# WHU-USI3DV/LaneMapping

Measured on AMD Instinct MI355X. Metric: BEV tiles/sec end-to-end (LAS points -> polylines), higher is better.
Workload: dtype f32; 1 GPU; on-GPU LAS->BEV raster (4,194,304 points/tile resident in HBM) + configs/Proj_polyline_fpn_vit_vertex_2.py, batch=16 per GPU, seeded random weights; lines_per_tile=45, streams=2, hip_graphs=True, points=resident, stream_check=not run (--full runs it), gather_check=n/a (1 rank), raster_check=not run (--full runs it), dist_ranks=1, rccl_ranks=1

## Files before the change

include/lanemap_hip.h:

```cpp
#ifndef LANEMAP_HIP_H
#define LANEMAP_HIP_H
#include <stdint.h>
#ifdef __cplusplus
extern "C" {
#endif

enum { LM_OK = 0, LM_ERR_ARG = 1, LM_ERR_HIP = 2, LM_ERR_NO_DEVICE = 3, LM_ERR_CAPACITY = 4 };
enum { LM_ACT_NONE = 0, LM_ACT_RELU = 1, LM_ACT_GELU = 2 };

int lm_abi_version(void);
const char* lm_last_error(void);
int lm_device_count(void);

int lm_conv2d_nhwc_mfma_f32(void* stream, const float* x, int ldx, const float* wp, int CoutP,
                            const float* scale, const float* shift, const float* res, int ldr, int res_rows,
                            float* y, int ldy, int B, int H, int W, int Cin, int Cout, int KH, int KW,
                            int stride, int pad_h, int pad_w, int dil, int act);
int lm_conv2d_nhwc_mfma_resup_f32(void* stream, const float* x, int ldx, const float* wp, int CoutP, const float* scale,
                                  const float* shift, const float* res_coarse, int ldr, int Hr, int Wr, float* y, int ldy,
                                  int B, int H, int W, int Cin, int Cout, int KH, int KW, int stride, int pad_h, int pad_w,
                                  int dil, int act);

int lm_winograd44_supported(int H, int W, int Cin, int dil);
int lm_winograd44_gn_chunks(int H, int W, int dil);
long lm_winograd44_tiles(int B, int H, int W, int dil);
long lm_winograd44_twin_workspace_bytes(int B, int H, int W, int Cin, int CoutP, int dil);
int lm_conv3x3_winograd44_f32(void* stream, const float* x, int ldx, const float* wu_frag, int CoutP, const float* scale,
                              const float* shift, const float* res, int ldr, float* y, int ldy, int B, int H, int W,
                              int Cin, int Cout, int dil, int act, double* gn_partial);
int lm_conv3x3_winograd44_twin_f32(void* stream, const float* x, int ldx, const float* wu, int CoutP, const float* scale,
                                   const float* shift, const float* res, int ldr, float* y, int ldy, int B, int H, int W,
                                   int Cin, int Cout, int dil, int act, void* workspace, long workspace_bytes);
int lm_wino44_split_fragments(void* stream, const float* frag, float* out, long n_quads);
int lm_conv3x3_winograd44_split_f32(void* stream, const float* x, int ldx, const float* wu_split, int CoutP, const float* scale,
                                    const float* shift, const float* res, int ldr, float* y, int ldy, int B, int H, int W,
                                    int Cin, int Cout, int dil, int act, double* gn_partial, float post);
int lm_conv3x3_winograd44_split_twin_f32(void* stream, const float* x, int ldx, const float* wu, int CoutP, const float* scale,
                                         const float* shift, const float* res, int ldr, float* y, int ldy, int B, int H, int W,
                                         int Cin, int Cout, int dil, int act, void* workspace, long workspace_bytes, float post);

int lm_conv2d_nhwc_mfma_f32_gnstats(void* stream, const float* x, int ldx, const float* wp, int CoutP, const float* shift,
                                    float* y, int ldy, double* gn_partial, int B, int H, int W, int Cin, int Cout,
                                    int KH, int KW, int stride, int pad_h, int pad_w, int dil);
int lm_gn_finalize(void* stream, const double* partial, float* stats, int B, int HW, int C, int nchunk, float eps);
int lm_gn_finalize_split(void* stream, const double* partial, float* stats, int B, int HW, int C, int nchunk, float eps, int split);

int lm_stem_conv7x7_bn_relu(void* stream, const float* x_chw, const float* w_k64, const float* scale,
                            const float* shift, float* y_nhwc, int B, int H, int W);
int lm_stem_conv7x7_bn_relu_u8(void* stream, const unsigned char* x_hwc3, const float* w_k64, const float* scale,
                               const float* shift, float* y_nhwc, int B, int H, int W);
int lm_maxpool3x3s2_nhwc(void* stream, const float* x, float* y, int B, int H, int W, int C);
int lm_conv2d_nhwc_small(void* stream, const float* x, int ldx, const float* w_tc16, const float* scale,
                         const float* shift, float* y, int ldy, int B, int H, int W, int Cin, int Cout,
                         int KH, int KW, int stride, int pad_h, int pad_w, int pre_relu, int act);

int lm_gn_stats(void* stream, const float* x, double* workspace, float* stats, int B, int HW, int C, float eps);
long lm_gn_stats_workspace_bytes(int B, int HW, int C);
int lm_gn_relu_upsample(void* stream, const float* x, const float* stats, const float* gamma, const float* beta,
                        float* y, int B, int Hi, int Wi, int Ho, int Wo, int C, int accumulate);
int lm_gn_relu_upsample_sum(void* stream, int n, const float* const* x, const float* const* stats, const int* Hi, const int* Wi,
                            const int* ldx , const float* gamma, const float* beta,
                            float* y, int B, int Ho, int Wo, int C);
int lm_gn_relu_upsample_sum_conv1x1(void* stream, int n, const float* const* x, const float* const* stats, const int* Hi, const int* Wi,
                                    const int* ldx, const float* gamma, const float* beta, float* y, int B, int Ho, int Wo, int C,
                                    const float* w_c16, const float* bias, int cout, float* y1, int ldy1);
int lm_upsample_bilinear_nhwc(void* stream, const float* x, int ldx, const float* add, int lda, float* y, int ldy,
                              int B, int Hi, int Wi, int Ho, int Wo, int C);
int lm_upsample_bilinear_to_chw(void* stream, const float* x, int ldx, float* y_chw, int B, int Hi, int Wi,
                                int Ho, int Wo, int C);
int lm_layernorm_rows(void* stream, const float* x, const float* gamma, const float* beta, float* y,
                      long rows, int D, float eps);
int lm_unpatchify(void* stream, const float* tokens, float* y_nhwc, int B, int G, int P, int C);
int lm_token_mix_mfma_f32(void* stream, const float* x, const float* wt, int ldw, const float* bias, const float* res, float* y,
                          int B, int M, int K, int N, int act);

int lm_attention_f32(void* stream, const float* qkv, float* out, int B, int N, int heads, int dim_head, float scale);
int lm_attention_masked_f32(void* stream, const float* qkv, float* out, const int* valid, int B, int N, int heads, int dim_head, float scale);

int lm_head_tokens(void* stream, const float* seg, const float* row_nhwc16, float* tok, float seg_bias,
                   int B, int P, int Hr, int Wr, int prop_width, int half_buff);
int lm_head_tokens_window(void* stream, const float* row_nhwc16, float* tok, int B, int P, int Hr, int Wr, int prop_width, int half_buff);
int lm_head_stage2(void* stream, const float* hid, int ldh, int D, const float* w2, const float* b2,
                   float* ext2, float* cls2, float* off2, long M);
int lm_head_proposal_conf(void* stream, const float* tok, const float* wt, const float* bias, float* conf,
                          int BP, int L);

int lm_head_endpoint_tile(void);
int lm_head_endpoint(void* hip_stream, const float* col, int ldc, const float* x_endp, const float* w1p, const float* b1,
                     const float* bn_scale, const float* bn_shift, const float* w2, const float* b2, float* out, int B, int h, int w,
                     int H, int W);

int lm_decode_proposals(void* stream, const float* pconf, const float* ext2, const float* cls2, const float* off2,
                        float* prop_conf, float* v_ext, float* cls_conf, int* cls_idx, double* cls_offset,
                        int B, int P, int R, float exist_thre, int prop_width, int half_buff);
int lm_decode_orient(void* stream, const float* x_nhwc, int ldx, int C, unsigned char* y, long pixels);
int lm_decode_semantic(void* stream, const float* logit_chw3, unsigned char* sem, float* biseg, float* rows,
                       int B, int H, int W, float thre, int raw_mode);
long lm_endp_topk_workspace_bytes(int B);
int lm_endp_topk(void* stream, const float* endp_logit, void* workspace, int* out_idx, float* out_score,
                 int* out_status, int B, int H, int W, int clip, int K);

int lm_pack_segments(void* stream, int n, const void* const* src, const long* bytes, const long* dst_offsets, void* dst);


typedef struct {
    float quat[4];
    float trans[3];
    float bev_img_offset[2];
    float img_reso[2];
    float local_min_ele;
    float ele_reso;
    float inten_lo, inten_hi;
} LmRasterParams;
long lm_bev_raster_workspace_bytes(int B, long max_points_per_tile, int H, int W);
int lm_bev_raster_batch(void* stream, const float* points_xyzi, const long* tile_offsets, const LmRasterParams* params,
                        int B, void* workspace, long workspace_bytes, float* out_chw, unsigned char* out_hwc_u8,
                        int H, int W);
int lm_bev_raster_batch_scaled(void* hip_stream, const float* points_xyzi, const long* tile_offsets, const LmRasterParams* params,
                               int B, void* workspace, long workspace_bytes, float* out_chw, unsigned char* out_hwc_u8,
                               int H, int W, const float* inten_scale);
int lm_tile_ingest_u8(void* stream, const unsigned char* src_hwc, float* dst_chw, int B, int H, int W, int C);

typedef struct {
    double x0, y0, cell;
    int nx, ny;
} LmStripGrid;
int lm_strip_build_grid(const LmRasterParams* params, int T, int H, int W, double z_lo, double z_hi, LmStripGrid* grid,
                        unsigned short* cells, long cells_cap);
long lm_strip_bin_workspace_bytes(long N, int T);
int lm_strip_bin_points(void* hip_stream, const float* points_xyzi, long N, const LmRasterParams* params, int T, int H, int W,
                        double z_lo, double z_hi, void* workspace, long workspace_bytes, long* counts, long* offsets,
                        long* offsets_host, float* binned, long capacity);

long lm_tile_ground_workspace_bytes(int B, int H, int W, int cell_px);
int lm_tile_ground(void* hip_stream, const float* points_xyzi, const long* tile_offsets, const LmRasterParams* params, int B, int H,
                   int W, int cell_px, void* workspace, long workspace_bytes, float* ground, float* ground_min, float* cell_min);
long lm_ground_select_workspace_bytes(long N, int B);
int lm_ground_select(void* hip_stream, const float* points_xyzi, const long* tile_offsets, const LmRasterParams* params, int B, int H,
                     int W, int cell_px, const float* ground, float h_lo, float h_hi, void* workspace, long workspace_bytes,
                     float* points_out, long* out_offsets, long* out_offsets_host);

long lm_tile_intensity_workspace_bytes(int B, int G);
int lm_tile_intensity_window(void* hip_stream, const float* points_xyzi, const long* tile_offsets, const LmRasterParams* params, int B,
                             int H, int W, const int* group, int G, int q_lo_ppm, int q_hi_ppm, void* workspace, long workspace_bytes,
                             int* window, long* count, unsigned* coarse_hist);

long lm_drape_workspace_bytes(long n_vertices, int B, int radius_px);
int lm_drape_vertices(void* hip_stream, const float* points_xyzi, const long* tile_offsets, const LmRasterParams* params, int B, int H,
                      int W, const int* vertices_rc, const long* vertex_offsets, int radius_px, void* workspace, long workspace_bytes,
                      float* z, int* npix, float* pixel_min);

int lm_tile_gap_hist(void* hip_stream, const unsigned char* tiles_hwc_u8, int B, int H, int W, int max_radius_px, unsigned* hist);
int lm_tile_gap_fill(void* hip_stream, const unsigned char* tiles_hwc_u8, int B, int H, int W, const int* radius_px,
                     unsigned char* out_hwc_u8);

int lm_endp_cluster(const int* topk_idx, int n_avail, int Wc, int clip, int k0, int k_step, int k_max, int radius,
                    int min_clusters, int* out_hw, int max_out, int* n_out, int* k_used);
int lm_polyline_assemble(const float* prop_conf, const float* prop_v_ext, const double* cls_offset,
                         const float* bi_seg_rows, const int* endp_hw, int n_endp, int P, int R, float obj_thre,
                         int min_vertices, double* out_lanes, int* endp_keep);
int lm_raster_polylines(const double* lanes, int P, int R, unsigned char* out);
int lm_line8(unsigned char* out, int x1, int y1, int x2, int y2, int colour);
int lm_trace_lines(const double* cols, int n, int R, const float* seg_rows, double* out);
int lm_polyline_backproject(unsigned char* bev_hwc, int H, int W, int C, const double* img_seqs, const int* seq_lens, int L,
                            int Vmax, const double* params13, const double* las_read_offset, double* out);
int lm_polyline_backproject_z(unsigned char* bev_hwc, int H, int W, int C, const double* img_seqs, const int* seq_lens, int L,
                              int Vmax, const double* params13, const double* las_read_offset, double* out,
                              const float* vertex_z, int fit);

long lm_skeletonize_lee_2d(unsigned char* img, int H, int W);

void* lm_merge_create(void);
void lm_merge_destroy(void* merger);
int lm_merge_add_tile(void* merger, const double* points, const int* lens, int n);
long lm_merge_finish(void* merger, long* total_points);
int lm_merge_result(void* merger, double* points, int* lens);
int lm_downsample_seq(const double* seq, int n, double dist_min, double* out);

int lm_softmax_rows(void* stream, float* x, long rows, int cols);
int lm_rowref_select(void* stream, const float* ext, const float* cls, float* mean_out, int* valid, float thr_ext, int* corr,
                     int B, int H, int W, int L);
int lm_rowref_gather(void* stream, const float* x_nhwc8, const int* corr, float* tok, int B, int H, int W, int L);
int lm_rowref_scatter(void* stream, const float* x_nhwc8, const float* tok, const int* corr, const int* valid,
                      float* y_nhwc8, int B, int H, int W, int L);
int lm_rowref_gather_win(void* hip_stream, const float* x_nhwc8, const int* corr, float* tok, int B, int H, int W, int L, int off_grid);
int lm_rowref_scatter_win(void* hip_stream, const float* x_nhwc8, const float* tok, const int* corr, const int* valid,
                          float* y_nhwc8, int B, int H, int W, int L, int off_grid);
int lm_rowref_decode(void* stream, const float* ext2, const float* cls2, unsigned char* conf, unsigned char* cls_map,
                     int* col_idx, int B, int H, int W, int L);

long lm_voxelize_workspace_bytes(long n_points);
long lm_scan_workspace_bytes(long n);
int lm_exclusive_scan_u32(void* stream, const unsigned* in, unsigned* out, long n, void* workspace, long workspace_bytes);
long lm_sort_pairs_workspace_bytes(long n);
int lm_sort_pairs_u32(void* stream, unsigned* keys_io, unsigned* vals_io, long n, int end_bit, void* workspace, long workspace_bytes);
int lm_voxelize_hard(void* stream, const float* points, long n, const float* range_lo_xyz, const float* voxel_size_xyz,
                     const int* grid_xyz, int max_points, int max_voxels, int batch_idx, const int* row_base, int cap_rows,
                     float* feats, int ldf, int* coords, int* row_end, int raster_order, void* workspace,
                     long workspace_bytes);
int lm_sparse_grid_build(void* stream, const int* coords, long n, int* grid, int B, int D, int H, int W);
long lm_sparse_conv_outputs_workspace_bytes(long out_cells);
int lm_sparse_conv_outputs(void* stream, const int* in_coords, long n_in, int B, const int* ksp_zyx9, int Do, int Ho, int Wo,
                           int* out_grid, int* out_coords, int cap_rows, int* out_count, void* workspace, long workspace_bytes);
int lm_sparse_rulebook(void* stream, const int* out_coords, long n_out, const int* in_grid, int B, int D, int H, int W,
                       const int* ksp_zyx9, int* nbr);
int lm_conv_gather_mfma_f32(void* stream, const float* x, int ldx, const int* nbr, int taps, const float* wp, int CoutP,
                            const float* scale, const float* shift, const float* res, int ldr, float* y, int ldy,
                            long M, int Cin, int Cout, int act);
int lm_sparse_to_dense_nhwc(void* stream, const float* feats, int ldf, const int* coords, long n, float* out, int B, int D,
                            int H, int W, int C, int flip_h);
int lm_upsample_bicubic_nhwc(void* stream, const float* x, float* y, int B, int H, int W, int C, int Ho, int Wo);

typedef struct {
    int version_major, version_minor, point_format, record_len;
    long n_points, offset_to_points;
    double scale[3], offset[3], min_xyz[3], max_xyz[3];
} LmLasHeader;
int lm_las_parse_header(const unsigned char* bytes, long len, LmLasHeader* out);
int lm_las_decode_points(void* stream, const unsigned char* records, int record_len, long n, const double* scale,
                         const double* offset, const double* shift, float inten_lo, float inten_hi, int normalise,
                         float* out_xyzi);
enum { LM_LAS_DROP_SYNTHETIC = 1, LM_LAS_DROP_KEYPOINT = 2, LM_LAS_DROP_WITHHELD = 4, LM_LAS_DROP_OVERLAP = 8 };
enum { LM_LAS_RETURNS_ALL = 0, LM_LAS_RETURNS_FIRST = 1, LM_LAS_RETURNS_LAST = 2, LM_LAS_RETURNS_SINGLE = 3 };
typedef struct { unsigned class_mask[8]; unsigned drop_flags; int returns; float z_lo, z_hi; } LmLasSelect;
long lm_las_select_workspace_bytes(long n);
int lm_las_decode_select(void* hip_stream, const unsigned char* records, int record_len, int point_format, long n,
                         const double* scale, const double* offset, const double* shift, float inten_lo, float inten_hi,
                         int normalise, const LmLasSelect* select, void* workspace, long workspace_bytes, float* out_xyzi,
                         long* kept, unsigned long* class_hist);

typedef struct {
    double x0, y0, cell;
    int nx, ny, min_line, max_line;
    long n_segments, n_entries;
    float half_width;
} LmLineGrid;
int lm_line_index_build(const float* segments, long S, float half_width, double cell, LmLineGrid* grid, int* cell_start,
                        long cell_start_cap, int* cell_segs, long cell_segs_cap);
int lm_label_points(void* hip_stream, const float* points_xyzi, long N, const float* segments, long S, const LmLineGrid* grid,
                    const int* cell_start, const int* cell_segs, float half_width, float z_tol, float min_intensity, int* line,
                    float* dist2);
int lm_las_label_records(void* hip_stream, const unsigned char* records, int record_len, int point_format, long n, const double* scale,
                         const double* offset, const double* shift, const LmLasSelect* select, const float* segments, long S,
                         const LmLineGrid* grid, const int* cell_start, const int* cell_segs, float half_width, float z_tol,
                         float min_intensity, int marking_class, int write_line_id, unsigned char* records_out, int* line,
                         unsigned long* counts, int L);

int lm_line_profile_points(void* hip_stream, const float* points_xyzi, long N, const float* segments, long S, const LmLineGrid* grid,
                           const int* cell_start, const int* cell_segs, float half_width, const float* stations, const int* bin_start,
                           const int* bin_start_host, int L, double bin, float z_tol, float min_intensity, int accumulate, long* bins,
                           long n_bins);
int lm_las_line_profile_records(void* hip_stream, const unsigned char* records, int record_len, int point_format, long n,
                                const double* scale, const double* offset, const double* shift, const LmLasSelect* select,
                                const float* segments, long S, const LmLineGrid* grid, const int* cell_start, const int* cell_segs,
                                float half_width, const float* stations, const int* bin_start, const int* bin_start_host, int L, double bin,
                                float z_tol, float min_intensity, int accumulate, long* bins, long n_bins);

int lm_png_info(const unsigned char* data, long size, int* H, int* W, int* C);
int lm_png_decode_u8(const unsigned char* data, long size, unsigned char* out_hwc, long out_bytes);
int lm_png_decode_files_u8(const char* const* paths, int n, unsigned char* out_nhwc, int H, int W, int C, int threads);
int lm_zlib_inflate(const unsigned char* data, long size, unsigned char* out, long capacity, long* produced);

long lm_lane_json_text(const double* lane_vertexes, int n_lines, int row_size, int with_pervertex_semantics, char* out, long cap);
int lm_lane_json_write(const double* lane_vertexes, int n_lines, int row_size, int with_pervertex_semantics, const char* path);
int lm_seqs_json_write(const double* seqs, const int* lens, int L, int Vmax, int D, const char* path);

#ifdef __cplusplus
}
#endif
#endif
```

lanemapping_amd/_lib.py:

```python
import ctypes as C
import os

_HERE = os.path.dirname(os.path.abspath(__file__))
LIB_PATH = os.environ.get('LANEMAP_HIP_LIB') or os.path.join(_HERE, 'liblanemap_hip.so')

c_f32p = C.POINTER(C.c_float)
vp, i32, i64, f32 = C.c_void_p, C.c_int, C.c_long, C.c_float


class LmRasterParams(C.Structure):
    _fields_ = [('quat', C.c_float * 4), ('trans', C.c_float * 3), ('bev_img_offset', C.c_float * 2),
                ('img_reso', C.c_float * 2), ('local_min_ele', C.c_float), ('ele_reso', C.c_float),
                ('inten_lo', C.c_float), ('inten_hi', C.c_float)]


class LmLasHeader(C.Structure):
    _fields_ = [('version_major', C.c_int), ('version_minor', C.c_int), ('point_format', C.c_int), ('record_len', C.c_int),
                ('n_points', C.c_long), ('offset_to_points', C.c_long), ('scale', C.c_double * 3), ('offset', C.c_double * 3),
                ('min_xyz', C.c_double * 3), ('max_xyz', C.c_double * 3)]


class LmStripGrid(C.Structure):
    _fields_ = [('x0', C.c_double), ('y0', C.c_double), ('cell', C.c_double), ('nx', C.c_int), ('ny', C.c_int)]


class LmLasSelect(C.Structure):
    _fields_ = [('class_mask', C.c_uint * 8), ('drop_flags', C.c_uint), ('returns', C.c_int), ('z_lo', C.c_float), ('z_hi', C.c_float)]


class LmLineGrid(C.Structure):
    _fields_ = [('x0', C.c_double), ('y0', C.c_double), ('cell', C.c_double), ('nx', C.c_int), ('ny', C.c_int), ('min_line', C.c_int),
                ('max_line', C.c_int), ('n_segments', C.c_long), ('n_entries', C.c_long), ('half_width', C.c_float)]


SIGNATURES = {
    'lm_abi_version': (i32, []),
    'lm_last_error': (C.c_char_p, []),
    'lm_device_count': (i32, []),
    'lm_conv2d_nhwc_mfma_f32': (i32, [vp, vp, i32, vp, i32, vp, vp, vp, i32, i32, vp, i32,
                                      i32, i32, i32, i32, i32, i32, i32, i32, i32, i32, i32, i32]),
    'lm_conv2d_nhwc_mfma_resup_f32': (i32, [vp, vp, i32, vp, i32, vp, vp, vp, i32, i32, i32, vp, i32,
                                            i32, i32, i32, i32, i32, i32, i32, i32, i32, i32, i32, i32]),
    'lm_winograd44_supported': (i32, [i32, i32, i32, i32]),
    'lm_winograd44_gn_chunks': (i32, [i32, i32, i32]),
    'lm_winograd44_tiles': (i64, [i32, i32, i32, i32]),
    'lm_winograd44_twin_workspace_bytes': (i64, [i32, i32, i32, i32, i32, i32]),
    'lm_conv3x3_winograd44_f32': (i32, [vp, vp, i32, vp, i32, vp, vp, vp, i32, vp, i32, i32, i32, i32, i32, i32, i32, i32, vp]),
    'lm_conv3x3_winograd44_twin_f32': (i32, [vp, vp, i32, vp, i32, vp, vp, vp, i32, vp, i32, i32, i32, i32, i32, i32, i32, i32, vp, i64]),
    'lm_wino44_split_fragments': (i32, [vp, vp, vp, i64]),
    'lm_conv3x3_winograd44_split_f32': (i32, [vp, vp, i32, vp, i32, vp, vp, vp, i32, vp, i32, i32, i32, i32, i32, i32, i32, i32, vp, f32]),
    'lm_conv3x3_winograd44_split_twin_f32': (i32, [vp, vp, i32, vp, i32, vp, vp, vp, i32, vp, i32, i32, i32, i32, i32, i32, i32, i32, vp, i64, f32]),
    'lm_conv2d_nhwc_mfma_f32_gnstats': (i32, [vp, vp, i32, vp, i32, vp, vp, i32, vp] + [i32] * 11),
    'lm_gn_finalize': (i32, [vp, vp, vp, i32, i32, i32, i32, f32]),
    'lm_gn_finalize_split': (i32, [vp, vp, vp, i32, i32, i32, i32, f32, i32]),
    'lm_stem_conv7x7_bn_relu': (i32, [vp, vp, vp, vp, vp, vp, i32, i32, i32]),
    'lm_stem_conv7x7_bn_relu_u8': (i32, [vp, vp, vp, vp, vp, vp, i32, i32, i32]),
    'lm_maxpool3x3s2_nhwc': (i32, [vp, vp, vp, i32, i32, i32, i32]),
    'lm_conv2d_nhwc_small': (i32, [vp, vp, i32, vp, vp, vp, vp, i32, i32, i32, i32, i32, i32, i32, i32, i32, i32, i32, i32, i32]),
    'lm_gn_stats': (i32, [vp, vp, vp, vp, i32, i32, i32, f32]),
    'lm_gn_stats_workspace_bytes': (i64, [i32, i32, i32]),
    'lm_gn_relu_upsample': (i32, [vp, vp, vp, vp, vp, vp, i32, i32, i32, i32, i32, i32, i32]),
    'lm_gn_relu_upsample_sum': (i32, [vp, i32, vp, vp, vp, vp, vp, vp, vp, vp, i32, i32, i32, i32]),
    'lm_gn_relu_upsample_sum_conv1x1': (i32, [vp, i32, vp, vp, vp, vp, vp, vp, vp, vp, i32, i32, i32, i32, vp, vp, i32, vp, i32]),
    'lm_upsample_bilinear_nhwc': (i32, [vp, vp, i32, vp, i32, vp, i32, i32, i32, i32, i32, i32, i32]),
    'lm_upsample_bilinear_to_chw': (i32, [vp, vp, i32, vp, i32, i32, i32, i32, i32, i32]),
    'lm_layernorm_rows': (i32, [vp, vp, vp, vp, vp, i64, i32, f32]),
    'lm_token_mix_mfma_f32': (i32, [vp, vp, vp, i32, vp, vp, vp, i32, i32, i32, i32, i32]),
    'lm_unpatchify': (i32, [vp, vp, vp, i32, i32, i32, i32]),
    'lm_attention_f32': (i32, [vp, vp, vp, i32, i32, i32, i32, f32]),
    'lm_attention_masked_f32': (i32, [vp, vp, vp, vp, i32, i32, i32, i32, f32]),
    'lm_head_tokens': (i32, [vp, vp, vp, vp, f32, i32, i32, i32, i32, i32, i32]),
    'lm_head_tokens_window': (i32, [vp, vp, vp, i32, i32, i32, i32, i32, i32]),
    'lm_head_stage2': (i32, [vp, vp, i32, i32, vp, vp, vp, vp, vp, i64]),
    'lm_head_proposal_conf': (i32, [vp, vp, vp, vp, vp, i32, i32]),
    'lm_head_endpoint_tile': (i32, []),
    'lm_head_endpoint': (i32, [vp, vp, i32, vp, vp, vp, vp, vp, vp, vp, vp, i32, i32, i32, i32, i32]),
    'lm_decode_proposals': (i32, [vp, vp, vp, vp, vp, vp, vp, vp, vp, vp, i32, i32, i32, f32, i32, i32]),
    'lm_decode_orient': (i32, [vp, vp, i32, i32, vp, i64]),
    'lm_decode_semantic': (i32, [vp, vp, vp, vp, vp, i32, i32, i32, f32, i32]),
    'lm_endp_topk_workspace_bytes': (i64, [i32]),
    'lm_endp_topk': (i32, [vp, vp, vp, vp, vp, vp, i32, i32, i32, i32, i32]),
    'lm_pack_segments': (i32, [vp, i32, vp, vp, vp, vp]),
    'lm_bev_raster_workspace_bytes': (i64, [i32, i64, i32, i32]),
    'lm_bev_raster_batch': (i32, [vp, vp, C.POINTER(i64), C.POINTER(LmRasterParams), i32, vp, i64, vp, vp, i32, i32]),
    'lm_bev_raster_batch_scaled': (i32, [vp, vp, C.POINTER(i64), C.POINTER(LmRasterParams), i32, vp, i64, vp, vp, i32, i32, c_f32p]),
    'lm_tile_ingest_u8': (i32, [vp, vp, vp, i32, i32, i32, i32]),
    'lm_strip_build_grid': (i32, [C.POINTER(LmRasterParams), i32, i32, i32, C.c_double, C.c_double, C.POINTER(LmStripGrid), vp, i64]),
    'lm_strip_bin_workspace_bytes': (i64, [i64, i32]),
    'lm_strip_bin_points': (i32, [vp, vp, i64, C.POINTER(LmRasterParams), i32, i32, i32, C.c_double, C.c_double, vp, i64, vp, vp,
                                  C.POINTER(i64), vp, i64]),
    'lm_tile_ground_workspace_bytes': (i64, [i32, i32, i32, i32]),
    'lm_tile_ground': (i32, [vp, vp, C.POINTER(i64), C.POINTER(LmRasterParams), i32, i32, i32, i32, vp, i64, vp, vp, vp]),
    'lm_ground_select_workspace_bytes': (i64, [i64, i32]),
    'lm_ground_select': (i32, [vp, vp, C.POINTER(i64), C.POINTER(LmRasterParams), i32, i32, i32, i32, vp, f32, f32, vp, i64, vp, vp,
                               C.POINTER(i64)]),
    'lm_tile_intensity_workspace_bytes': (i64, [i32, i32]),
    'lm_tile_intensity_window': (i32, [vp, vp, C.POINTER(i64), C.POINTER(LmRasterParams), i32, i32, i32, C.POINTER(i32), i32, i32, i32, vp, i64,
                                       vp, vp, vp]),
    'lm_drape_workspace_bytes': (i64, [i64, i32, i32]),
    'lm_drape_vertices': (i32, [vp, vp, C.POINTER(i64), C.POINTER(LmRasterParams), i32, i32, i32, vp, C.POINTER(i64), i32, vp, i64, vp, vp, vp]),
    'lm_tile_gap_hist': (i32, [vp, vp, i32, i32, i32, i32, vp]),
    'lm_tile_gap_fill': (i32, [vp, vp, i32, i32, i32, C.POINTER(i32), vp]),
    'lm_endp_cluster': (i32, [vp, i32, i32, i32, i32, i32, i32, i32, i32, vp, i32, vp, vp]),
    'lm_polyline_assemble': (i32, [vp, vp, vp, vp, vp, i32, i32, i32, f32, i32, vp, vp]),
    'lm_raster_polylines': (i32, [vp, i32, i32, vp]),
    'lm_line8': (i32, [vp, i32, i32, i32, i32, i32]),
    'lm_trace_lines': (i32, [vp, i32, i32, vp, vp]),
    'lm_polyline_backproject': (i32, [vp, i32, i32, i32, vp, vp, i32, i32, vp, vp, vp]),
    'lm_polyline_backproject_z': (i32, [vp, i32, i32, i32, vp, vp, i32, i32, vp, vp, vp, vp, i32]),
    'lm_skeletonize_lee_2d': (i64, [vp, i32, i32]),
    'lm_merge_create': (vp, []),
    'lm_merge_destroy': (None, [vp]),
    'lm_merge_add_tile': (i32, [vp, vp, vp, i32]),
    'lm_merge_finish': (i64, [vp, C.POINTER(i64)]),
    'lm_merge_result': (i32, [vp, vp, vp]),
    'lm_downsample_seq': (i32, [vp, i32, C.c_double, vp]),
    'lm_softmax_rows': (i32, [vp, vp, i64, i32]),
    'lm_rowref_select': (i32, [vp, vp, vp, vp, vp, f32, vp, i32, i32, i32, i32]),
    'lm_rowref_gather': (i32, [vp, vp, vp, vp, i32, i32, i32, i32]),
    'lm_rowref_scatter': (i32, [vp, vp, vp, vp, vp, vp, i32, i32, i32, i32]),
    'lm_rowref_gather_win': (i32, [vp, vp, vp, vp, i32, i32, i32, i32, i32]),
    'lm_rowref_scatter_win': (i32, [vp, vp, vp, vp, vp, vp, i32, i32, i32, i32, i32]),
    'lm_rowref_decode': (i32, [vp, vp, vp, vp, vp, vp, i32, i32, i32, i32]),
    'lm_voxelize_workspace_bytes': (i64, [i64]),
    'lm_scan_workspace_bytes': (i64, [i64]),
    'lm_exclusive_scan_u32': (i32, [vp, vp, vp, i64, vp, i64]),
    'lm_sort_pairs_workspace_bytes': (i64, [i64]),
    'lm_sort_pairs_u32': (i32, [vp, vp, vp, i64, i32, vp, i64]),
    'lm_voxelize_hard': (i32, [vp, vp, i64, c_f32p, c_f32p, C.POINTER(i32), i32, i32, i32, vp, i32, vp, i32, vp, vp, i32, vp, i64]),
    'lm_sparse_grid_build': (i32, [vp, vp, i64, vp, i32, i32, i32, i32]),
    'lm_sparse_conv_outputs_workspace_bytes': (i64, [i64]),
    'lm_sparse_conv_outputs': (i32, [vp, vp, i64, i32, C.POINTER(i32), i32, i32, i32, vp, vp, i32, vp, vp, i64]),
    'lm_sparse_rulebook': (i32, [vp, vp, i64, vp, i32, i32, i32, i32, C.POINTER(i32), vp]),
    'lm_conv_gather_mfma_f32': (i32, [vp, vp, i32, vp, i32, vp, i32, vp, vp, vp, i32, vp, i32, i64, i32, i32, i32]),
    'lm_sparse_to_dense_nhwc': (i32, [vp, vp, i32, vp, i64, vp, i32, i32, i32, i32, i32, i32]),
    'lm_upsample_bicubic_nhwc': (i32, [vp, vp, vp, i32, i32, i32, i32, i32, i32]),
    'lm_las_parse_header': (i32, [vp, i64, C.POINTER(LmLasHeader)]),
    'lm_las_decode_points': (i32, [vp, vp, i32, i64, C.POINTER(C.c_double), C.POINTER(C.c_double), C.POINTER(C.c_double), f32, f32,
                                   i32, vp]),
    'lm_las_select_workspace_bytes': (i64, [i64]),
    'lm_las_decode_select': (i32, [vp, vp, i32, i32, i64, C.POINTER(C.c_double), C.POINTER(C.c_double), C.POINTER(C.c_double), f32, f32,
                                   i32, C.POINTER(LmLasSelect), vp, i64, vp, vp, vp]),
    'lm_line_index_build': (i32, [vp, i64, f32, C.c_double, C.POINTER(LmLineGrid), vp, i64, vp, i64]),
    'lm_label_points': (i32, [vp, vp, i64, vp, i64, C.POINTER(LmLineGrid), vp, vp, f32, f32, f32, vp, vp]),
    'lm_las_label_records': (i32, [vp, vp, i32, i32, i64, C.POINTER(C.c_double), C.POINTER(C.c_double), C.POINTER(C.c_double),
                                   C.POINTER(LmLasSelect), vp, i64, C.POINTER(LmLineGrid), vp, vp, f32, f32, f32, i32, i32, vp, vp, vp, i32]),
    'lm_line_profile_points': (i32, [vp, vp, i64, vp, i64, C.POINTER(LmLineGrid), vp, vp, f32, vp, vp, vp, i32, C.c_double, f32, f32, i32, vp, i64]),
    'lm_las_line_profile_records': (i32, [vp, vp, i32, i32, i64, C.POINTER(C.c_double), C.POINTER(C.c_double), C.POINTER(C.c_double),
                                          C.POINTER(LmLasSelect), vp, i64, C.POINTER(LmLineGrid), vp, vp, f32, vp, vp, vp, i32, C.c_double, f32, f32,
                                          i32, vp, i64]),
    'lm_png_info': (i32, [vp, i64, C.POINTER(i32), C.POINTER(i32), C.POINTER(i32)]),
    'lm_png_decode_u8': (i32, [vp, i64, vp, i64]),
    'lm_png_decode_files_u8': (i32, [C.POINTER(C.c_char_p), i32, vp, i32, i32, i32, i32]),
    'lm_zlib_inflate': (i32, [vp, i64, vp, i64, C.POINTER(i64)]),
    'lm_lane_json_text': (i64, [vp, i32, i32, i32, vp, i64]),
    'lm_lane_json_write': (i32, [vp, i32, i32, i32, C.c_char_p]),
    'lm_seqs_json_write': (i32, [vp, vp, i32, i32, i32, C.c_char_p]),
}

_lib = None


class LanemapHipError(RuntimeError):
    pass


def lib():
    global _lib
    if _lib is None:
        if not os.path.exists(LIB_PATH):
            raise LanemapHipError(
                f'{LIB_PATH} is missing: the HIP library is the only implementation of this package '
                '(no CPU fallback). Build it with `python -m lanemapping_amd.build`.')
        import torch
        L = C.CDLL(LIB_PATH)
        for name, (res, args) in SIGNATURES.items():
            fn = getattr(L, name)
            fn.restype = res
            fn.argtypes = args
        _lib = L
    return _lib


def check(code):
    if code != 0:
        raise LanemapHipError(f'lanemap_hip error {code}: {lib().lm_last_error().decode()}')
```

lanemapping_amd/csrc/conv_wino44.hip:

```cpp
#include "common.h"

#include <cstdlib>

typedef float f32x16 __attribute__((ext_vector_type(16)));
typedef float f32x4 __attribute__((ext_vector_type(4)));
typedef float f32x2 __attribute__((ext_vector_type(2)));
typedef _Float16 f16x4 __attribute__((ext_vector_type(4)));
typedef unsigned u32x2 __attribute__((ext_vector_type(2)));

namespace {

__device__ __forceinline__ u32x2 w44_split2(f32x2 t) {
#pragma clang fp contract(off)
    typedef __fp16 f16x2r __attribute__((ext_vector_type(2)));
    const f16x2r h = __builtin_amdgcn_cvt_pkrtz(t[0], t[1]);
    const float h0 = (float)h[0], h1 = (float)h[1];
    const f16x2r l = __builtin_amdgcn_cvt_pkrtz(t[0] - h0, t[1] - h1);
    return u32x2{__builtin_bit_cast(unsigned, h), __builtin_bit_cast(unsigned, l)};
}

constexpr int QBM = 32, QBN = 64, QSEG = 4;
constexpr int QNCELL = 144;
constexpr int QLPW = 14;
constexpr int QGRP = 256 + 8;
constexpr int QRAWF = QLPW * 4 * QGRP;
constexpr int QVF = 36 * 256;
constexpr int QBD = 5, QRING = 6;
static_assert(6 * (QNCELL / 16) * QGRP <= QRAWF && QNCELL % 16 == 0, "patch loads cover the unit");

__device__ __attribute__((aligned(16))) float g_w44_zeros[1024 + 32];

struct W44Geom {
    int B, H, W, dil, Ty, Tx;
    int Timg, Tpad;
    long T;
    LmFastDiv dTx, dTy, ddil, dTpad;
};

W44Geom geom44(int B, int H, int W, int dil) {
    W44Geom g;
    g.B = B; g.H = H; g.W = W; g.dil = dil;
    g.Ty = ((H + dil - 1) / dil + 3) / 4;
    g.Tx = ((W + dil - 1) / dil + 3) / 4;
    g.Timg = dil * dil * g.Ty * g.Tx;
    g.Tpad = (g.Timg + QBM - 1) / QBM * QBM;
    g.T = (long)B * g.Tpad;
    g.dTx = lm_fastdiv_make((unsigned)g.Tx); g.dTy = lm_fastdiv_make((unsigned)g.Ty);
    g.ddil = lm_fastdiv_make((unsigned)dil); g.dTpad = lm_fastdiv_make((unsigned)g.Tpad);
    return g;
}

__device__ __forceinline__ void tile44_decode(const W44Geom& g, int t, int& pa, int& pb, int& ty, int& tx) {
    tx = t % g.Tx;
    t /= g.Tx;
    ty = t % g.Ty;
    const int ph = t / g.Ty;
    pa = ph / g.dil;
    pb = ph - pa * g.dil;
}

__device__ __forceinline__ void w44_bt(const float (&d)[6], float (&t)[6]) {
#pragma clang fp contract(off)
    t[0] = __builtin_fmaf(4.f, d[0], __builtin_fmaf(-5.f, d[2], d[4]));
    t[5] = __builtin_fmaf(4.f, d[1], __builtin_fmaf(-5.f, d[3], d[5]));
    const float p = __builtin_fmaf(-4.f, d[2], d[4]), q = __builtin_fmaf(-4.f, d[1], d[3]);
    t[1] = p + q;
    t[2] = p - q;
    const float r = d[4] - d[2], s = d[3] - d[1];
    t[3] = __builtin_fmaf(2.f, s, r);
    t[4] = __builtin_fmaf(-2.f, s, r);
}

__device__ __forceinline__ float w44_fma(float k, float a, float c) { return __builtin_fmaf(k, a, c); }
__device__ __forceinline__ f32x4 w44_fma(float k, f32x4 a, f32x4 c) { return __builtin_elementwise_fma(f32x4{k, k, k, k}, a, c); }
template <typename T>
__device__ __forceinline__ void w44_at(const T (&m)[6], T (&y)[4]) {
#pragma clang fp contract(off)
    const T s1 = m[1] + m[2], d1 = m[1] - m[2], s3 = m[3] + m[4], d3 = m[3] - m[4];
    y[0] = (m[0] + s1) + s3;
    y[1] = w44_fma(2.f, d3, d1);
    y[2] = w44_fma(4.f, s3, s1);
    y[3] = w44_fma(8.f, d3, d1) + m[5];
}

__global__ __launch_bounds__(256) void wino44_input_kernel(const float* __restrict__ x, int ldx, W44Geom g, int C, float* __restrict__ V) {
    const long e = (long)blockIdx.x * 256 + threadIdx.x;
    if (e >= g.T * C) return;
    const int c = (int)(e % C);
    const long m = e / C;
    const int b = (int)(m / g.Tpad), t = (int)(m - (long)b * g.Tpad);
    float d[6][6];
    int pa = 0, pb = 0, ty = 0, tx = 0;
    const bool real = t < g.Timg;
    if (real) tile44_decode(g, t, pa, pb, ty, tx);
#pragma unroll
    for (int i = 0; i < 6; ++i)
#pragma unroll
        for (int j = 0; j < 6; ++j) {
            const int yy = (4 * ty + i - 1) * g.dil + pa, xx = (4 * tx + j - 1) * g.dil + pb;
            const bool ok = real && (4 * ty + i - 1) >= 0 && (4 * tx + j - 1) >= 0 && yy < g.H && xx < g.W;
            d[i][j] = ok ? x[(((long)b * g.H + yy) * g.W + xx) * ldx + c] : 0.f;
        }
    float w[6][6];
#pragma unroll
    for (int j = 0; j < 6; ++j) {
        const float col[6] = {d[0][j], d[1][j], d[2][j], d[3][j], d[4][j], d[5][j]};
        float t6[6];
        w44_bt(col, t6);
#pragma unroll
        for (int i = 0; i < 6; ++i) w[i][j] = t6[i];
    }
#pragma unroll
    for (int i = 0; i < 6; ++i) {
        float t6[6];
        w44_bt(w[i], t6);
#pragma unroll
        for (int j = 0; j < 6; ++j) V[((long)(6 * i + j) * g.T + m) * C + c] = t6[j];
    }
}

template <bool SPLIT>
__global__ __launch_bounds__(64) void wino44_gemm_kernel(const float* __restrict__ V, const float* __restrict__ U, float* __restrict__ M, long T,
                                                         int C, int CoutP) {
    const int lane = threadIdx.x;
    const long m0 = (long)blockIdx.x * 32;
    const int n0 = blockIdx.y * 32, xi = blockIdx.z;
    f32x16 acc;
#pragma unroll
    for (int r = 0; r < 16; ++r) acc[r] = 0.f;
    const float* a = V + ((long)xi * T + m0 + (lane & 31)) * C + 4 * (lane >> 5);
    const float* b = U + ((long)xi * CoutP + n0 + (lane & 31)) * C + 4 * (lane >> 5);
    for (int u = 0; u < C / 8; ++u) {
        const f32x4 av = *reinterpret_cast<const f32x4*>(a + 8 * u), bv = *reinterpret_cast<const f32x4*>(b + 8 * u);
        if constexpr (SPLIT) {
            const u32x2 a01 = w44_split2(f32x2{av[0], av[1]}), a23 = w44_split2(f32x2{av[2], av[3]});
            const u32x2 b01 = w44_split2(f32x2{bv[0], bv[1]}), b23 = w44_split2(f32x2{bv[2], bv[3]});
            const f16x4 ah = __builtin_bit_cast(f16x4, u32x2{a01[0], a23[0]}), al = __builtin_bit_cast(f16x4, u32x2{a01[1], a23[1]});
            const f16x4 bh = __builtin_bit_cast(f16x4, u32x2{b01[0], b23[0]}), bl = __builtin_bit_cast(f16x4, u32x2{b01[1], b23[1]});
            acc = __builtin_amdgcn_mfma_f32_32x32x8f16(ah, bh, acc, 0, 0, 0);
            acc = __builtin_amdgcn_mfma_f32_32x32x8f16(ah, bl, acc, 0, 0, 0);
            acc = __builtin_amdgcn_mfma_f32_32x32x8f16(al, bh, acc, 0, 0, 0);
        } else {
#pragma unroll
            for (int e = 0; e < 4; ++e) acc = __builtin_amdgcn_mfma_f32_32x32x2f32(av[e], bv[e], acc, 0, 0, 0);
        }
    }
#pragma unroll
    for (int r = 0; r < 16; ++r) {
        const int i = (r & 3) + 8 * (r >> 2) + 4 * (lane >> 5);
        M[((long)xi * T + m0 + i) * CoutP + n0 + (lane & 31)] = acc[r];
    }
}

struct W44Epi {
    const float* scale; const float* shift; const float* res; float* y;
    int ldr, ldy, Cout, act;
    float post;
};

__device__ __forceinline__ float w44_tail(float v, int n, const W44Epi& e, long pix) {
#pragma clang fp contract(off)
    const float sh = e.shift ? e.shift[n] : 0.f;
    if (e.post != 0.f) v = v * ((e.scale ? e.scale[n] : 1.f) * e.post) + sh;
    else v = e.scale ? v * e.scale[n] + sh : v + sh;
    if (e.res) v += e.res[pix * e.ldr + n];
    if (e.act == LM_ACT_RELU) v = fmaxf(v, 0.f);
    return v;
}

__global__ __launch_bounds__(256) void wino44_output_kernel(const float* __restrict__ M, W44Geom g, int CoutP, W44Epi e) {
    const long idx = (long)blockIdx.x * 256 + threadIdx.x;
    if (idx >= g.T * e.Cout) return;
    const int n = (int)(idx % e.Cout);
    const long m = idx / e.Cout;
    const int b = (int)(m / g.Tpad), t = (int)(m - (long)b * g.Tpad);
    if (t >= g.Timg) return;
    int pa, pb, ty, tx;
    tile44_decode(g, t, pa, pb, ty, tx);
    float z[4][6];
#pragma unroll
    for (int j = 0; j < 6; ++j) {
        float col[6], y4[4];
#pragma unroll
        for (int i = 0; i < 6; ++i) col[i] = M[((long)(6 * i + j) * g.T + m) * CoutP + n];
        w44_at(col, y4);
#pragma unroll
        for (int yy = 0; yy < 4; ++yy) z[yy][j] = y4[yy];
    }
#pragma unroll
    for (int yy = 0; yy < 4; ++yy) {
        float o[4];
        w44_at(z[yy], o);
#pragma unroll
        for (int xx = 0; xx < 4; ++xx) {
            const int oy = (4 * ty + yy) * g.dil + pa, ox = (4 * tx + xx) * g.dil + pb;
            if (oy >= g.H || ox >= g.W) continue;
            const long pix = ((long)b * g.H + oy) * g.W + ox;
            e.y[pix * e.ldy + n] = w44_tail(o[xx], n, e, pix);
        }
    }
}

__global__ __launch_bounds__(256) void wino44_split_frag_kernel(const f32x4* __restrict__ in, f32x4* __restrict__ out, long n) {
    const long i = (long)blockIdx.x * 256 + threadIdx.x;
    if (i >= n) return;
    const f32x4 v = in[i];
    const u32x2 a = w44_split2(f32x2{v[0], v[1]}), b = w44_split2(f32x2{v[2], v[3]});
    typedef unsigned u32x4 __attribute__((ext_vector_type(4)));
    out[i] = __builtin_bit_cast(f32x4, u32x4{a[0], b[0], a[1], b[1]});
}

struct W44Params {
    const float* x; const float* U; const float* scale; const float* shift; const float* res; float* y; const float* zeros;
    int ldx, ldr, ldy, C, Cout, NT, act;
    int n_inner;
    LmFastDiv dnt;
    double* gn_part;
    W44Geom g;
    float post;
};

__device__ __forceinline__ f32x2 pk_fma(const f32x2 a, const f32x2 b, const f32x2 c) {
    f32x2 r;
    asm("v_pk_fma_f32 %0, %1, %2, %3" : "=v"(r) : "v"(a), "s"(b), "v"(c));
    return r;
}
__device__ __forceinline__ f32x2 pk_fnma(const f32x2 a, const f32x2 b, const f32x2 c) {
    f32x2 r;
    asm("v_pk_fma_f32 %0, %1, %2, %3 neg_lo:[1,0,0] neg_hi:[1,0,0]" : "=v"(r) : "v"(a), "s"(b), "v"(c));
    return r;
}
__device__ __forceinline__ f32x2 pk_add(const f32x2 a, const f32x2 b) {
    f32x2 r;
    asm("v_pk_add_f32 %0, %1, %2" : "=v"(r) : "v"(a), "v"(b));
    return r;
}
__device__ __forceinline__ f32x2 pk_sub(const f32x2 a, const f32x2 b) {
    f32x2 r;
    asm("v_pk_add_f32 %0, %1, %2 neg_lo:[0,1] neg_hi:[0,1]" : "=v"(r) : "v"(a), "v"(b));
    return r;
}

struct W44K {
    f32x2 c2, c4, c5;
};

__device__ __forceinline__ void pk_bt(const f32x2 (&d)[6], f32x2 (&t)[6], const W44K& k) {
    const f32x2 a = pk_fnma(d[2], k.c5, d[4]), b = pk_fnma(d[3], k.c5, d[5]);
    const f32x2 p = pk_fnma(d[2], k.c4, d[4]), q = pk_fnma(d[1], k.c4, d[3]);
    const f32x2 r = pk_sub(d[4], d[2]), s = pk_sub(d[3], d[1]);
    t[0] = pk_fma(d[0], k.c4, a);
    t[5] = pk_fma(d[1], k.c4, b);
    t[1] = pk_add(p, q);
    t[2] = pk_sub(p, q);
    t[3] = pk_fma(s, k.c2, r);
    t[4] = pk_fnma(s, k.c2, r);
}

struct W44Xf {
    f32x2 e[6][5];
    f32x2 w[3][6];
    f32x2 tA[6], tB[6], tC[6];
};
template <int C>
__device__ __forceinline__ void w44_preread(W44Xf& d, const float* rawrow, const int (&roff)[6]) {
    constexpr int ROWF = (QNCELL / 16) * QGRP;
    const float* s = rawrow + roff[C];
#pragma unroll
    for (int r = 0; r < 5; ++r) d.e[C][r] = *reinterpret_cast<const f32x2*>(s + r * ROWF);
}
template <bool LOWER, int C>
__device__ __forceinline__ void w44_pass1x2(W44Xf& d, const W44K& k) {
    const f32x2 (&e)[5] = d.e[C];
    const f32x2 (&f)[5] = d.e[C + 1];
    if constexpr (!LOWER) {
        const f32x2 a0 = pk_fnma(e[2], k.c5, e[4]), a1 = pk_fnma(f[2], k.c5, f[4]);
        const f32x2 p0 = pk_fnma(e[2], k.c4, e[4]), p1 = pk_fnma(f[2], k.c4, f[4]);
        const f32x2 q0 = pk_fnma(e[1], k.c4, e[3]), q1 = pk_fnma(f[1], k.c4, f[3]);
        d.w[0][C] = pk_fma(e[0], k.c4, a0);
        d.w[0][C + 1] = pk_fma(f[0], k.c4, a1);
        d.w[1][C] = pk_add(p0, q0);
        d.w[1][C + 1] = pk_add(p1, q1);
        d.w[2][C] = pk_sub(p0, q0);
        d.w[2][C + 1] = pk_sub(p1, q1);
    } else {
        const f32x2 a0 = pk_fnma(e[2], k.c5, e[4]), a1 = pk_fnma(f[2], k.c5, f[4]);
        const f32x2 r0 = pk_sub(e[3], e[1]), r1 = pk_sub(f[3], f[1]);
        const f32x2 s0 = pk_sub(e[2], e[0]), s1 = pk_sub(f[2], f[0]);
        d.w[2][C] = pk_fma(e[0], k.c4, a0);
        d.w[2][C + 1] = pk_fma(f[0], k.c4, a1);
        d.w[0][C] = pk_fma(s0, k.c2, r0);
        d.w[0][C + 1] = pk_fma(s1, k.c2, r1);
        d.w[1][C] = pk_fnma(s0, k.c2, r0);
        d.w[1][C + 1] = pk_fnma(s1, k.c2, r1);
    }
}
template <bool SPLIT>
__device__ __forceinline__ void w44_vstore(float* v, int j, const f32x2 t) {
    if constexpr (SPLIT) {
        const u32x2 w = w44_split2(t);
        reinterpret_cast<unsigned*>(v)[j * 256] = w[0];
        reinterpret_cast<unsigned*>(v)[j * 256 + 128] = w[1];
    } else {
        *reinterpret_cast<f32x2*>(v + j * 256) = t;
    }
}
template <int K, bool SPLIT>
__device__ __forceinline__ void w44_xf_lds(W44Xf& d, const float* rawrow, const int (&roff)[6], float* vA, float* vB, float* vC) {
    auto st = [](float* v, int j, const f32x2 t) { w44_vstore<SPLIT>(v, j, t); };
    if constexpr (K == 0) {
        st(vB, 2, d.tB[2]); st(vB, 5, d.tB[5]);
        w44_preread<0>(d, rawrow, roff); w44_preread<1>(d, rawrow, roff);
    } else if constexpr (K == 1) {
        st(vC, 0, d.tC[0]); st(vC, 1, d.tC[1]);
        w44_preread<2>(d, rawrow, roff); w44_preread<3>(d, rawrow, roff);
    } else if constexpr (K == 2) {
        st(vC, 2, d.tC[2]); st(vC, 3, d.tC[3]);
        w44_preread<4>(d, rawrow, roff); w44_preread<5>(d, rawrow, roff);
    } else if constexpr (K == 3) {
        st(vC, 4, d.tC[4]); st(vC, 5, d.tC[5]);
    } else if constexpr (K == 5) {
        st(vA, 0, d.tA[0]); st(vA, 1, d.tA[1]); st(vA, 2, d.tA[2]);
    } else if constexpr (K == 6) {
        st(vA, 3, d.tA[3]); st(vA, 4, d.tA[4]); st(vA, 5, d.tA[5]);
    } else if constexpr (K == 7) {
        st(vB, 0, d.tB[0]); st(vB, 1, d.tB[1]); st(vB, 3, d.tB[3]); st(vB, 4, d.tB[4]);
    }
}
template <int K>
__device__ __forceinline__ void w44_xf_valu(W44Xf& d, bool lower, const W44K& k) {
    if constexpr (K >= 1 && K <= 3) {
        if (lower) w44_pass1x2<true, 2 * K - 2>(d, k);
        else w44_pass1x2<false, 2 * K - 2>(d, k);
    } else if constexpr (K == 4) {
        pk_bt(d.w[0], d.tA, k);
    } else if constexpr (K == 5) {
        pk_bt(d.w[1], d.tB, k);
    } else if constexpr (K == 6) {
        pk_bt(d.w[2], d.tC, k);
    }
}
template <bool SPLIT>
__device__ __forceinline__ void w44_xf_all(W44Xf& d, const float* rawrow, const int (&roff)[6], float* vA, float* vB, float* vC, bool lower,
                                           const W44K& k) {
    w44_preread<0>(d, rawrow, roff); w44_preread<1>(d, rawrow, roff); w44_preread<2>(d, rawrow, roff);
    w44_preread<3>(d, rawrow, roff); w44_preread<4>(d, rawrow, roff); w44_preread<5>(d, rawrow, roff);
    w44_xf_valu<1>(d, lower, k); w44_xf_valu<2>(d, lower, k); w44_xf_valu<3>(d, lower, k);
    w44_xf_valu<4>(d, lower, k); w44_xf_valu<5>(d, lower, k); w44_xf_valu<6>(d, lower, k);
#pragma unroll
    for (int j = 0; j < 6; ++j) {
        w44_vstore<SPLIT>(vA, j, d.tA[j]);
        w44_vstore<SPLIT>(vB, j, d.tB[j]);
        w44_vstore<SPLIT>(vC, j, d.tC[j]);
    }
}

__device__ __forceinline__ void q_bload2(f32x4 (&b)[2], unsigned voff, const float* sbase) {
    asm volatile("global_load_dwordx4 %0, %2, %3\n\t"
                 "global_load_dwordx4 %1, %2, %3 offset:1024"
                 : "=&v"(b[0]), "=&v"(b[1]) : "v"(voff), "s"(sbase) : "memory");
}
template <int N>
__device__ __forceinline__ void q_bwait(f32x4 (&b)[2]) {
    asm volatile("s_waitcnt vmcnt(%2)" : "+v"(b[0]), "+v"(b[1]) : "n"(N) : "memory");
}

__device__ __forceinline__ void mfma_vgpr(f32x16& acc, float a, float b) {
    asm volatile("v_mfma_f32_32x32x2_f32 %0, %1, %2, %0" : "+v"(acc) : "v"(a), "v"(b));
}
template <bool VACC>
__device__ __forceinline__ void q_mfma(f32x16& acc, float a, float b) {
    if constexpr (VACC) mfma_vgpr(acc, a, b);
    else acc = __builtin_amdgcn_mfma_f32_32x32x2f32(a, b, acc, 0, 0, 0);
}
template <bool VACC>
__device__ __forceinline__ void q_mfma16(f32x16& acc, f32x2 a, f32x2 b) {
    const f16x4 ah = __builtin_bit_cast(f16x4, a), bh = __builtin_bit_cast(f16x4, b);
    if constexpr (VACC) asm volatile("v_mfma_f32_32x32x8_f16 %0, %1, %2, %0" : "+v"(acc) : "v"(ah), "v"(bh));
    else acc = __builtin_amdgcn_mfma_f32_32x32x8f16(ah, bh, acc, 0, 0, 0);
}
constexpr int q_ndma(int S) { return S < 9 ? 0 : (S < 14 ? 2 : 1); }
constexpr int q_dma0(int S) { return S < 9 ? 0 : (S < 14 ? 2 * (S - 9) : 10 + (S - 14)); }
constexpr int q_nwait(int S) {
    int c = 0;
    for (int j = S - QBD; j <= S; ++j) c += q_ndma(((j % 18) + 18) % 18);
    return 2 * QBD + c;
}
static_assert(q_dma0(17) + q_ndma(17) == QLPW, "the second phase issues every patch load of a unit");

template <bool SPLIT>
__device__ __forceinline__ f32x4 q_aread(const float* v) {
    if constexpr (SPLIT) {
        return f32x4{v[0], v[32], v[128], v[160]};
    } else {
        const f32x2 lo = *reinterpret_cast<const f32x2*>(v), hi = *reinterpret_cast<const f32x2*>(v + 64);
        return f32x4{lo[0], lo[1], hi[0], hi[1]};
    }
}

template <int S, bool SPLIT>
__device__ __forceinline__ void w44_step(f32x16& acc0, f32x16& acc1, f32x4 (&bq)[QRING][2], unsigned bvoff, const float* bpre,
                                         const float* anext, const f32x4& a_cur, f32x4& a_nxt, const float* const (&gsrc)[QLPW], long goff,
                                         float* rawld, int wave, W44Xf& xf, const float* prerow, const int (&roff)[6], float* vA, float* vB,
                                         float* vC, bool lower, const W44K& kk) {
    typedef __attribute__((address_space(1))) const void gptr_t;
    typedef __attribute__((address_space(3))) void lptr_t;
    constexpr int K = S % 9;
    q_bload2(bq[(S + QBD) % QRING], bvoff, bpre);
#pragma unroll
    for (int i = 0; i < q_ndma(S); ++i) {
        constexpr int L0 = q_dma0(S);
        __builtin_amdgcn_global_load_lds((gptr_t*)(gsrc[L0 + i] + goff), (lptr_t*)(rawld + ((L0 + i) * 4 + wave) * QGRP), 16, 0, 0);
    }
    f32x4 (&b)[2] = bq[S % QRING];
    q_bwait<q_nwait(S)>(b);
    constexpr bool VACC = K == 8;
    const f32x2 a_hi = {a_cur[0], a_cur[1]}, a_lo = {a_cur[2], a_cur[3]};
    if constexpr (SPLIT) q_mfma16<VACC>(acc0, a_hi, f32x2{b[0][0], b[0][1]});
    else q_mfma<VACC>(acc0, a_cur[0], b[0][0]);
    if constexpr (!SPLIT) __builtin_amdgcn_sched_barrier(0);
    if constexpr (K != 4 && K != 8) a_nxt = q_aread<SPLIT>(anext);
    w44_xf_lds<K, SPLIT>(xf, prerow, roff, vA, vB, vC);
    if constexpr (!SPLIT) __builtin_amdgcn_sched_barrier(0);
    w44_xf_valu<K>(xf, lower, kk);
    if constexpr (!SPLIT) __builtin_amdgcn_sched_barrier(0);
    if constexpr (SPLIT) {
        q_mfma16<VACC>(acc1, a_hi, f32x2{b[1][0], b[1][1]});
        q_mfma16<VACC>(acc0, a_hi, f32x2{b[0][2], b[0][3]});
        q_mfma16<VACC>(acc1, a_hi, f32x2{b[1][2], b[1][3]});
        q_mfma16<VACC>(acc0, a_lo, f32x2{b[0][0], b[0][1]});
        q_mfma16<VACC>(acc1, a_lo, f32x2{b[1][0], b[1][1]});
        if constexpr (!VACC) {
#pragma unroll
            for (int i = 0; i < 6; ++i) {
                __builtin_amdgcn_sched_group_barrier(0x008, 1, 0);
                __builtin_amdgcn_sched_group_barrier(0x002, 6, 0);
                __builtin_amdgcn_sched_group_barrier(0x300, 3, 0);
            }
        }
    } else {
        q_mfma<VACC>(acc1, a_cur[0], b[1][0]);
#pragma unroll
        for (int t = 1; t < 4; ++t) {
            q_mfma<VACC>(acc0, a_cur[t], b[0][t]);
            q_mfma<VACC>(acc1, a_cur[t], b[1][t]);
        }
    }
    __builtin_amdgcn_sched_barrier(0);
}

__device__ __forceinline__ float w44_vmax(float a, float b) {
    float r;
    asm("v_max_f32 %0, %1, %2" : "=v"(r) : "v"(a), "v"(b));
    return r;
}
template <bool FULL>
__device__ __forceinline__ void w44_tail_vec(const f32x4 (&z)[4][6], const f32x4 (&rpre)[16], float* yp, int rowstep, int colstep, const f32x4 sc,
                                             const f32x4 sh, float relu_lo, bool has_res, bool gn, f32x4& gsum, f32x4& gsq, int eny, int enx) {
#pragma unroll
    for (int yy = 0; yy < 4; ++yy) {
        f32x4 o[4];
        w44_at(z[yy], o);
#pragma unroll
        for (int xx = 0; xx < 4; ++xx) {
#pragma clang fp contract(off)
            if (!FULL && !(yy < eny && xx < enx)) continue;
            f32x4 v = o[xx] * sc + sh;
            if (gn) {
#pragma unroll
                for (int e = 0; e < 4; ++e) {
                    gsum[e] += v[e];
                    gsq[e] = __builtin_fmaf(v[e], v[e], gsq[e]);
                }
            }
            if (has_res) v += rpre[yy * 4 + xx];
#pragma unroll
            for (int e = 0; e < 4; ++e) v[e] = w44_vmax(v[e], relu_lo);
            *reinterpret_cast<f32x4*>(yp + yy * rowstep + xx * colstep) = v;
        }
    }
}

template <bool SPLIT>
__global__ __launch_bounds__(256) void wino44_kernel(W44Params p) {
    extern __shared__ __attribute__((aligned(16))) float smem[];
    float* const raw0 = smem;
    float* const Vbuf = smem + 2 * QRAWF;
    typedef __attribute__((address_space(1))) const void gptr_t;
    typedef __attribute__((address_space(3))) void lptr_t;
    const int tid = threadIdx.x, lane = tid & 63;
    const int wave = __builtin_amdgcn_readfirstlane(tid >> 6);
    const int n_tiles = (p.Cout + QBN - 1) / QBN;
    unsigned mblk, ntile;
    if (p.n_inner) {
        const unsigned bid = blockIdx.x, per = gridDim.x / 8;
        const unsigned lin = bid < per * 8 ? (bid % 8) * per + bid / 8 : bid;
        mblk = lm_fastdiv(lin, p.dnt);
        ntile = lin - mblk * (unsigned)n_tiles;
    } else {
        const unsigned bid = blockIdx.x, mb = gridDim.x / (unsigned)n_tiles, mbx = mb / 8, full = mbx * 8 * (unsigned)n_tiles;
        if (bid < full) {
            const unsigned xcd = bid % 8, idx = bid / 8;
            ntile = idx / mbx;
            mblk = xcd * mbx + idx % mbx;
        } else {
            const unsigned r = bid - full;
            mblk = 8 * mbx + r / (unsigned)n_tiles;
            ntile = r % (unsigned)n_tiles;
        }
    }
    const long m0 = (long)mblk * QBM;
    const int n0 = (int)ntile * QBN;
    const W44Geom& g = p.g;
    const int bi = (int)lm_fastdiv((unsigned)m0, g.dTpad);
    const int t0 = (int)(m0 - (long)bi * g.Tpad);
    int ts[QSEG + 1], sn[QSEG], iy0[QSEG], ix0[QSEG], oy0[QSEG], ox0[QSEG];
    {
        int at = 0, t = t0;
        const int rest = (int)lm_fastdiv((unsigned)t0, g.dTx), ph = (int)lm_fastdiv((unsigned)rest, g.dTy);
        int tx = t0 - rest * g.Tx, ty = rest - ph * g.Ty;
        int pa = (int)lm_fastdiv((unsigned)ph, g.ddil), pb = ph - pa * g.dil;
#pragma unroll
        for (int s_ = 0; s_ < QSEG; ++s_) {
            ts[s_] = at;
            const bool real = t < g.Timg && at < QBM;
            const int n = at < QBM ? min(QBM - at, g.Tx - tx) : 0;
            sn[s_] = real ? n : 0;
            iy0[s_] = (4 * ty - 1) * g.dil + pa;
            ix0[s_] = (4 * tx - 1) * g.dil + pb;
            oy0[s_] = 4 * ty * g.dil + pa;
            ox0[s_] = 4 * tx * g.dil + pb;
            at += n;
            t += n;
            tx += n;
            if (tx >= g.Tx) {
                tx = 0;
                if (++ty >= g.Ty) {
                    ty = 0;
                    if (++pb >= g.dil) {
                        pb = 0;
                        ++pa;
                    }
                }
            }
        }
        ts[QSEG] = at;
    }
    const float* gsrc[QLPW];
    const int img_pix0 = bi * g.H * g.W;
    int tab_x, tab_y, tab_n;
    {
        int n = sn[0], yb = iy0[0], xb = ix0[0], s0 = 0;
#pragma unroll
        for (int k = 1; k < QSEG; ++k) {
            const bool in = lane >= ts[k] + k;
            n = in ? sn[k] : n;
            yb = in ? iy0[k] : yb;
            xb = in ? ix0[k] : xb;
            s0 = in ? ts[k] + k : s0;
        }
        const int j = lane - s0;
        tab_x = xb + 4 * j * g.dil;
        tab_y = yb;
        tab_n = n > 0 ? 4 * (n - j) + 2 : 0;
    }
    const int gcc = (lane >> 4) & 3, gccd = gcc * g.dil, gsl4 = ((lane >> 2) & 3) << 2, gcq4 = (lane & 3) * 4;
#pragma unroll
    for (int s_ = 0; s_ < QLPW; ++s_) {
        const int q = s_ * 4 + wave;
        const int r = q / (QNCELL / 16), gq = q - r * (QNCELL / 16);
        const int idx = 16 * gq + gsl4;
        const int x0 = __builtin_amdgcn_ds_bpermute(idx, tab_x), y0 = __builtin_amdgcn_ds_bpermute(idx, tab_y);
        const int nn = __builtin_amdgcn_ds_bpermute(idx, tab_n);
        const int yy = y0 + r * g.dil, xx = x0 + gccd;
        const bool ok = (r < 6) & (gcc < nn) & ((unsigned)yy < (unsigned)g.H) & ((unsigned)xx < (unsigned)g.W);
        const long m = -(long)ok;
        const long eoff = ((long)(img_pix0 + yy * g.W + xx) * p.ldx) & m;
        const unsigned long base = (unsigned long)p.zeros + (((unsigned long)p.x - (unsigned long)p.zeros) & (unsigned long)m);
        gsrc[s_] = (const float*)base + eoff + gcq4;
        __builtin_amdgcn_global_load_lds((gptr_t*)gsrc[s_], (lptr_t*)(raw0 + (s_ * 4 + wave) * QGRP), 16, 0, 0);
        __builtin_amdgcn_sched_barrier(0);
    }
    int roff[6], tvoff;
    {
        const int tl = lane & 31;
        int sg = 0;
#pragma unroll
        for (int k = 1; k < QSEG; ++k) sg += (ts[k] < QBM && tl >= ts[k]) ? 1 : 0;
        const int slot = tl + sg, slot1 = slot + 1;
        const int cp = (2 * (wave & 1) + (lane >> 5) + slot) & 3;
        const int pos0 = 16 * (slot >> 2) + (slot & 3), pos1 = 16 * (slot1 >> 2) + (slot1 & 3);
#pragma unroll
        for (int c = 0; c < 6; ++c) {
            const int pos = c < 4 ? pos0 + 4 * c : pos1 + 4 * (c - 4);
            roff[c] = (pos >> 4) * QGRP + (pos & 15) * 16 + 2 * cp;
        }
        tvoff = SPLIT ? cp * 32 + tl : cp * 64 + tl * 2;
    }
    const bool lower = (wave >> 1) != 0;
    float* const vA = Vbuf + (lower ? 3 : 0) * (6 * 256) + tvoff;
    float* const vB = Vbuf + (lower ? 4 : 1) * (6 * 256) + tvoff;
    float* const vC = Vbuf + (lower ? 5 : 2) * (6 * 256) + tvoff;
    const W44K kk = {f32x2{2.f, 2.f}, f32x2{4.f, 4.f}, f32x2{5.f, 5.f}};
    const int qa = wave >> 1, qb = wave & 1;
    const int xi00 = 18 * qa + 3 * qb;
    const float* const Vq = SPLIT ? Vbuf + xi00 * 256 + (lane >> 5) * 64 + (lane & 31)
                                  : Vbuf + xi00 * 256 + (lane >> 5) * 128 + (lane & 31) * 2;
    const int nun = p.C / 16;
    const unsigned bvoff = (unsigned)lane * 16u;
    const long ustride = (long)p.NT * 256;
    const long xstride = (long)(2 * nun) * ustride;
    const float* const bbase = p.U + (long)xi00 * xstride + (long)(n0 >> 5) * 256;

    f32x16 acc[9][2];
#pragma unroll
    for (int k = 0; k < 9; ++k)
#pragma unroll
        for (int b = 0; b < 2; ++b)
#pragma unroll
            for (int r = 0; r < 16; ++r) acc[k][b][r] = 0.f;
    f32x4 bq[QRING][2];
    W44Xf xf;
    const int lowoff = lower ? (QNCELL / 16) * QGRP : 0;
#define LM_QXI(K) (6 * ((K) / 3) + (K) % 3)
#pragma unroll
    for (int k = 0; k < QBD; ++k) q_bload2(bq[k], bvoff, bbase + (long)LM_QXI(k) * xstride);
    {
        const long goff1 = nun > 1 ? 16 : 0;
#pragma unroll
        for (int s_ = 0; s_ < QLPW; ++s_)
            __builtin_amdgcn_global_load_lds((gptr_t*)(gsrc[s_] + goff1), (lptr_t*)(raw0 + QRAWF + (s_ * 4 + wave) * QGRP), 16, 0, 0);
    }
    q_bwait<QLPW>(bq[0]);
    __builtin_amdgcn_s_barrier();
    w44_xf_all<SPLIT>(xf, raw0 + lowoff, roff, vA, vB, vC, lower, kk);
    asm volatile("s_waitcnt lgkmcnt(0)" ::: "memory");
    __builtin_amdgcn_s_barrier();

#define LM_QBPRE(S5) ((S5) < 18 ? bu + (long)((S5) / 9) * ustride + (long)LM_QXI((S5) % 9) * xstride : bu_next + (long)LM_QXI((S5) - 18) * xstride)
#define LM_QSTEP(S, AC, AN) \
    w44_step<S, SPLIT>(acc[(S) % 9][0], acc[(S) % 9][1], bq, bvoff, LM_QBPRE((S) + QBD), Vq + LM_QXI(((S) % 9) + 1 < 9 ? ((S) % 9) + 1 : 0) * 256, \
                AC, AN, gsrc, goff, rawc_w, wave, xf, (S) < 9 ? rawc + 8 + lowoff : rawn + lowoff, roff, vA, vB, vC, lower, kk)
#define LM_QMID(AN)                                          \
    asm volatile("s_waitcnt lgkmcnt(0)" ::: "memory");       \
    __builtin_amdgcn_s_barrier();                            \
    AN = q_aread<SPLIT>(Vq + LM_QXI(5) * 256);
    for (int u = 0; u < nun; ++u) {
        const float* const rawc = raw0 + (u & 1) * QRAWF;
        float* const rawc_w = raw0 + (u & 1) * QRAWF;
        const float* const rawn = raw0 + ((u + 1) & 1) * QRAWF;
        const long goff = u + 2 < nun ? (long)(u + 2) * 16 : 0;
        const float* const bu = bbase + (long)(2 * u) * ustride;
        const float* const bu_next = bbase + (long)(u + 1 < nun ? 2 * (u + 1) : 0) * ustride;
        f32x4 a0, a1;
        a0 = q_aread<SPLIT>(Vq);
        LM_QSTEP(0, a0, a1); LM_QSTEP(1, a1, a0); LM_QSTEP(2, a0, a1); LM_QSTEP(3, a1, a0); LM_QSTEP(4, a0, a1);
        LM_QMID(a1)
        LM_QSTEP(5, a1, a0); LM_QSTEP(6, a0, a1); LM_QSTEP(7, a1, a0); LM_QSTEP(8, a0, a1);
        asm volatile("s_waitcnt lgkmcnt(0)" ::: "memory");
        q_bwait<2 * 9>(bq[0]);
        __builtin_amdgcn_s_barrier();
        a0 = q_aread<SPLIT>(Vq);
        LM_QSTEP(9, a0, a1);  LM_QSTEP(10, a1, a0); LM_QSTEP(11, a0, a1); LM_QSTEP(12, a1, a0); LM_QSTEP(13, a0, a1);
        LM_QMID(a1)
        LM_QSTEP(14, a1, a0); LM_QSTEP(15, a0, a1); LM_QSTEP(16, a1, a0); LM_QSTEP(17, a0, a1);
        asm volatile("s_waitcnt lgkmcnt(0)" ::: "memory");
        __builtin_amdgcn_s_barrier();
    }
#undef LM_QMID
#undef LM_QSTEP
#undef LM_QBPRE
#undef LM_QXI
    static_assert(18 % QRING == 0 && QBD < QRING, "eighteen steps per unit walk the ring a whole number of times");
#pragma unroll
    for (int k = 0; k < QRING; ++k) q_bwait<0>(bq[k]);

    const int etile = tid >> 3, ecq = tid & 7;
    int epix0;
    int eny = 0, enx = 0;
    {
        int nn = sn[0], oy = oy0[0], oxb = ox0[0], tb = 0;
#pragma unroll
        for (int k = 1; k < QSEG; ++k)
            if (etile >= ts[k]) {
                nn = sn[k]; oy = oy0[k]; oxb = ox0[k]; tb = ts[k];
            }
        const int ox = oxb + 4 * (etile - tb) * g.dil;
        epix0 = img_pix0 + oy * g.W + ox;
        if (nn > 0 && oy < g.H && ox < g.W) {
            eny = min(4, (int)lm_fastdiv((unsigned)(g.H - oy + g.dil - 1), g.ddil));
            enx = min(4, (int)lm_fastdiv((unsigned)(g.W - ox + g.dil - 1), g.ddil));
        }
    }
    float* const mw = smem + xi00 * 1024 + (4 * (lane >> 5)) * 32 + (lane & 31);
    const float* const mr = smem + etile * 32 + ecq * 4;
    f32x4 gsum[2] = {{0.f, 0.f, 0.f, 0.f}, {0.f, 0.f, 0.f, 0.f}}, gsq[2] = {{0.f, 0.f, 0.f, 0.f}, {0.f, 0.f, 0.f, 0.f}};
    const bool full = eny == 4 && enx == 4;
    const int ebase = eny > 0 ? epix0 : img_pix0;
    const int ey1 = max(eny - 1, 0), ex1 = max(enx - 1, 0);
    const float relu_lo = p.act == LM_ACT_RELU ? 0.f : -__builtin_inff();
    const bool has_res = p.res != nullptr, gn = p.gn_part != nullptr;
#pragma unroll
    for (int blk = 0; blk < 2; ++blk) {
        const int n = n0 + blk * 32 + ecq * 4;
        const bool vec = (n + 3 < p.Cout) && ((p.ldy & 3) == 0) && (!p.res || (p.ldr & 3) == 0);
        f32x4 sc = {1.f, 1.f, 1.f, 1.f}, sh = {0.f, 0.f, 0.f, 0.f};
        if (vec) {
            if (p.scale) sc = *reinterpret_cast<const f32x4*>(p.scale + n);
            if (p.shift) sh = *reinterpret_cast<const f32x4*>(p.shift + n);
            if constexpr (SPLIT) sc = sc * p.post;
        } else {
#pragma unroll
            for (int e = 0; e < 4; ++e)
                if (n + e < p.Cout) {
                    if (p.scale) sc[e] = p.scale[n + e];
                    if (p.shift) sh[e] = p.shift[n + e];
                    if constexpr (SPLIT) sc[e] = sc[e] * p.post;
                }
        }
        f32x4 rpre[16];
        const bool load_res = vec && has_res;
        const float* const rp = p.res + (long)ebase * p.ldr + n;
        const int rs = g.W * g.dil * p.ldr, cs = g.dil * p.ldr;
        asm volatile("s_waitcnt lgkmcnt(0)" ::: "memory");
        __builtin_amdgcn_s_barrier();
#pragma unroll
        for (int k = 0; k < 9; ++k) {
#pragma unroll
            for (int r = 0; r < 16; ++r) mw[(6 * (k / 3) + k % 3) * 1024 + ((r & 3) + 8 * (r >> 2)) * 32] = acc[k][blk][r];
            if (k < 8 && load_res) {
#pragma unroll
                for (int q = 2 * k; q < 2 * k + 2; ++q)
                    rpre[q] = *reinterpret_cast<const f32x4*>(rp + min(q >> 2, ey1) * rs + min(q & 3, ex1) * cs);
            }
            __builtin_amdgcn_sched_barrier(0);
        }
        asm volatile("s_waitcnt lgkmcnt(0)" ::: "memory");
        __builtin_amdgcn_s_barrier();
        if (n < p.Cout && eny > 0) {
            f32x4 z[4][6];
#pragma unroll
            for (int j = 0; j < 6; ++j) {
                f32x4 col[6], y4[4];
#pragma unroll
                for (int i = 0; i < 6; ++i) col[i] = *reinterpret_cast<const f32x4*>(mr + (6 * i + j) * 1024);
                w44_at(col, y4);
#pragma unroll
                for (int yy = 0; yy < 4; ++yy) z[yy][j] = y4[yy];
            }
            float* const yp = p.y + (long)ebase * p.ldy + n;
            const int rowstep = g.W * g.dil * p.ldy, colstep = g.dil * p.ldy;
            if (vec) {
                if (full) w44_tail_vec<true>(z, rpre, yp, rowstep, colstep, sc, sh, relu_lo, has_res, gn, gsum[blk], gsq[blk], eny, enx);
                else w44_tail_vec<false>(z, rpre, yp, rowstep, colstep, sc, sh, relu_lo, has_res, gn, gsum[blk], gsq[blk], eny, enx);
            } else {
#pragma unroll
                for (int yy = 0; yy < 4; ++yy) {
                    f32x4 o[4];
                    w44_at(z[yy], o);
#pragma unroll
                    for (int xx = 0; xx < 4; ++xx) {
#pragma clang fp contract(off)
                        const f32x4 v = o[xx] * sc + sh;
#pragma unroll
                        for (int e = 0; e < 4; ++e) {
                            if (!(yy < eny && xx < enx && n + e < p.Cout)) continue;
                            if (gn) {
                                gsum[blk][e] += v[e];
                                gsq[blk][e] = __builtin_fmaf(v[e], v[e], gsq[blk][e]);
                            }
                            float u = v[e];
                            if (has_res) u += p.res[((long)ebase + (yy * g.W + xx) * g.dil) * p.ldr + n + e];
                            yp[yy * rowstep + xx * colstep + e] = fmaxf(u, relu_lo);
                        }
                    }
                }
            }
        }
    }
    if (p.gn_part) {
#pragma unroll
        for (int blk = 0; blk < 2; ++blk)
#pragma unroll
            for (int o = 8; o < 64; o <<= 1)
#pragma unroll
                for (int e = 0; e < 4; ++e) {
                    gsum[blk][e] += __shfl_xor(gsum[blk][e], o);
                    gsq[blk][e] += __shfl_xor(gsq[blk][e], o);
                }
        __syncthreads();
        if (lane < 8) {
#pragma unroll
            for (int blk = 0; blk < 2; ++blk) {
                *reinterpret_cast<f32x4*>(smem + (((wave * 2 + blk) * 8 + lane) * 2) * 4) = gsum[blk];
                *reinterpret_cast<f32x4*>(smem + (((wave * 2 + blk) * 8 + lane) * 2 + 1) * 4) = gsq[blk];
            }
        }
        __syncthreads();
        if (tid < 16) {
#pragma clang fp contract(off)
            const int blk = tid >> 3, cq = tid & 7;
            const int n = n0 + blk * 32 + cq * 4;
            f32x4 s = {0.f, 0.f, 0.f, 0.f}, q = {0.f, 0.f, 0.f, 0.f};
#pragma unroll
            for (int w = 0; w < 4; ++w) {
                const f32x4 a = *reinterpret_cast<const f32x4*>(smem + (((w * 2 + blk) * 8 + cq) * 2) * 4);
                const f32x4 b = *reinterpret_cast<const f32x4*>(smem + (((w * 2 + blk) * 8 + cq) * 2 + 1) * 4);
#pragma unroll
                for (int e = 0; e < 4; ++e) {
                    s[e] += a[e];
                    q[e] += b[e];
                }
            }
            const long chunk = t0 / 32;
            double* o = p.gn_part + (((long)bi * (g.Tpad / 32) + chunk) * p.Cout + n) * 2;
            for (int e = 0; e < 4 && n + e < p.Cout; ++e) {
                o[2 * e] = (double)s[e];
                o[2 * e + 1] = (double)q[e];
            }
        }
    }
}

bool w44_ok(const W44Geom& g) { return (QBM - 2) / g.Tx + 2 <= QSEG; }

int w44_zeros(const float** out) {
    static const float* cache[64] = {nullptr};
    int dev = 0;
    LM_HIP(hipGetDevice(&dev));
    LM_REQUIRE(dev >= 0 && dev < 64, "conv_wino44: device index %d", dev);
    if (!cache[dev]) {
        void* sym = nullptr;
        LM_HIP(hipGetSymbolAddress(&sym, HIP_SYMBOL(g_w44_zeros)));
        cache[dev] = (const float*)sym;
    }
    *out = cache[dev];
    return LM_OK;
}

}

LM_API int lm_winograd44_supported(int H, int W, int Cin, int dil) {
    if (dil < 1 || H < 1 || W < 1 || Cin < 16 || Cin % 16 != 0 || Cin > 1024) return 0;
    return w44_ok(geom44(1, H, W, dil)) ? 1 : 0;
}

LM_API int lm_winograd44_gn_chunks(int H, int W, int dil) { return dil < 1 ? 0 : geom44(1, H, W, dil).Tpad / 32; }

LM_API long lm_winograd44_tiles(int B, int H, int W, int dil) { return dil < 1 ? 0 : geom44(B, H, W, dil).T; }

LM_API long lm_winograd44_twin_workspace_bytes(int B, int H, int W, int Cin, int CoutP, int dil) {
    if (dil < 1) return 0;
    return 36 * geom44(B, H, W, dil).T * (long)(Cin + CoutP) * (long)sizeof(float);
}

static int w44_launch(void* stream, const float* x, int ldx, const float* wu_frag, int CoutP, const float* scale,
                      const float* shift, const float* res, int ldr, float* y, int ldy, int B, int H, int W,
                      int Cin, int Cout, int dil, int act, double* gn_partial, float split_post) {
    LM_REQUIRE(x && wu_frag && y, "conv_wino44: null pointer");
    LM_REQUIRE(lm_winograd44_supported(H, W, Cin, dil) && B > 0, "conv_wino44: unsupported shape (H=%d W=%d Cin=%d dil=%d)", H, W, Cin, dil);
    LM_REQUIRE(CoutP >= Cout && CoutP % QBN == 0, "conv_wino44: CoutP=%d must be Cout=%d rounded up to %d", CoutP, Cout, QBN);
    LM_REQUIRE(ldx >= Cin && ldx % 4 == 0 && ldy >= Cout, "conv_wino44: bad leading dimension");
    LM_REQUIRE(act == LM_ACT_NONE || act == LM_ACT_RELU, "conv_wino44: activation %d not supported", act);
    LM_REQUIRE(!gn_partial || (res == nullptr && act == LM_ACT_NONE && Cout % 4 == 0), "conv_wino44(gn stats): no residual / activation");
    W44Params p;
    p.g = geom44(B, H, W, dil);
    LM_REQUIRE((long)B * H * W * ldx < (1L << 40) && (long)B * H * W < (1L << 31) && p.g.T < (1L << 31), "conv_wino44: tensor too large");
    p.x = x; p.U = wu_frag; p.scale = scale; p.shift = shift; p.res = res; p.y = y;
    p.ldx = ldx; p.ldr = ldr; p.ldy = ldy; p.C = Cin; p.Cout = Cout; p.NT = CoutP / 32; p.act = act;
    p.gn_part = gn_partial;
    if (int e = w44_zeros(&p.zeros)) return e;
    static const int order = getenv("LANEMAP_W44_ORDER") ? atoi(getenv("LANEMAP_W44_ORDER")) : 1;
    p.n_inner = order;
    p.dnt = lm_fastdiv_make((unsigned)((Cout + QBN - 1) / QBN));
    const size_t lds = (size_t)(2 * QRAWF + QVF) * sizeof(float);
    static_assert(36 * 32 * 32 <= 2 * QRAWF + QVF, "the product buffer of the epilogue fits");
    const long blocks = (p.g.T / QBM) * ((Cout + QBN - 1) / QBN);
    LM_REQUIRE(blocks > 0 && blocks < (1L << 31) && p.g.T % QBM == 0, "conv_wino44: bad grid %ld", blocks);
    p.post = split_post != 0.f ? split_post : 1.f;
    if (split_post != 0.f) {
        if (int e = lm_ensure_dynamic_lds((const void*)wino44_kernel<true>, lds)) return e;
        hipLaunchKernelGGL(wino44_kernel<true>, dim3((unsigned)blocks), dim3(256), lds, (hipStream_t)stream, p);
    } else {
        if (int e = lm_ensure_dynamic_lds((const void*)wino44_kernel<false>, lds)) return e;
        hipLaunchKernelGGL(wino44_kernel<false>, dim3((unsigned)blocks), dim3(256), lds, (hipStream_t)stream, p);
    }
    LM_LAUNCH_CHECK();
    return LM_OK;
}

LM_API int lm_conv3x3_winograd44_f32(void* stream, const float* x, int ldx, const float* wu_frag, int CoutP, const float* scale,
                                     const float* shift, const float* res, int ldr, float* y, int ldy, int B, int H, int W,
                                     int Cin, int Cout, int dil, int act, double* gn_partial) {
    return w44_launch(stream, x, ldx, wu_frag, CoutP, scale, shift, res, ldr, y, ldy, B, H, W, Cin, Cout, dil, act, gn_partial, 0.f);
}

LM_API int lm_conv3x3_winograd44_split_f32(void* stream, const float* x, int ldx, const float* wu_split, int CoutP, const float* scale,
                                           const float* shift, const float* res, int ldr, float* y, int ldy, int B, int H, int W,
                                           int Cin, int Cout, int dil, int act, double* gn_partial, float post) {
    LM_REQUIRE(post > 0.f, "conv_wino44(split): post scale must be positive");
    return w44_launch(stream, x, ldx, wu_split, CoutP, scale, shift, res, ldr, y, ldy, B, H, W, Cin, Cout, dil, act, gn_partial, post);
}

LM_API int lm_wino44_split_fragments(void* stream, const float* frag, float* out, long n_quads) {
    LM_REQUIRE(frag && out && n_quads > 0 && n_quads < (1L << 38), "wino44_split_fragments: bad arguments");
    hipLaunchKernelGGL(wino44_split_frag_kernel, dim3((unsigned)((n_quads + 255) / 256)), dim3(256), 0, (hipStream_t)stream,
                       reinterpret_cast<const f32x4*>(frag), reinterpret_cast<f32x4*>(out), n_quads);
    LM_LAUNCH_CHECK();
    return LM_OK;
}


static int w44_twin(void* stream, const float* x, int ldx, const float* wu, int CoutP, const float* scale,
                    const float* shift, const float* res, int ldr, float* y, int ldy, int B, int H, int W,
                    int Cin, int Cout, int dil, int act, void* workspace, long workspace_bytes, float split_post) {
    LM_REQUIRE(x && wu && y && workspace, "conv_wino44_twin: null pointer");
    LM_REQUIRE(Cin > 0 && Cin % 8 == 0 && dil >= 1 && B > 0 && H > 0 && W > 0, "conv_wino44_twin: bad shape");
    LM_REQUIRE(CoutP >= Cout && CoutP % 32 == 0 && ldx >= Cin && ldy >= Cout, "conv_wino44_twin: bad CoutP / leading dimension");
    LM_REQUIRE(act == LM_ACT_NONE || act == LM_ACT_RELU, "conv_wino44_twin: activation %d not supported", act);
    LM_REQUIRE(lm_winograd44_twin_workspace_bytes(B, H, W, Cin, CoutP, dil) <= workspace_bytes, "conv_wino44_twin: workspace too small");
    const W44Geom g = geom44(B, H, W, dil);
    LM_REQUIRE(g.T * (long)(Cin > Cout ? Cin : Cout) < (1L << 31) * 256L && g.T / 32 < 65536L * 32768L, "conv_wino44_twin: too large");
    float* V = (float*)workspace;
    float* M = V + 36 * g.T * Cin;
    hipStream_t s = (hipStream_t)stream;
    hipLaunchKernelGGL(wino44_input_kernel, dim3((unsigned)((g.T * Cin + 255) / 256)), dim3(256), 0, s, x, ldx, g, Cin, V);
    LM_LAUNCH_CHECK();
    if (split_post != 0.f)
        hipLaunchKernelGGL(wino44_gemm_kernel<true>, dim3((unsigned)(g.T / 32), (unsigned)(CoutP / 32), 36), dim3(64), 0, s, (const float*)V, wu, M,
                           g.T, Cin, CoutP);
    else
        hipLaunchKernelGGL(wino44_gemm_kernel<false>, dim3((unsigned)(g.T / 32), (unsigned)(CoutP / 32), 36), dim3(64), 0, s, (const float*)V, wu, M,
                           g.T, Cin, CoutP);
    LM_LAUNCH_CHECK();
    W44Epi e;
    e.scale = scale; e.shift = shift; e.res = res; e.y = y; e.ldr = ldr; e.ldy = ldy; e.Cout = Cout; e.act = act;
    e.post = split_post;
    hipLaunchKernelGGL(wino44_output_kernel, dim3((unsigned)((g.T * Cout + 255) / 256)), dim3(256), 0, s, (const float*)M, g, CoutP, e);
    LM_LAUNCH_CHECK();
    return LM_OK;
}

LM_API int lm_conv3x3_winograd44_twin_f32(void* stream, const float* x, int ldx, const float* wu, int CoutP, const float* scale,
                                          const float* shift, const float* res, int ldr, float* y, int ldy, int B, int H, int W,
                                          int Cin, int Cout, int dil, int act, void* workspace, long workspace_bytes) {
    return w44_twin(stream, x, ldx, wu, CoutP, scale, shift, res, ldr, y, ldy, B, H, W, Cin, Cout, dil, act, workspace, workspace_bytes, 0.f);
}

LM_API int lm_conv3x3_winograd44_split_twin_f32(void* stream, const float* x, int ldx, const float* wu, int CoutP, const float* scale,
                                                const float* shift, const float* res, int ldr, float* y, int ldy, int B, int H, int W,
                                                int Cin, int Cout, int dil, int act, void* workspace, long workspace_bytes, float post) {
    LM_REQUIRE(post > 0.f, "conv_wino44_twin(split): post scale must be positive");
    return w44_twin(stream, x, ldx, wu, CoutP, scale, shift, res, ldr, y, ldy, B, H, W, Cin, Cout, dil, act, workspace, workspace_bytes, post);
}
```

lanemapping_amd/ops.py:

```python
import ctypes as C
import math

import torch

from ._lib import lib, check, LmRasterParams, LmStripGrid, LmLineGrid, LanemapHipError

ACT_NONE, ACT_RELU, ACT_GELU = 0, 1, 2


def _stream():
    return C.c_void_p(torch._C._cuda_getCurrentRawStream(torch._C._cuda_getDevice()))


def _ptr(t):
    if t is None:
        return None
    if not t.is_cuda:
        raise LanemapHipError('lanemapping_amd ops need tensors on an MI355X (HIP) device; no CPU fallback exists')
    if t.device.index != torch._C._cuda_getDevice():
        raise LanemapHipError(f'tensor on cuda:{t.device.index} but the current device is cuda:{torch._C._cuda_getDevice()}: '
                              'call torch.cuda.set_device() (one process drives one GPU)')
    return C.c_void_p(t.data_ptr())


def new_act(B, C_, H, W, device, dtype=torch.float32):
    return torch.empty((B, H, W, C_), device=device, dtype=dtype).permute(0, 3, 1, 2)


def as_nhwc(x):
    B, C_, H, W = x.shape
    sb, sc, sh, sw = x.stride()
    ok = (sc == 1 or C_ == 1) and sw >= C_ and (sh == W * sw or H == 1) and (sb == H * W * sw or B == 1)
    if not ok:
        x = x.permute(0, 2, 3, 1).contiguous().permute(0, 3, 1, 2)
        sw = C_
    return x, sw


def fold_bn(bn, conv_bias=None, eps=1e-5):
    scale = bn.weight / torch.sqrt(bn.running_var + eps)
    shift = bn.bias - bn.running_mean * scale
    if conv_bias is not None:
        shift = shift + conv_bias * scale
    return scale.float().contiguous(), shift.float().contiguous()


def pack_mfma(w):
    if w.dim() == 2:
        w = w[:, :, None, None]
    if w.dim() == 3:
        w = w[:, :, :, None]
    co, ci, kh, kw = w.shape
    cop = (co + 127) // 128 * 128
    p = torch.zeros((kh * kw, cop, ci), device=w.device, dtype=torch.float32)
    p[:, :co, :] = w.permute(2, 3, 0, 1).reshape(kh * kw, co, ci)
    return p.contiguous()


_W44_G = [[1 / 4, 0, 0], [-1 / 6, -1 / 6, -1 / 6], [-1 / 6, 1 / 6, -1 / 6], [1 / 24, 1 / 12, 1 / 6], [1 / 24, -1 / 12, 1 / 6], [0, 0, 1]]


def pack_wino44(w):
    co, ci, kh, kw = w.shape
    assert kh == 3 and kw == 3
    G = torch.tensor(_W44_G, device=w.device, dtype=torch.float64)
    U = torch.einsum('ij,ocjk,lk->iloc', G, w.double(), G).reshape(36, co, ci).float()
    cop = (co + 63) // 64 * 64
    p = torch.zeros((36, cop, ci), device=w.device, dtype=torch.float32)
    p[:, :co, :] = U
    return p.contiguous()


def pack_wino44_fragments(wu):
    xi, cop, ci = wu.shape
    assert xi == 36 and cop % 64 == 0 and ci % 16 == 0
    t = wu.reshape(36, cop // 32, 32, ci // 8, 2, 4)
    return t.permute(0, 3, 1, 4, 2, 5).contiguous().reshape(36, ci // 8, cop // 32, 64, 4)


class SplitFragments:
    __slots__ = ('words', 'post')

    def __init__(self, words, post):
        self.words, self.post = words, float(post)

    @property
    def shape(self):
        return self.words.shape


def split_scale(wu):
    m = float(wu.abs().max())
    return 1.0 if m == 0.0 else 2.0 ** (12 - math.floor(math.log2(m)))


def pack_wino44_fragments_split(wu):
    assert wu.is_cuda, 'the fragments are split on the device (no CPU path)'
    sc = split_scale(wu)
    frag = pack_wino44_fragments(wu * sc)
    out = torch.empty_like(frag)
    check(lib().lm_wino44_split_fragments(_stream(), _ptr(frag), _ptr(out), frag.numel() // 4))
    return SplitFragments(out, 1.0 / sc)


def pack_small(w):
    co, ci, kh, kw = w.shape
    if co > 16:
        assert co % 16 == 0 and co <= 64, f'pack_small: Cout={co} must be <= 16 or 32 / 48 / 64'
        return torch.stack([pack_small(w[16 * i:16 * (i + 1)]) for i in range(co // 16)]).contiguous()
    p = torch.zeros((kh * kw, ci, 16), device=w.device, dtype=torch.float32)
    p[:, :, :co] = w.permute(2, 3, 1, 0).reshape(kh * kw, ci, co)
    return p.contiguous()


def pack_token_mix(w):
    if w.dim() == 3:
        w = w[:, :, 0]
    m, k = w.shape
    p = torch.zeros(((k + 15) // 16 * 16, (m + 127) // 128 * 128), device=w.device, dtype=torch.float32)
    p[:k, :m] = w.t()
    return p.contiguous()


_conv_hook = None


def set_conv_hook(fn):
    global _conv_hook
    _conv_hook = fn


def conv_mfma(x, wp, cout, kh=1, kw=1, stride=1, pad=0, dil=1, scale=None, shift=None, res=None, act=ACT_NONE,
              out=None, res_rows=0, res_up=None):
    x, ldx = as_nhwc(x)
    B, cin, H, W = x.shape
    ph, pw = (pad, pad) if isinstance(pad, int) else pad
    Ho = (H + 2 * ph - dil * (kh - 1) - 1) // stride + 1
    Wo = (W + 2 * pw - dil * (kw - 1) - 1) // stride + 1
    if out is None:
        out = new_act(B, cout, Ho, Wo, x.device)
    out_, ldy = as_nhwc(out)
    assert out_.data_ptr() == out.data_ptr(), 'conv_mfma: `out` must already be NHWC-stored'
    ldr = 0
    if res is not None:
        if res.dim() == 4:
            res, ldr = as_nhwc(res)
        else:
            ldr = res.stride(0)
    if res_up is not None:
        assert res is None and res_rows == 0
        ru, ldu = as_nhwc(res_up)
        assert ru.shape[0] == B and ru.shape[1] == cout

    def launch():
        if res_up is not None:
            check(lib().lm_conv2d_nhwc_mfma_resup_f32(_stream(), _ptr(x), ldx, _ptr(wp), wp.shape[1], _ptr(scale), _ptr(shift),
                                                      _ptr(ru), ldu, ru.shape[2], ru.shape[3], _ptr(out), ldy, B, H, W, cin, cout,
                                                      kh, kw, stride, ph, pw, dil, act))
            return
        check(lib().lm_conv2d_nhwc_mfma_f32(_stream(), _ptr(x), ldx, _ptr(wp), wp.shape[1], _ptr(scale), _ptr(shift),
                                            _ptr(res), ldr, res_rows, _ptr(out), ldy, B, H, W, cin, cout, kh, kw,
                                            stride, ph, pw, dil, act))
    if _conv_hook is not None:
        _conv_hook(f'conv {cin}->{cout} k{kh}x{kw} s{stride} d{dil} @{H}x{W} B{B}', 2.0 * B * Ho * Wo * cout * cin * kh * kw, launch)
    else:
        launch()
    return out


def _hooked(kind, flops, launch, executed=None):
    if _conv_hook is not None:
        _conv_hook(kind, flops, launch, executed)
    else:
        launch()


def wino44_supported(H, W, cin, dil=1):
    return bool(lib().lm_winograd44_supported(int(H), int(W), int(cin), int(dil)))


def conv_wino44(x, wf, cout, dil=1, scale=None, shift=None, res=None, act=ACT_NONE, out=None, gn_eps=None, gn_split=1):
    x, ldx = as_nhwc(x)
    B, cin, H, W = x.shape
    cop = wf.shape[2] * 32
    y = out if out is not None else new_act(B, cout, H, W, x.device)
    y_, ldy = as_nhwc(y)
    assert y_.data_ptr() == y.data_ptr(), 'conv_wino44: `out` must already be NHWC-stored'
    r, ldr = (None, 0) if res is None else as_nhwc(res)
    part = None
    if gn_eps is not None:
        part = torch.empty((B, lib().lm_winograd44_gn_chunks(H, W, dil), cout, 2), device=x.device, dtype=torch.float64)
    tiles = lib().lm_winograd44_tiles(B, H, W, dil)
    if isinstance(wf, SplitFragments):
        _hooked(f'wino44split {cin}->{cout} k3x3 d{dil} @{H}x{W} B{B}', 2.0 * B * H * W * cout * cin * 9,
                lambda: check(lib().lm_conv3x3_winograd44_split_f32(_stream(), _ptr(x), ldx, _ptr(wf.words), cop, _ptr(scale), _ptr(shift), _ptr(r),
                                                                    ldr, _ptr(y), ldy, B, H, W, cin, cout, dil, act, _ptr(part), wf.post)),
                3 * 2.0 * 36 * tiles * cin * cout)
    else:
        _hooked(f'wino44 {cin}->{cout} k3x3 d{dil} @{H}x{W} B{B}', 2.0 * B * H * W * cout * cin * 9,
                lambda: check(lib().lm_conv3x3_winograd44_f32(_stream(), _ptr(x), ldx, _ptr(wf), cop, _ptr(scale), _ptr(shift), _ptr(r), ldr,
                                                              _ptr(y), ldy, B, H, W, cin, cout, dil, act, _ptr(part))),
                2.0 * 36 * tiles * cin * cout)
    if gn_eps is None:
        return y
    if gn_split > 1:
        stats = torch.empty((gn_split, B, cout // gn_split, 2), device=x.device, dtype=torch.float32)
        check(lib().lm_gn_finalize_split(_stream(), _ptr(part), _ptr(stats), B, H * W, cout, part.shape[1], gn_eps, gn_split))
        return y, stats
    stats = torch.empty((B, cout, 2), device=x.device, dtype=torch.float32)
    check(lib().lm_gn_finalize(_stream(), _ptr(part), _ptr(stats), B, H * W, cout, part.shape[1], gn_eps))
    return y, stats


def conv_wino44_twin(x, wu, cout, dil=1, scale=None, shift=None, res=None, act=ACT_NONE, out=None, split=False):
    x, ldx = as_nhwc(x)
    B, cin, H, W = x.shape
    cop = wu.shape[1]
    y = out if out is not None else new_act(B, cout, H, W, x.device)
    y_, ldy = as_nhwc(y)
    assert y_.data_ptr() == y.data_ptr(), 'conv_wino44_twin: `out` must already be NHWC-stored'
    r, ldr = (None, 0) if res is None else as_nhwc(res)
    need = lib().lm_winograd44_twin_workspace_bytes(B, H, W, cin, cop, dil)
    ws = torch.empty(need, device=x.device, dtype=torch.uint8)
    if split:
        sc = split_scale(wu)
        wus = (wu * sc).contiguous()
        check(lib().lm_conv3x3_winograd44_split_twin_f32(_stream(), _ptr(x), ldx, _ptr(wus), cop, _ptr(scale), _ptr(shift), _ptr(r), ldr,
                                                         _ptr(y), ldy, B, H, W, cin, cout, dil, act, _ptr(ws), need, 1.0 / sc))
        return y
    check(lib().lm_conv3x3_winograd44_twin_f32(_stream(), _ptr(x), ldx, _ptr(wu), cop, _ptr(scale), _ptr(shift), _ptr(r), ldr,
                                               _ptr(y), ldy, B, H, W, cin, cout, dil, act, _ptr(ws), need))
    return y


def conv_mfma_gnstats(x, wp, cout, kh, kw, stride, pad, dil, shift, eps=1e-5):
    x, ldx = as_nhwc(x)
    B, cin, H, W = x.shape
    Ho = (H + 2 * pad - dil * (kh - 1) - 1) // stride + 1
    Wo = (W + 2 * pad - dil * (kw - 1) - 1) // stride + 1
    out = new_act(B, cout, Ho, Wo, x.device)
    nchunk = Ho * Wo // 64
    part = torch.empty((B, nchunk, cout, 2), device=x.device, dtype=torch.float64)
    stats = torch.empty((B, cout, 2), device=x.device, dtype=torch.float32)
    def launch():
        check(lib().lm_conv2d_nhwc_mfma_f32_gnstats(_stream(), _ptr(x), ldx, _ptr(wp), wp.shape[1], _ptr(shift), _ptr(out), cout,
                                                    _ptr(part), B, H, W, cin, cout, kh, kw, stride, pad, pad, dil))
    if _conv_hook is not None:
        _conv_hook(f'conv+gn {cin}->{cout} k{kh}x{kw} s{stride} d{dil} @{H}x{W} B{B}', 2.0 * B * Ho * Wo * cout * cin * kh * kw, launch)
    else:
        launch()
    check(lib().lm_gn_finalize(_stream(), _ptr(part), _ptr(stats), B, Ho * Wo, cout, nchunk, eps))
    return out, stats


def linear_mfma(x2d, wp, n_out, scale=None, shift=None, res=None, res_rows=0, act=ACT_NONE, out=None):
    assert x2d.dim() == 2 and x2d.stride(1) == 1
    M, K = x2d.shape
    if out is None:
        out = torch.empty((M, n_out), device=x2d.device, dtype=torch.float32)
    ldr = res.stride(0) if res is not None else 0
    def launch():
        check(lib().lm_conv2d_nhwc_mfma_f32(_stream(), _ptr(x2d), x2d.stride(0), _ptr(wp), wp.shape[1], _ptr(scale),
                                            _ptr(shift), _ptr(res), ldr, res_rows, _ptr(out), out.stride(0),
                                            1, 1, M, K, n_out, 1, 1, 1, 0, 0, 1, act))
    if _conv_hook is not None:
        _conv_hook(f'gemm M{M} K{K} N{n_out}', 2.0 * M * n_out * K, launch)
    else:
        launch()
    return out


def token_mix(x2d, wt, M, bias, B, res=None, act=ACT_NONE, out=None):
    assert x2d.dim() == 2 and x2d.is_contiguous() and x2d.shape[0] % B == 0
    K, N = x2d.shape[0] // B, x2d.shape[1]
    assert wt.shape[0] >= K and wt.shape[1] >= M and bias.numel() == M
    if out is None:
        out = torch.empty((B * M, N), device=x2d.device, dtype=torch.float32)
    assert out.is_contiguous() and tuple(out.shape) == (B * M, N)
    if res is not None:
        assert res.is_contiguous() and tuple(res.shape) == (B * M, N)
    def launch():
        check(lib().lm_token_mix_mfma_f32(_stream(), _ptr(x2d), _ptr(wt), wt.shape[1], _ptr(bias), _ptr(res), _ptr(out),
                                          B, M, K, N, act))
    if _conv_hook is not None:
        _conv_hook(f'token_mix M{M} K{K} N{N} B{B}', 2.0 * B * M * K * N, launch)
    else:
        launch()
    return out


def conv_small(x, w16, cout, kh=1, kw=1, stride=1, pad=0, scale=None, shift=None, pre_relu=False, act=ACT_NONE, out=None):
    x, ldx = as_nhwc(x)
    B, cin, H, W = x.shape
    ph, pw = (pad, pad) if isinstance(pad, int) else pad
    Ho = (H + 2 * ph - kh) // stride + 1
    Wo = (W + 2 * pw - kw) // stride + 1
    if out is None:
        out = new_act(B, cout, Ho, Wo, x.device)
    out_, ldy = as_nhwc(out)
    assert out_.data_ptr() == out.data_ptr()
    check(lib().lm_conv2d_nhwc_small(_stream(), _ptr(x), ldx, _ptr(w16), _ptr(scale), _ptr(shift), _ptr(out), ldy,
                                     B, H, W, cin, cout, kh, kw, stride, ph, pw, int(pre_relu), act))
    return out


def stem(x, w_k64, scale, shift):
    x = x.contiguous()
    if x.dtype == torch.uint8:
        B, H, W, C_ = x.shape
        assert C_ == 3, 'u8 tiles are [B,H,W,3]'
    else:
        B, _, H, W = x.shape
    Ho, Wo = (H - 1) // 2 + 1, (W - 1) // 2 + 1
    out = new_act(B, 64, Ho, Wo, x.device)
    fn = lib().lm_stem_conv7x7_bn_relu_u8 if x.dtype == torch.uint8 else lib().lm_stem_conv7x7_bn_relu
    check(fn(_stream(), _ptr(x), _ptr(w_k64), _ptr(scale), _ptr(shift), _ptr(out), B, H, W))
    return out


def maxpool3x3s2(x):
    x, ld = as_nhwc(x)
    B, C_, H, W = x.shape
    assert ld == C_
    out = new_act(B, C_, (H - 1) // 2 + 1, (W - 1) // 2 + 1, x.device)
    check(lib().lm_maxpool3x3s2_nhwc(_stream(), _ptr(x), _ptr(out), B, H, W, C_))
    return out


def gn_stats(x, eps=1e-5):
    x, ld = as_nhwc(x)
    B, C_, H, W = x.shape
    assert ld == C_
    ws = torch.empty(lib().lm_gn_stats_workspace_bytes(B, H * W, C_) // 8, device=x.device, dtype=torch.float64)
    stats = torch.empty((B, C_, 2), device=x.device, dtype=torch.float32)
    check(lib().lm_gn_stats(_stream(), _ptr(x), _ptr(ws), _ptr(stats), B, H * W, C_, eps))
    return stats


def gn_relu_upsample(x, stats, gamma, beta, size, out=None, accumulate=False):
    x, ld = as_nhwc(x)
    B, C_, H, W = x.shape
    assert ld == C_
    Ho, Wo = size
    if out is None:
        assert not accumulate
        out = new_act(B, C_, Ho, Wo, x.device)
    check(lib().lm_gn_relu_upsample(_stream(), _ptr(x), _ptr(stats), _ptr(gamma), _ptr(beta), _ptr(out),
                                    B, H, W, Ho, Wo, C_, int(accumulate)))
    return out


def gn_relu_upsample_sum(terms, gamma, beta, size, out=None, proj=None, keep_sum=True):
    n = len(terms)
    xs = [as_nhwc(x) for x, _ in terms]
    B, C_ = xs[0][0].shape[:2]
    for (x, ld) in xs:
        assert ld >= C_ and ld % 4 == 0 and x.shape[0] == B and x.shape[1] == C_
    Ho, Wo = size
    dev = xs[0][0].device
    if out is None and (keep_sum or proj is None):
        out = new_act(B, C_, Ho, Wo, dev)
    vp_arr, i_arr = C.c_void_p * n, C.c_int * n
    head = (_stream(), n, vp_arr(*[_ptr(x) for x, _ in xs]), vp_arr(*[_ptr(st) for _, st in terms]),
            i_arr(*[x.shape[2] for x, _ in xs]), i_arr(*[x.shape[3] for x, _ in xs]), i_arr(*[ld for _, ld in xs]),
            _ptr(gamma), _ptr(beta))
    if proj is None:
        check(lib().lm_gn_relu_upsample_sum(*head, _ptr(out), B, Ho, Wo, C_))
        return out
    w16, bias, cout = proj[:3]
    out1 = proj[3] if len(proj) > 3 and proj[3] is not None else new_act(B, cout, Ho, Wo, dev)
    o1, ldy1 = as_nhwc(out1)
    assert o1.data_ptr() == out1.data_ptr()
    check(lib().lm_gn_relu_upsample_sum_conv1x1(*head, _ptr(out) if keep_sum else None, B, Ho, Wo, C_, _ptr(w16), _ptr(bias), cout,
                                                _ptr(out1), ldy1))
    return (out, out1) if keep_sum else out1


def upsample_nhwc(x, size, add=None, out=None):
    x, ldx = as_nhwc(x)
    B, C_, H, W = x.shape
    Ho, Wo = size
    if out is None and add is None and (Ho, Wo) == (H, W):
        return x
    if out is None:
        out = new_act(B, C_, Ho, Wo, x.device)
    out_, ldy = as_nhwc(out)
    assert out_.data_ptr() == out.data_ptr()
    lda = 0
    if add is not None:
        add, lda = as_nhwc(add)
    check(lib().lm_upsample_bilinear_nhwc(_stream(), _ptr(x), ldx, _ptr(add), lda, _ptr(out), ldy, B, H, W, Ho, Wo, C_))
    return out


def pack_head_endpoint(conv1, bn, conv2):
    s, beta = fold_bn(bn)
    return (conv1.weight.permute(1, 2, 3, 0).float().contiguous(), conv1.bias.float().contiguous(), s, beta,
            conv2.weight[0].float().contiguous(), conv2.bias.float().contiguous())


def head_endpoint_tile():
    return int(lib().lm_head_endpoint_tile())


def head_endpoint(col, x_endp, packed, out=None):
    col_, ldc = as_nhwc(col)
    B, C_, h, w = col_.shape
    assert C_ == 16, 'head_endpoint: col has 16 channels'
    x_endp = x_endp.contiguous()
    assert x_endp.dim() == 4 and x_endp.shape[0] == B and x_endp.shape[1] == 1 and x_endp.dtype == torch.float32
    H, W = x_endp.shape[2:]
    if out is None:
        out = torch.empty((B, 1, H, W), device=col.device, dtype=torch.float32)
    w1p, b1, s, beta, w2, b2 = packed
    assert w1p.numel() == 17 * 36 and w2.numel() == 36
    check(lib().lm_head_endpoint(_stream(), _ptr(col_), ldc, _ptr(x_endp), _ptr(w1p), _ptr(b1), _ptr(s), _ptr(beta), _ptr(w2), _ptr(b2),
                                 _ptr(out), B, h, w, H, W))
    return out


def upsample_to_chw(x, size):
    x, ldx = as_nhwc(x)
    B, C_, H, W = x.shape
    Ho, Wo = size
    out = torch.empty((B, C_, Ho, Wo), device=x.device, dtype=torch.float32)
    check(lib().lm_upsample_bilinear_to_chw(_stream(), _ptr(x), ldx, _ptr(out), B, H, W, Ho, Wo, C_))
    return out


def layernorm(x2d, gamma, beta, eps=1e-5):
    assert x2d.is_contiguous()
    out = torch.empty_like(x2d)
    check(lib().lm_layernorm_rows(_stream(), _ptr(x2d), _ptr(gamma), _ptr(beta), _ptr(out), x2d.shape[0], x2d.shape[1], eps))
    return out


def unpatchify(tokens, B, G, P, C_):
    out = new_act(B, C_, G * P, G * P, tokens.device)
    check(lib().lm_unpatchify(_stream(), _ptr(tokens.contiguous()), _ptr(out), B, G, P, C_))
    return out


def attention(qkv, B, N, heads, dim_head, scale, valid=None):
    assert qkv.is_contiguous()
    out = torch.empty((B * N, heads * dim_head), device=qkv.device, dtype=torch.float32)
    if valid is None:
        check(lib().lm_attention_f32(_stream(), _ptr(qkv), _ptr(out), B, N, heads, dim_head, float(scale)))
    else:
        assert valid.dtype == torch.int32 and valid.is_contiguous() and tuple(valid.shape) == (B, N)
        check(lib().lm_attention_masked_f32(_stream(), _ptr(qkv), _ptr(out), _ptr(valid), B, N, heads, dim_head, float(scale)))
    return out


def head_tokens(seg, row, P, prop_width, half_buff, seg_bias):
    row, ld = as_nhwc(row)
    B, C_, Hr, Wr = row.shape
    assert C_ == 16 and ld == 16
    tok = torch.empty((B * P * Hr, 16 * (prop_width + 2 * half_buff)), device=row.device, dtype=torch.float32)
    if seg is None:
        check(lib().lm_head_tokens_window(_stream(), _ptr(row), _ptr(tok), B, P, Hr, Wr, prop_width, half_buff))
        return tok
    seg = seg.reshape(B, 2 * Hr, 2 * Wr).contiguous()
    check(lib().lm_head_tokens(_stream(), _ptr(seg), _ptr(row), _ptr(tok), float(seg_bias), B, P, Hr, Wr, prop_width, half_buff))
    return tok


def head_stage2(hid, D, w2, b2, B, P, R, w_small=None):
    M = hid.shape[0]
    FW = (w2.shape[0] - 3) // 2
    assert w2.shape == (3 + 2 * FW, D) and b2.numel() == 3 + 2 * FW and hid.shape[1] >= 3 * D and hid.stride(1) == 1
    ext2 = torch.empty((B, P, R, 3), device=hid.device, dtype=torch.float32)
    cls2 = torch.empty((B, P, R, FW), device=hid.device, dtype=torch.float32)
    off2 = torch.empty((B, P, R, FW), device=hid.device, dtype=torch.float32)
    if FW == 10:
        check(lib().lm_head_stage2(_stream(), _ptr(hid), hid.stride(0), D, _ptr(w2), _ptr(b2), _ptr(ext2), _ptr(cls2), _ptr(off2), M))
        return ext2, cls2, off2
    if w_small is None:
        raise ValueError(f'head_stage2: prop_fea_width {FW} runs through lm_conv2d_nhwc_small and needs the pack_small weights')
    bounds = (0, 3, 3 + FW, 3 + 2 * FW)
    for br, (y, w16) in enumerate(zip((ext2, cls2, off2), w_small)):
        n = bounds[br + 1] - bounds[br]
        assert tuple(w16.shape) == (1, D, 16)
        x = hid[:, br * D:(br + 1) * D]
        shift = b2[bounds[br]:bounds[br + 1]]
        check(lib().lm_conv2d_nhwc_small(_stream(), _ptr(x), hid.stride(0), _ptr(w16), None, _ptr(shift), _ptr(y), n,
                                         1, 1, M, D, n, 1, 1, 1, 0, 0, 0, ACT_NONE))
    return ext2, cls2, off2


def head_proposal_conf(tok, wt, bias, B, P):
    L = tok.numel() // (B * P)
    conf = torch.empty((B, P, 2), device=tok.device, dtype=torch.float32)
    check(lib().lm_head_proposal_conf(_stream(), _ptr(tok), _ptr(wt), _ptr(bias), _ptr(conf), B * P, L))
    return conf


def pack_readback(tensors, block=None):
    offs, sizes, off = [], [], 0
    for t in tensors:
        assert t.is_contiguous()
        nb = t.numel() * t.element_size()
        assert nb % 4 == 0, 'lm_pack_segments copies 4-byte words'
        off = (off + 255) // 256 * 256
        offs.append(off); sizes.append(nb)
        off += nb
    if block is None or block.numel() < off or block.device != tensors[0].device:
        block = torch.empty(max(off, 1), device=tensors[0].device, dtype=torch.uint8)
    n = len(tensors)
    src = (C.c_void_p * n)(*[t.data_ptr() for t in tensors])
    nby = (C.c_long * n)(*sizes)
    dof = (C.c_long * n)(*offs)
    check(lib().lm_pack_segments(_stream(), n, src, nby, dof, _ptr(block)))
    return block, list(zip(offs, sizes))


def decode_proposals(pconf, ext2, cls2, off2, exist_thre, prop_width, half_buff):
    B, P, R, FW = cls2.shape
    assert FW == prop_width + 2 * half_buff and off2.shape[-1] == FW, 'cls2 / offset2 are prop_fea_width wide'
    dev = cls2.device
    prop_conf = torch.empty((B, P, 2), device=dev, dtype=torch.float32)
    v_ext = torch.empty((B, P, R), device=dev, dtype=torch.float32)
    cls_conf = torch.empty((B, P, R, FW), device=dev, dtype=torch.float32)
    cls_idx = torch.empty((B, P, R), device=dev, dtype=torch.int32)
    cls_offset = torch.empty((B, P, R), device=dev, dtype=torch.float64)
    check(lib().lm_decode_proposals(_stream(), _ptr(pconf.contiguous()), _ptr(ext2.contiguous()), _ptr(cls2.contiguous()),
                                    _ptr(off2.contiguous()), _ptr(prop_conf), _ptr(v_ext), _ptr(cls_conf), _ptr(cls_idx),
                                    _ptr(cls_offset), B, P, R, float(exist_thre), prop_width, half_buff))
    return prop_conf, v_ext, cls_conf, cls_idx, cls_offset


def decode_orient(orient_logits):
    x, ld = as_nhwc(orient_logits)
    B, C_, H, W = x.shape
    out = torch.empty((B, H, W), device=x.device, dtype=torch.uint8)
    check(lib().lm_decode_orient(_stream(), _ptr(x), ld, C_, _ptr(out), B * H * W))
    return out


def decode_semantic(logits_chw, thre, raw_mode=False, want_biseg=True):
    x = logits_chw.contiguous()
    B, C_, H, W = x.shape
    assert C_ == 3
    sem = torch.empty((B, H, W), device=x.device, dtype=torch.uint8)
    biseg = rows = None
    if want_biseg:
        biseg = torch.empty((B, H, W), device=x.device, dtype=torch.float32)
        rows = torch.empty((B, H // 8, W), device=x.device, dtype=torch.float32)
    check(lib().lm_decode_semantic(_stream(), _ptr(x), _ptr(sem), _ptr(biseg), _ptr(rows), B, H, W, float(thre), int(raw_mode)))
    return sem, biseg, rows


def endp_topk(endp_logits, K=512, clip=20):
    x = endp_logits.contiguous()
    B, C_, H, W = x.shape
    assert C_ == 1
    ws = torch.empty(lib().lm_endp_topk_workspace_bytes(B), device=x.device, dtype=torch.uint8)
    idx = torch.empty((B, K), device=x.device, dtype=torch.int32)
    score = torch.empty((B, K), device=x.device, dtype=torch.float32)
    status = torch.empty((B,), device=x.device, dtype=torch.int32)
    check(lib().lm_endp_topk(_stream(), _ptr(x), _ptr(ws), _ptr(idx), _ptr(score), _ptr(status), B, H, W, clip, K))
    return idx, score, status


def make_raster_params(quat=(1, 0, 0, 0), trans=(0, 0, 0), bev_img_offset=(0, 0), img_reso=(0.05, 0.05),
                       local_min_ele=0.0, ele_reso=0.05, inten_lo=800.0, inten_hi=33000.0):
    p = LmRasterParams()
    p.quat[:] = [float(v) for v in quat]
    p.trans[:] = [float(v) for v in trans]
    p.bev_img_offset[:] = [float(v) for v in bev_img_offset]
    p.img_reso[:] = [float(v) for v in img_reso]
    p.local_min_ele, p.ele_reso, p.inten_lo, p.inten_hi = float(local_min_ele), float(ele_reso), float(inten_lo), float(inten_hi)
    return p


_raster_ws = {}


def _workspace(points, need):
    key = (points.device, _stream().value)
    ws = _raster_ws.get(key)
    if ws is None or ws.numel() < need:
        ws = _raster_ws[key] = torch.empty(need, device=points.device, dtype=torch.uint8)
    return ws


def _tile_range_args(who, points, tile_offsets, params):
    if not points.is_cuda:
        _ptr(points)
    assert points.dim() == 2 and points.shape[1] == 4 and points.is_contiguous() and points.dtype == torch.float32
    B = len(params)
    if len(tile_offsets) != B + 1:
        raise ValueError(f'{who}: {len(tile_offsets)} tile_offsets for {B} tiles (B + 1 are needed)')
    offs = (C.c_long * (B + 1))(*[int(o) for o in tile_offsets])
    if B and offs[B] > points.shape[0]:
        raise ValueError(f'{who}: tile_offsets end at {offs[B]}, points has {points.shape[0]} rows')
    return B, offs, (LmRasterParams * B)(*params)


def bev_raster_batch(points, tile_offsets, params, H=1152, W=1152, out=None, want_u8=False, u8_only=False, out_u8=None, inten_scale=None):
    assert points.dim() == 2 and points.shape[1] == 4 and points.is_contiguous() and points.dtype == torch.float32
    B = len(params)
    assert len(tile_offsets) == B + 1
    offs = (C.c_long * (B + 1))(*[int(o) for o in tile_offsets])
    par = (LmRasterParams * B)(*params)
    cap = max([offs[b + 1] - offs[b] for b in range(B)] + [0])
    ws = _workspace(points, lib().lm_bev_raster_workspace_bytes(B, cap, H, W))
    want_u8 = want_u8 or u8_only or out_u8 is not None
    if out is None and not u8_only:
        out = torch.empty((B, 3, H, W), device=points.device, dtype=torch.float32)
    u8 = None
    if want_u8:
        u8 = out_u8 if out_u8 is not None else torch.empty((B, H, W, 3), device=points.device, dtype=torch.uint8)
        assert u8.dtype == torch.uint8 and u8.is_contiguous() and tuple(u8.shape) == (B, H, W, 3)
    if inten_scale is None:
        check(lib().lm_bev_raster_batch(_stream(), _ptr(points) if points.numel() else None, offs, par, B, _ptr(ws), ws.numel(),
                                        None if u8_only else _ptr(out), _ptr(u8), H, W))
    else:
        if len(inten_scale) != B:
            raise ValueError(f'bev_raster_batch: {len(inten_scale)} inten_scale entries for {B} tiles')
        scale = (C.c_float * B)(*[0.0 if v is None else float(v) for v in inten_scale])
        check(lib().lm_bev_raster_batch_scaled(_stream(), _ptr(points) if points.numel() else None, offs, par, B, _ptr(ws), ws.numel(),
                                               None if u8_only else _ptr(out), _ptr(u8), H, W, scale))
    if u8_only:
        return u8
    return (out, u8) if want_u8 else out


def bev_raster(points, params, H=1152, W=1152, want_u8=False):
    r = bev_raster_batch(points, [0, points.shape[0]], [params], H, W, want_u8=want_u8)
    return (r[0][0], r[1][0]) if want_u8 else r[0]


def strip_grid(params, H=1152, W=1152, z_range=None):
    import numpy as np
    T = len(params)
    par = (LmRasterParams * T)(*params)
    z_lo, z_hi = (float(z_range[0]), float(z_range[1])) if z_range is not None else (-math.inf, math.inf)
    g = LmStripGrid()
    check(lib().lm_strip_build_grid(par, T, H, W, z_lo, z_hi, C.byref(g), None, 0))
    cells = np.empty((g.ny, g.nx, 8), dtype=np.uint16)
    check(lib().lm_strip_build_grid(par, T, H, W, z_lo, z_hi, C.byref(g), C.c_void_p(cells.ctypes.data), g.nx * g.ny))
    return {'x0': g.x0, 'y0': g.y0, 'cell': g.cell, 'nx': g.nx, 'ny': g.ny}, cells


class LineIndex:

    def __init__(self, segments, cell_start, cell_segs, grid, half_width):
        self.segments, self.cell_start, self.cell_segs, self.grid, self.half_width = segments, cell_start, cell_segs, grid, half_width
        self.n_segments, self.n_lines = int(segments.shape[0]), int(grid.max_line)

    def args(self):
        S = self.n_segments
        return (_ptr(self.segments) if S else None, S, C.byref(self.grid), _ptr(self.cell_start) if S else None,
                _ptr(self.cell_segs) if S else None, float(self.half_width))


def line_index_host(segments, half_width, cell=None):
    import numpy as np
    seg = np.ascontiguousarray(segments, dtype=np.float32)
    if seg.ndim != 2 or seg.shape[1] != 8:
        raise ValueError(f'line_index: segments must be [S,8] float32 (las_io.line_segments), not {seg.shape}')
    S, g = int(seg.shape[0]), LmLineGrid()
    if cell is not None and not float(cell) > 0.0:
        raise ValueError(f'line_index: cell={cell!r} must be a size > 0 (None: the default)')
    cell = 0.0 if cell is None else float(cell)
    sp = C.c_void_p(seg.ctypes.data) if S else None
    check(lib().lm_line_index_build(sp, S, float(half_width), cell, C.byref(g), None, 0, None, 0))
    cell_start = np.zeros(g.nx * g.ny + 1, dtype=np.int32)
    cell_segs = np.zeros(max(int(g.n_entries), 1), dtype=np.int32)
    check(lib().lm_line_index_build(sp, S, float(half_width), cell, C.byref(g), C.c_void_p(cell_start.ctypes.data), cell_start.size,
                                    C.c_void_p(cell_segs.ctypes.data), cell_segs.size))
    return g, cell_start, cell_segs[:int(g.n_entries)]


def line_index(segments, half_width, cell=None, device='cuda:0'):
    import numpy as np
    seg = np.ascontiguousarray(segments, dtype=np.float32)
    g, cell_start, cell_segs = line_index_host(seg, half_width, cell)
    device = torch.device(device)
    if device.type != 'cuda':
        raise LanemapHipError('lanemapping_amd ops need tensors on an MI355X (HIP) device; no CPU fallback exists')
    up = lambda a: torch.from_numpy(np.array(a, order='C', copy=True)).to(device)
    return LineIndex(up(seg), up(cell_start), up(cell_segs), g, np.float32(half_width))


def label_points(points, index, z_tol, min_intensity=None, want_dist2=False):
    if not points.is_cuda:
        raise LanemapHipError('lanemapping_amd ops need tensors on an MI355X (HIP) device; no CPU fallback exists')
    assert points.dim() == 2 and points.shape[1] == 4 and points.is_contiguous() and points.dtype == torch.float32
    if not isinstance(index, LineIndex):
        raise TypeError(f'label_points: index must be an ops.LineIndex (ops.line_index), not {type(index).__name__}')
    N = int(points.shape[0])
    line = torch.empty((N,), device=points.device, dtype=torch.int32)
    dist2 = torch.empty((N,), device=points.device, dtype=torch.float32) if want_dist2 else None
    mi = math.nan if min_intensity is None else float(min_intensity)
    check(lib().lm_label_points(_stream(), _ptr(points) if N else None, N, *index.args(), float(z_tol), mi, _ptr(line) if N else None,
                                _ptr(dist2) if (want_dist2 and N) else None))
    return (line, dist2) if want_dist2 else line


class LineStations:

    def __init__(self, stations, bin_start, bin_start_host, bin):
        self.stations, self.bin_start, self.bin_start_host, self.bin = stations, bin_start, bin_start_host, float(bin)
        self.n_segments, self.n_lines, self.n_bins = int(stations.shape[0]), int(bin_start_host.shape[0]) - 1, int(bin_start_host[-1])

    def args(self):
        return (_ptr(self.stations) if self.n_segments else None, _ptr(self.bin_start), C.c_void_p(self.bin_start_host.ctypes.data),
                self.n_lines, self.bin)

    def new_bins(self):
        return torch.empty((self.n_bins, 6), device=self.bin_start.device, dtype=torch.int64)


def line_stations(stations, bin_start, bin, device='cuda:0'):
    import numpy as np
    st = np.ascontiguousarray(stations, dtype=np.float32)
    bs = np.array(bin_start, dtype=np.int32, order='C', copy=True)
    if st.ndim != 2 or st.shape[1] != 4 or bs.ndim != 1 or bs.shape[0] < 1:
        raise ValueError(f'line_stations: stations must be [S,4] float32 and bin_start [L + 1] int32, not {st.shape} and {bs.shape}')
    if not (math.isfinite(float(bin)) and float(bin) > 0.0):
        raise ValueError(f'line_stations: bin={bin!r} must be a finite length > 0')
    device = torch.device(device)
    if device.type != 'cuda':
        raise LanemapHipError('lanemapping_amd ops need tensors on an MI355X (HIP) device; no CPU fallback exists')
    return LineStations(torch.from_numpy(st.copy()).to(device), torch.from_numpy(bs).to(device), bs, bin)


def line_profile(points, index, stations, z_tol, min_intensity=None, out=None):
    if not points.is_cuda:
        raise LanemapHipError('lanemapping_amd ops need tensors on an MI355X (HIP) device; no CPU fallback exists')
    assert points.dim() == 2 and points.shape[1] == 4 and points.is_contiguous() and points.dtype == torch.float32
    if not isinstance(index, LineIndex):
        raise TypeError(f'line_profile: index must be an ops.LineIndex (ops.line_index), not {type(index).__name__}')
    if not isinstance(stations, LineStations):
        raise TypeError(f'line_profile: stations must be an ops.LineStations (ops.line_stations), not {type(stations).__name__}')
    if stations.n_segments != index.n_segments:
        raise ValueError(f'line_profile: stations hold {stations.n_segments} rows, the index {index.n_segments} segments')
    bins = _profile_out('line_profile', stations, out, points.device)
    N = int(points.shape[0])
    mi = math.nan if min_intensity is None else float(min_intensity)
    check(lib().lm_line_profile_points(_stream(), _ptr(points) if N else None, N, *index.args(), *stations.args(), float(z_tol), mi,
                                       int(out is not None), _ptr(bins) if stations.n_bins else None, stations.n_bins))
    return bins


def _profile_out(who, stations, out, device):
    if out is None:
        return stations.new_bins()
    if tuple(out.shape) != (stations.n_bins, 6) or out.dtype != torch.int64 or not out.is_contiguous() or out.device != device:
        raise ValueError(f'{who}: out must be a contiguous [{stations.n_bins},6] int64 tensor on {device}')
    return out


def _tilted(p):
    return p.quat[1] != 0.0 or p.quat[2] != 0.0


def strip_bin_points(points, params, H=1152, W=1152, z_range=None, capacity=None):
    if not points.is_cuda:
        _ptr(points)
    assert points.dim() == 2 and points.shape[1] == 4 and points.is_contiguous() and points.dtype == torch.float32
    T, N = len(params), points.shape[0]
    par = (LmRasterParams * T)(*params)
    if z_range is None and N and any(_tilted(p) for p in params):
        z = points[:, 2]
        z = z[torch.isfinite(z)]
        z_range = (float(z.min()), float(z.max())) if z.numel() else (0.0, 0.0)
    z_lo, z_hi = (float(z_range[0]), float(z_range[1])) if z_range is not None else (-math.inf, math.inf)
    if not (math.isfinite(z_lo) and math.isfinite(z_hi)) and any(_tilted(p) for p in params):
        if N:
            raise ValueError('strip_bin_points: tilted tiles need a finite z_range (or None: it is then taken from the points)')
        z_lo, z_hi = 0.0, 0.0
    need = lib().lm_strip_bin_workspace_bytes(N, T)
    if need <= 0:
        raise LanemapHipError(f'strip_bin_points: {T} tiles / {N} points are not supported (1 to 4096 tiles)')
    ws = _workspace(points, need)
    meta = torch.empty(2 * T + 1, device=points.device, dtype=torch.int64)
    offs = (C.c_long * (T + 1))()
    cap = int(capacity) if capacity is not None else N + N // 4
    binned = None
    for attempt in range(2):
        del binned
        binned = torch.empty((cap, 4), device=points.device, dtype=torch.float32)
        rc = lib().lm_strip_bin_points(_stream(), _ptr(points) if N else None, N, par, T, H, W, z_lo, z_hi, _ptr(ws), ws.numel(),
                                       C.c_void_p(meta.data_ptr()), C.c_void_p(meta.data_ptr() + 8 * T), offs, _ptr(binned) if cap else None, cap)
        if rc == 4 and attempt == 0 and capacity is None:
            cap = int(offs[T])
            continue
        check(rc)
        break
    return binned[:offs[T]], [int(o) for o in offs]


def tile_ground(points, tile_offsets, params, H=1152, W=1152, cell_px=32, want_cell_min=False):
    B, offs, par = _tile_range_args('tile_ground', points, tile_offsets, params)
    H, W, cell_px = int(H), int(W), int(cell_px)
    need = lib().lm_tile_ground_workspace_bytes(B, H, W, cell_px)
    Gy, Gx = (-(-H // cell_px), -(-W // cell_px)) if cell_px > 0 else (0, 0)
    ws = _workspace(points, max(need, 16))
    ground = torch.empty((B, Gy, Gx), device=points.device, dtype=torch.float32)
    gmin = torch.empty((B,), device=points.device, dtype=torch.float32)
    cmin = torch.empty_like(ground) if want_cell_min else None
    check(lib().lm_tile_ground(_stream(), _ptr(points) if points.numel() else None, offs, par, B, H, W, cell_px, _ptr(ws), ws.numel() if need else 0,
                               _ptr(ground), _ptr(gmin), _ptr(cmin)))
    return (ground, gmin, cmin) if want_cell_min else (ground, gmin)


def ground_select(points, tile_offsets, params, ground, H=1152, W=1152, cell_px=32, h_range=(-math.inf, math.inf)):
    B, offs, par = _tile_range_args('ground_select', points, tile_offsets, params)
    H, W, cell_px = int(H), int(W), int(cell_px)
    Gy, Gx = (-(-H // cell_px), -(-W // cell_px)) if cell_px > 0 else (0, 0)
    if tuple(ground.shape) != (B, Gy, Gx) or ground.dtype != torch.float32 or not ground.is_contiguous() or ground.device != points.device:
        raise ValueError(f'ground_select: ground must be a contiguous [{B},{Gy},{Gx}] float32 tensor on {points.device} (tile_ground\'s output)')
    N = int(offs[B] - offs[0]) if B else 0
    need = lib().lm_ground_select_workspace_bytes(max(N, 0), B)
    ws = _workspace(points, max(need, 16))
    out = torch.empty((max(N, 0), 4), device=points.device, dtype=torch.float32)
    doffs = torch.empty((B + 1,), device=points.device, dtype=torch.int64)
    hoffs = (C.c_long * (B + 1))()
    check(lib().lm_ground_select(_stream(), _ptr(points) if points.numel() else None, offs, par, B, H, W, cell_px, _ptr(ground),
                                 float(h_range[0]), float(h_range[1]), _ptr(ws), ws.numel() if need else 0, _ptr(out) if N > 0 else None,
                                 C.c_void_p(doffs.data_ptr()), hoffs))
    return out[:hoffs[B]], [int(o) for o in hoffs]


def tile_intensity_window(points, tile_offsets, params, H=1152, W=1152, percentiles=(1.0, 99.9), group=None, want_hist=False):
    B, offs, par = _tile_range_args('tile_intensity_window', points, tile_offsets, params)
    H, W = int(H), int(W)
    if group is None:
        G, grp = B, None
    else:
        if len(group) != B:
            raise ValueError(f'tile_intensity_window: {len(group)} group entries for {B} tiles')
        ids = [int(g) for g in group]
        if any(not 0 <= g < B for g in ids):
            bad = next(b for b, g in enumerate(ids) if not 0 <= g < B)
            raise ValueError(f'tile_intensity_window: group[{bad}]={ids[bad]} is outside 0..B-1={B - 1} (G = max(group) + 1 <= B)')
        grp = (C.c_int * B)(*ids)
        G = max(ids + [0]) + 1
    q_lo, q_hi = (int(round(float(p) * 1e4)) for p in percentiles)
    need = lib().lm_tile_intensity_workspace_bytes(B, G)
    ws = _workspace(points, max(need, 16))
    window = torch.empty((max(G, 0), 2), device=points.device, dtype=torch.int32)
    count = torch.empty((max(G, 0),), device=points.device, dtype=torch.int64)
    hist = torch.empty((max(G, 0), 4096), device=points.device, dtype=torch.int32) if want_hist else None
    check(lib().lm_tile_intensity_window(_stream(), _ptr(points) if points.numel() else None, offs, par, B, H, W, grp, G, q_lo, q_hi,
                                         _ptr(ws), ws.numel() if need else 0, _ptr(window), _ptr(count), _ptr(hist)))
    return (window, count, hist) if want_hist else (window, count)


def drape_vertices(points, tile_offsets, params, vertices, vertex_offsets, H=1152, W=1152, radius_px=4, want_pixel_min=False):
    import numpy as np
    B, offs, par = _tile_range_args('drape_vertices', points, tile_offsets, params)
    H, W, R = int(H), int(W), int(radius_px)
    vert = np.ascontiguousarray(np.asarray(vertices, dtype=np.int32).reshape(-1, 2))
    if len(vertex_offsets) != B + 1:
        raise ValueError(f'drape_vertices: {len(vertex_offsets)} vertex_offsets for {B} tiles (B + 1 are needed)')
    voffs = (C.c_long * (B + 1))(*[int(o) for o in vertex_offsets])
    if voffs[B] != vert.shape[0]:
        raise ValueError(f'drape_vertices: vertex_offsets end at {voffs[B]}, vertices has {vert.shape[0]} rows')
    V, D = vert.shape[0], 2 * max(R, 0) + 1
    need = lib().lm_drape_workspace_bytes(V, B, R)
    ws = _workspace(points, max(need, 16))
    z = torch.empty((V,), device=points.device, dtype=torch.float32)
    npix = torch.empty((V,), device=points.device, dtype=torch.int32)
    pmin = torch.empty((V, D, D), device=points.device, dtype=torch.float32) if want_pixel_min else None
    check(lib().lm_drape_vertices(_stream(), _ptr(points) if points.numel() else None, offs, par, B, H, W, C.c_void_p(vert.ctypes.data), voffs, R,
                                  _ptr(ws), ws.numel() if need else 0, _ptr(z), _ptr(npix), _ptr(pmin)))
    return (z, npix, pmin) if want_pixel_min else (z, npix)


def _gap_args(who, u8):
    if not u8.is_cuda:
        _ptr(u8)
    if u8.dtype != torch.uint8 or u8.dim() != 4 or u8.shape[3] != 3 or not u8.is_contiguous():
        raise ValueError(f'{who}: tiles must be a contiguous uint8 tensor [B,H,W,3], not {u8.dtype} {tuple(u8.shape)}'
                         + ('' if u8.is_contiguous() else ' (not contiguous)'))
    return int(u8.shape[0]), int(u8.shape[1]), int(u8.shape[2])


def tile_gap_hist(u8, max_radius_px=4):
    B, H, W = _gap_args('tile_gap_hist', u8)
    R = int(max_radius_px)
    hist = torch.empty((B, max(R, 0) + 2), device=u8.device, dtype=torch.int32)
    check(lib().lm_tile_gap_hist(_stream(), _ptr(u8), B, H, W, R, _ptr(hist)))
    return hist


def tile_gap_fill(u8, radius_px):
    B, H, W = _gap_args('tile_gap_fill', u8)
    radii = [int(r) for r in radius_px] if hasattr(radius_px, '__len__') else [int(radius_px)] * B
    if len(radii) != B:
        raise ValueError(f'tile_gap_fill: {len(radii)} radius_px entries for {B} tiles')
    out = torch.empty_like(u8)
    check(lib().lm_tile_gap_fill(_stream(), _ptr(u8), B, H, W, (C.c_int * B)(*radii), _ptr(out)))
    return out


def tile_ingest(u8_hwc):
    x = u8_hwc.contiguous()
    B, H, W, C_ = x.shape
    out = torch.empty((B, 3, H, W), device=x.device, dtype=torch.float32)
    check(lib().lm_tile_ingest_u8(_stream(), _ptr(x), _ptr(out), B, H, W, C_))
    return out


_vox_ws = {}


def exclusive_scan_u32(x, out=None):
    x = x.contiguous()
    assert x.dim() == 1 and x.dtype in (torch.int32, torch.uint32)
    out = torch.empty_like(x) if out is None else out
    n = x.numel()
    ws = torch.empty((lib().lm_scan_workspace_bytes(n),), device=x.device, dtype=torch.uint8)
    check(lib().lm_exclusive_scan_u32(_stream(), _ptr(x), _ptr(out), n, _ptr(ws), ws.numel()))
    return out


def sort_pairs_u32_(keys, vals, end_bit=32):
    assert keys.dim() == 1 and keys.shape == vals.shape and keys.is_contiguous() and vals.is_contiguous()
    assert keys.dtype in (torch.int32, torch.uint32) and vals.dtype in (torch.int32, torch.uint32)
    n = keys.numel()
    ws = torch.empty((lib().lm_sort_pairs_workspace_bytes(n),), device=keys.device, dtype=torch.uint8)
    check(lib().lm_sort_pairs_u32(_stream(), _ptr(keys), _ptr(vals), n, int(end_bit), _ptr(ws), ws.numel()))
    return keys, vals


def voxelize_batch(points, range_lo, voxel_size, grid_xyz, max_points, max_voxels, ldf=16, raster_order=False):
    dev = points[0].device
    B = len(points)
    cells = int(grid_xyz[0]) * int(grid_xyz[1]) * int(grid_xyz[2])
    caps = [min(int(p.shape[0]), int(max_voxels), cells) for p in points]
    cap = max(1, sum(caps))
    feats = torch.empty((cap, ldf), device=dev, dtype=torch.float32)
    coords = torch.empty((cap, 4), device=dev, dtype=torch.int32)
    ends = torch.zeros((B,), device=dev, dtype=torch.int32)
    nmax = max(int(p.shape[0]) for p in points)
    need = lib().lm_voxelize_workspace_bytes(nmax)
    key = (dev.index, _stream().value)
    ws = _vox_ws.get(key)
    if ws is None or ws.numel() < need:
        ws = torch.empty((need,), device=dev, dtype=torch.uint8)
        _vox_ws[key] = ws
    lo = (C.c_float * 3)(*[float(v) for v in range_lo])
    vs = (C.c_float * 3)(*[float(v) for v in voxel_size])
    g = (C.c_int * 3)(*[int(v) for v in grid_xyz])
    for b, p in enumerate(points):
        if not p.is_cuda:
            raise LanemapHipError('voxelize_batch needs device tensors; no CPU fallback exists')
        p = p.contiguous().float()
        assert p.dim() == 2 and p.shape[1] == 4
        base = C.c_void_p(ends[b - 1:b].data_ptr()) if b > 0 else None
        check(lib().lm_voxelize_hard(_stream(), _ptr(p) if p.shape[0] else None, p.shape[0], lo, vs, g, int(max_points),
                                     int(max_voxels), b, base, cap, _ptr(feats), ldf, _ptr(coords),
                                     C.c_void_p(ends[b:b + 1].data_ptr()), int(raster_order), _ptr(ws), ws.numel()))
    row_ends = [int(v) for v in ends.cpu()]
    V = row_ends[-1]
    return feats[:V], coords[:V], row_ends


def _ksp(kernel, stride, padding):
    return (C.c_int * 9)(*[int(v) for v in (*kernel, *stride, *padding)])


def sparse_grid(coords, B, shape):
    D, H, W = shape
    grid = torch.empty((B, D, H, W), device=coords.device, dtype=torch.int32)
    check(lib().lm_sparse_grid_build(_stream(), _ptr(coords), coords.shape[0], _ptr(grid), B, D, H, W))
    return grid


def sparse_conv_outputs(in_coords, B, in_shape, kernel, stride, padding):
    out_shape = tuple((in_shape[a] + 2 * padding[a] - kernel[a]) // stride[a] + 1 for a in range(3))
    Do, Ho, Wo = out_shape
    dev = in_coords.device
    cells = B * Do * Ho * Wo
    n_in = in_coords.shape[0]
    taps_per_axis = [(kernel[a] + stride[a] - 1) // stride[a] for a in range(3)]
    cap = max(1, min(cells, n_in * taps_per_axis[0] * taps_per_axis[1] * taps_per_axis[2]))
    grid = torch.empty((B, Do, Ho, Wo), device=dev, dtype=torch.int32)
    coords = torch.empty((cap, 4), device=dev, dtype=torch.int32)
    count = torch.zeros((1,), device=dev, dtype=torch.int32)
    need = lib().lm_sparse_conv_outputs_workspace_bytes(cells)
    ws = torch.empty((need,), device=dev, dtype=torch.uint8)
    check(lib().lm_sparse_conv_outputs(_stream(), _ptr(in_coords), n_in, B, _ksp(kernel, stride, padding), Do, Ho, Wo,
                                       _ptr(grid), _ptr(coords), cap, _ptr(count), _ptr(ws), need))
    n = int(count.item())
    if n > cap:
        raise LanemapHipError(f'sparse_conv_outputs: {n} active sites exceed the bound {cap}')
    return grid, coords[:n], out_shape


def sparse_rulebook(out_coords, in_grid, kernel, stride, padding):
    B, D, H, W = in_grid.shape
    taps = kernel[0] * kernel[1] * kernel[2]
    nbr = torch.empty((out_coords.shape[0], taps), device=out_coords.device, dtype=torch.int32)
    check(lib().lm_sparse_rulebook(_stream(), _ptr(out_coords), out_coords.shape[0], _ptr(in_grid), B, D, H, W,
                                   _ksp(kernel, stride, padding), _ptr(nbr)))
    return nbr


def pack_sparse(w):
    kd, kh, kw, ci, co = w.shape
    taps = kd * kh * kw
    cop = (co + 127) // 128 * 128
    wt = w.reshape(taps, ci, co).permute(0, 2, 1).float()
    if ci <= 16:
        p = torch.zeros(((taps + 1) // 2 * 2, cop, 16), device=w.device, dtype=torch.float32)
        p[:taps, :co, :ci] = wt
        return p.reshape(-1, 2, cop, 16).permute(0, 2, 1, 3).reshape(-1, cop, 32).contiguous()
    cip = (ci + 31) // 32 * 32
    p = torch.zeros((taps, cop, cip), device=w.device, dtype=torch.float32)
    p[:, :co, :ci] = wt
    return p.contiguous()


def sparse_ld(c):
    return 16 if c <= 16 else (c + 31) // 32 * 32


def conv_gather(x, nbr, wp, cin, cout, scale=None, shift=None, res=None, act=ACT_NONE):
    M, taps = nbr.shape
    cin_k = sparse_ld(cin)
    assert x.stride(1) == 1 and x.stride(0) >= cin_k
    ldy = sparse_ld(cout)
    y = torch.zeros((M, ldy), device=x.device, dtype=torch.float32) if ldy != cout else \
        torch.empty((M, ldy), device=x.device, dtype=torch.float32)
    def launch():
        check(lib().lm_conv_gather_mfma_f32(_stream(), _ptr(x), x.stride(0), _ptr(nbr), taps, _ptr(wp), wp.shape[1], _ptr(scale),
                                            _ptr(shift), _ptr(res), res.stride(0) if res is not None else 0, _ptr(y), ldy,
                                            M, cin_k, cout, act))
    if _conv_hook is not None:
        _conv_hook(f'spconv M{M} taps{taps} {cin}->{cout}', 2.0 * M * taps * cin * cout, launch)
    else:
        launch()
    return y


def sparse_to_dense(feats, coords, B, shape, C_, flip_h):
    D, H, W = shape
    out = new_act(B, C_ * D, H, W, feats.device)
    check(lib().lm_sparse_to_dense_nhwc(_stream(), _ptr(feats), feats.stride(0), _ptr(coords), feats.shape[0], _ptr(out),
                                        B, D, H, W, C_, int(flip_h)))
    return out


def upsample_bicubic(x, size):
    x, ld = as_nhwc(x)
    B, C_, H, W = x.shape
    assert ld == C_
    out = new_act(B, C_, size[0], size[1], x.device)
    check(lib().lm_upsample_bicubic_nhwc(_stream(), _ptr(x), _ptr(out), B, H, W, C_, size[0], size[1]))
    return out
```

lanemapping_amd/pcencoder.py:

```python
import os

import torch
import torch.nn as nn

from . import ops, trace
from .registry import PCENCODER
from .packing import PackedModule

_LAYERS = {'resnet18': [2, 2, 2, 2], 'resnet34': [3, 4, 6, 3]}
MERGE_BRANCH_CONVS = os.environ.get('LANEMAP_MERGE_BRANCH_CONVS', '1') != '0'
WINO_F44 = os.environ.get('LANEMAP_WINO_F44', '1') != '0'
WINO_F44_MIN_CIN = int(os.environ.get('LANEMAP_WINO_F44_MIN_CIN', '64'))
WINO_SPLIT = os.environ.get('LANEMAP_WINO_SPLIT', '0') != '0'


def _frag44(w):
    if WINO_SPLIT:
        return ops.pack_wino44_fragments_split(ops.pack_wino44(w))
    return ops.pack_wino44_fragments(ops.pack_wino44(w))


def _f44_ok(conv):
    return WINO_F44 and conv.kernel_size == (3, 3) and conv.stride == (1, 1) and conv.in_channels >= WINO_F44_MIN_CIN and conv.in_channels % 16 == 0


class _ResBlock(nn.Module):

    def __init__(self, cin, cout, stride, dilation, with_down):
        super().__init__()
        self.conv1 = nn.Conv2d(cin, cout, 3, stride, dilation, dilation, bias=False)
        self.bn1 = nn.BatchNorm2d(cout)
        self.conv2 = nn.Conv2d(cout, cout, 3, 1, dilation, dilation, bias=False)
        self.bn2 = nn.BatchNorm2d(cout)
        self.downsample = nn.Sequential(nn.Conv2d(cin, cout, 1, stride, bias=False), nn.BatchNorm2d(cout)) if with_down else None
        self.stride, self.dilation = stride, dilation


def _stage(state, planes, blocks, stride, dilate):
    prev_dil = state[1]
    if dilate:
        state[1] *= stride
        stride = 1
    layers = [_ResBlock(state[0], planes, stride, prev_dil, stride != 1 or state[0] != planes)]
    state[0] = planes
    for _ in range(1, blocks):
        layers.append(_ResBlock(planes, planes, 1, state[1], False))
    return nn.Sequential(*layers)


class _BottomUp(nn.Module):

    def __init__(self, layers, dil, in_channels):
        super().__init__()
        self.conv1 = nn.Conv2d(3, 64, 7, 2, 3, bias=False)
        self.bn1 = nn.BatchNorm2d(64)
        st = [64, 1]
        self.layer1 = _stage(st, in_channels[0], layers[0], 1, False)
        self.layer2 = _stage(st, in_channels[1], layers[1], 2, dil[0])
        if in_channels[2] > 0:
            self.layer3 = _stage(st, in_channels[2], layers[2], 2, dil[1])
        if in_channels[3] > 0:
            self.layer4 = _stage(st, in_channels[3], layers[3], 2, dil[2])


class FPNEncoder(PackedModule):
    def __init__(self, resnet='resnet34', pretrained=False, replace_stride_with_dilation=(False, True, False),
                 out_conv=True, in_channels=(64, 128, 256, -1), cfg=None):
        super().__init__()
        if resnet not in _LAYERS:
            raise NotImplementedError(f'{resnet}: only BasicBlock ResNets are on the hot path')
        if in_channels[2] <= 0 or in_channels[3] > 0:
            raise NotImplementedError('hot path covers in_channels=[c1,c2,c3,-1] (all BASELINE configs)')
        dil = list(replace_stride_with_dilation)
        if len(dil) != 3:
            raise ValueError(f'replace_stride_with_dilation should be None or a 3-element tuple, got {dil}')
        layers = _LAYERS[resnet]
        self.cfg = cfg
        self.in_channels = list(in_channels)
        self.model_buttomup = _BottomUp(layers, dil, in_channels)
        self.conv1 = nn.Conv2d(3, 64, 7, 2, 3, bias=False)
        self.bn1 = nn.BatchNorm2d(64)
        st = [64, 1]
        self.layer1 = _stage(st, in_channels[0], layers[0], 1, False)
        self.layer2 = _stage(st, in_channels[1], layers[1], 2, dil[0])
        self.layer3 = _stage(st, in_channels[2], layers[2], 2, dil[1])
        c = st[0]
        self.out = nn.Conv2d(c, cfg.featuremap_out_channel, 1, bias=False) if out_conv else None
        self.toplayer = nn.Conv2d(c, 256, 1)
        self.smooth1 = nn.Conv2d(c, c, 3, 1, 1)
        self.smooth2 = nn.Conv2d(c, c, 3, 1, 1)
        self.smooth3 = nn.Conv2d(c, c, 3, 1, 1)
        self.latlayer1 = nn.Conv2d(in_channels[1], c, 1)
        self.latlayer2 = nn.Conv2d(in_channels[0], c, 1)
        self.semantic_branch = nn.Conv2d(c, c // 2, 3, 1, 1)
        self.semantic_branch2 = nn.Conv2d(c, c // 2, 3, 1, 1)
        self.conv2 = nn.Conv2d(c, c, 3, 1, 1)
        self.conv3 = nn.Conv2d(c, c, 3, 1, 1)
        self.feature_layer = nn.Conv2d(c // 2, 8, 1)
        self.output_layer_binary_seg = nn.Conv2d(8, 3, 1)
        self.output_layer_endp = nn.Conv2d(c // 2, 1, 1)
        self.gn11 = nn.GroupNorm(c // 2, c // 2)
        self.gn12 = nn.GroupNorm(c, c)
        self.gn21 = nn.GroupNorm(c // 2, c // 2)
        self.gn22 = nn.GroupNorm(c, c)

    def _pack(self):
        P = {}
        P['stem_w'] = self.conv1.weight.permute(2, 3, 1, 0).contiguous().float()
        P['stem_s'], P['stem_b'] = ops.fold_bn(self.bn1)
        for lname in ('layer1', 'layer2', 'layer3'):
            for i, blk in enumerate(getattr(self, lname)):
                k = f'{lname}.{i}'
                P[k + '.w1'] = ops.pack_mfma(blk.conv1.weight)
                P[k + '.s1'], P[k + '.b1'] = ops.fold_bn(blk.bn1)
                P[k + '.w2'] = ops.pack_mfma(blk.conv2.weight)
                P[k + '.s2'], P[k + '.b2'] = ops.fold_bn(blk.bn2)
                for q, conv in (('.w1q', blk.conv1), ('.w2q', blk.conv2)):
                    if _f44_ok(conv):
                        P[k + q] = _frag44(conv.weight)
                if blk.downsample is not None:
                    P[k + '.wd'] = ops.pack_mfma(blk.downsample[0].weight)
                    P[k + '.sd'], P[k + '.bd'] = ops.fold_bn(blk.downsample[1])
        for name in ('toplayer', 'smooth1', 'smooth2', 'smooth3', 'latlayer1', 'latlayer2', 'semantic_branch',
                     'semantic_branch2', 'conv2', 'conv3'):
            m = getattr(self, name)
            P[name + '.w'] = ops.pack_mfma(m.weight)
            P[name + '.b'] = m.bias.float().contiguous()
            if _f44_ok(m):
                P[name + '.wq'] = _frag44(m.weight)
        a, b2 = self.semantic_branch, self.semantic_branch2
        if (MERGE_BRANCH_CONVS and 'semantic_branch.wq' in P and 'semantic_branch2.wq' in P and a.out_channels == b2.out_channels
                and self.gn11.eps == self.gn21.eps):
            P['semantic_branch_ab.wq'] = _frag44(torch.cat([a.weight, b2.weight], dim=0))
            P['semantic_branch_ab.b'] = torch.cat([a.bias, b2.bias]).float().contiguous()
            if ('conv2.wq' in P and 'conv3.wq' in P and self.conv2.out_channels == self.conv3.out_channels
                    and self.gn12.eps == self.gn22.eps):
                P['conv23.wq'] = _frag44(torch.cat([self.conv2.weight, self.conv3.weight], dim=0))
                P['conv23.b'] = torch.cat([self.conv2.bias, self.conv3.bias]).float().contiguous()
        if self.out is not None:
            P['out.w'] = ops.pack_mfma(self.out.weight)
        for name in ('feature_layer', 'output_layer_binary_seg', 'output_layer_endp'):
            m = getattr(self, name)
            P[name + '.w'] = ops.pack_small(m.weight)
            P[name + '.b'] = m.bias.float().contiguous()
        for name in ('gn11', 'gn12', 'gn21', 'gn22'):
            m = getattr(self, name)
            P[name + '.g'], P[name + '.b'] = m.weight.float().contiguous(), m.bias.float().contiguous()
        return P

    @staticmethod
    def _c3(x, P, wkey, cout, stride, dil, **epi):
        if (wkey + 'q') in P and stride == 1 and ops.wino44_supported(x.shape[2], x.shape[3], x.shape[1], dil):
            return ops.conv_wino44(x, P[wkey + 'q'], cout, dil, **epi)
        return ops.conv_mfma(x, P[wkey], cout, 3, 3, stride, dil, dil, **epi)

    def _block(self, x, P, key, blk):
        cout = blk.conv1.out_channels
        y = self._c3(x, P, key + '.w1', cout, blk.stride, blk.dilation, scale=P[key + '.s1'], shift=P[key + '.b1'], act=ops.ACT_RELU)
        if blk.downsample is not None:
            x = ops.conv_mfma(x, P[key + '.wd'], cout, 1, 1, blk.stride, 0, 1, scale=P[key + '.sd'], shift=P[key + '.bd'])
        return self._c3(y, P, key + '.w2', cout, 1, blk.dilation, scale=P[key + '.s2'], shift=P[key + '.b2'], res=x, act=ops.ACT_RELU)

    def _conv3(self, x, P, name, cout):
        return self._c3(x, P, name + '.w', cout, 1, 1, shift=P[name + '.b'])

    def _conv_stats(self, P, src, conv, cout, gn):
        eps = getattr(self, gn).eps
        if (conv + '.wq') in P and ops.wino44_supported(src.shape[2], src.shape[3], src.shape[1], 1):
            return ops.conv_wino44(src, P[conv + '.wq'], cout, 1, shift=P[conv + '.b'], gn_eps=eps)
        if (src.shape[2] * src.shape[3]) % 128 == 0:
            return ops.conv_mfma_gnstats(src, P[conv + '.w'], cout, 3, 3, 1, 1, 1, P[conv + '.b'], eps)
        t = self._conv3(src, P, conv, cout)
        return t, ops.gn_stats(t, eps)

    def _semantic(self, P, p2, p3, p4, conv_a, gn_a, conv_b, gn_b, proj, pre=None, pre_a4=None):
        h, w = p2.shape[2:]
        c_half = self.semantic_branch.out_channels
        t, st = pre_a4 if pre_a4 is not None else self._conv_stats(P, p4, conv_a, p4.shape[1], gn_a)
        s4 = ops.gn_relu_upsample_sum([(t, st)], P[gn_a + '.g'], P[gn_a + '.b'], (h, w))
        terms = [pre[0] if pre is not None and pre[0] is not None else self._conv_stats(P, p2, conv_b, c_half, gn_b),
                 pre[1] if pre is not None and pre[1] is not None else self._conv_stats(P, p3, conv_b, c_half, gn_b)]
        terms.append(self._conv_stats(P, s4, conv_b, c_half, gn_b))
        return ops.gn_relu_upsample_sum(terms, P[gn_b + '.g'], P[gn_b + '.b'], (h, w), proj=proj, keep_sum=False)

    def forward(self, x, fea_up_out=None):
        from . import torch_ops
        if self.out is None:
            return self._forward_impl(x, fea_up_out)
        if fea_up_out is None:
            B, H, W = (x.shape[0], x.shape[1], x.shape[2]) if x.dtype == torch.uint8 else (x.shape[0], x.shape[2], x.shape[3])
            fea_up_out = ops.new_act(B, 8, (H + 3) // 4, (W + 3) // 4, x.device)
        fea, bi_seg, endp = torch_ops.fpn_encoder(x, fea_up_out, torch_ops.stage_weights(self), torch_ops.stage_name(self))
        return fea, fea_up_out, bi_seg, endp

    def _forward_impl(self, x, fea_up_out=None):
        P = self.packed()
        if x.dtype == torch.uint8:
            B, H, W, _ = x.shape
        else:
            B, _, H, W = x.shape
        with trace.stage('fpn.stem'):
            c1 = ops.maxpool3x3s2(ops.stem(x, P['stem_w'], P['stem_s'], P['stem_b']))
        feats = []
        t = c1
        for lname in ('layer1', 'layer2', 'layer3'):
            with trace.stage('fpn.' + lname):
                for i, blk in enumerate(getattr(self, lname)):
                    t = self._block(t, P, f'{lname}.{i}', blk)
            feats.append(t)
        c2, c3, c4 = feats
        trace.push('fpn.topdown')
        fea = ops.conv_mfma(c4, P['out.w'], self.out.out_channels) if self.out is not None else None
        p4 = ops.conv_mfma(c4, P['toplayer.w'], 256, shift=P['toplayer.b'])
        def lateral(c, name, coarse):
            if tuple(coarse.shape[2:]) == tuple(c.shape[2:]):
                return ops.conv_mfma(c, P[name + '.w'], 256, shift=P[name + '.b'], res=coarse)
            return ops.conv_mfma(c, P[name + '.w'], 256, shift=P[name + '.b'], res_up=coarse)

        p3 = lateral(c3, 'latlayer1', p4)
        p2 = lateral(c2, 'latlayer2', p3)
        del c1, c2, c3, c4, feats, t
        p4 = self._conv3(p4, P, 'smooth1', 256)
        p3 = self._conv3(p3, P, 'smooth2', 256)
        p2 = self._conv3(p2, P, 'smooth3', 256)
        trace.pop()
        trace.push('fpn.semantic')
        pre_a, pre_b = [None, None], [None, None]
        if 'semantic_branch_ab.wq' in P:
            ch = self.semantic_branch.out_channels
            for i, src in enumerate((p2, p3)):
                if ops.wino44_supported(src.shape[2], src.shape[3], src.shape[1], 1):
                    t, st = ops.conv_wino44(src, P['semantic_branch_ab.wq'], 2 * ch, 1, shift=P['semantic_branch_ab.b'],
                                            gn_eps=self.gn11.eps, gn_split=2)
                    pre_a[i], pre_b[i] = (t[:, :ch], st[0]), (t[:, ch:], st[1])
        a4 = b4 = None
        if 'conv23.wq' in P and ops.wino44_supported(p4.shape[2], p4.shape[3], p4.shape[1], 1):
            c4o = self.conv2.out_channels
            t, st = ops.conv_wino44(p4, P['conv23.wq'], 2 * c4o, 1, shift=P['conv23.b'], gn_eps=self.gn12.eps, gn_split=2)
            a4, b4 = (t[:, :c4o], st[0]), (t[:, c4o:], st[1])
        fea_up = self._semantic(P, p2, p3, p4, 'conv2', 'gn12', 'semantic_branch', 'gn11',
                                (P['feature_layer.w'], P['feature_layer.b'], 8, fea_up_out), pre_a, a4)
        seg288 = ops.conv_small(fea_up, P['output_layer_binary_seg.w'], 3, shift=P['output_layer_binary_seg.b'], pre_relu=True)
        bi_seg = ops.upsample_to_chw(seg288, (H, W))
        endp288 = self._semantic(P, p2, p3, p4, 'conv3', 'gn22', 'semantic_branch2', 'gn21',
                                 (P['output_layer_endp.w'], P['output_layer_endp.b'], 1, None), pre_b, b4)
        endp = ops.upsample_to_chw(endp288, (H, W))
        trace.pop()
        return fea, fea_up, bi_seg, endp


@PCENCODER.register_module
class PostProjector2(nn.Module):
    def __init__(self, resnet='resnet50', pretrained=False, replace_stride_with_dilation=[False, True, False],
                 out_conv=True, in_channels=[64, 128, 256, -1], cfg=None):
        super().__init__()
        self.cfg = cfg
        self.fpn = FPNEncoder(resnet=resnet, pretrained=pretrained, replace_stride_with_dilation=replace_stride_with_dilation,
                              out_conv=out_conv, in_channels=in_channels, cfg=cfg)

    def forward(self, sample):
        return self.fpn(sample['proj'])

    def infer_validate(self, preds, seg_thre=None, endp_thre=None, display=None):
        from .decode import segmentor_decode
        return segmentor_decode(preds['seg'], preds['endp'], seg_thre)
```

Before: 391.2 tiles/s.

## Use buffer-resource loads for Winograd patch gathers and unroll units by parity

Replaces the per-load 64-bit global pointers (with a zero-page fallback for padding) in the Winograd 4x4 conv kernel with a per-image buffer resource and 32-bit voffsets. Out-of-range taps are sent to a large offset so the hardware's bounds check returns zero. The unit loop is unrolled by buffer parity so LDS column pointers become compile-time selections, and some MFMA groups are deferred past the mid barrier. The aim is to cut address VGPRs and integer work in the hot loop, at the cost of a 2^31-byte per-image limit, which now needs an ldx-aware support check and a Python fallback path.

```diff
diff --git a/include/lanemap_hip.h b/include/lanemap_hip.h
--- a/include/lanemap_hip.h
+++ b/include/lanemap_hip.h
@@ -22,6 +22,7 @@
                                   int dil, int act);
 
 int lm_winograd44_supported(int H, int W, int Cin, int dil);
+int lm_winograd44_supported_ld(int H, int W, int Cin, int dil, int ldx);
 int lm_winograd44_gn_chunks(int H, int W, int dil);
 long lm_winograd44_tiles(int B, int H, int W, int dil);
 long lm_winograd44_twin_workspace_bytes(int B, int H, int W, int Cin, int CoutP, int dil);
diff --git a/lanemapping_amd/_lib.py b/lanemapping_amd/_lib.py
--- a/lanemapping_amd/_lib.py
+++ b/lanemapping_amd/_lib.py
@@ -42,6 +42,7 @@
     'lm_conv2d_nhwc_mfma_resup_f32': (i32, [vp, vp, i32, vp, i32, vp, vp, vp, i32, i32, i32, vp, i32,
                                             i32, i32, i32, i32, i32, i32, i32, i32, i32, i32, i32, i32]),
     'lm_winograd44_supported': (i32, [i32, i32, i32, i32]),
+    'lm_winograd44_supported_ld': (i32, [i32, i32, i32, i32, i32]),
     'lm_winograd44_gn_chunks': (i32, [i32, i32, i32]),
     'lm_winograd44_tiles': (i64, [i32, i32, i32, i32]),
     'lm_winograd44_twin_workspace_bytes': (i64, [i32, i32, i32, i32, i32, i32]),
diff --git a/lanemapping_amd/csrc/conv_wino44.hip b/lanemapping_amd/csrc/conv_wino44.hip
--- a/lanemapping_amd/csrc/conv_wino44.hip
+++ b/lanemapping_amd/csrc/conv_wino44.hip
@@ -28,7 +28,8 @@
 constexpr int QBD = 5, QRING = 6;
 static_assert(6 * (QNCELL / 16) * QGRP <= QRAWF && QNCELL % 16 == 0, "patch loads cover the unit");
 
-__device__ __attribute__((aligned(16))) float g_w44_zeros[1024 + 32];
+constexpr unsigned QPADOFF = 0x80000000u;
+typedef __amdgpu_buffer_rsrc_t w44_rsrc_t;
 
 struct W44Geom {
     int B, H, W, dil, Ty, Tx;
@@ -211,7 +212,7 @@
 }
 
 struct W44Params {
-    const float* x; const float* U; const float* scale; const float* shift; const float* res; float* y; const float* zeros;
+    const float* x; const float* U; const float* scale; const float* shift; const float* res; float* y;
     int ldx, ldr, ldy, C, Cout, NT, act;
     int n_inner;
     LmFastDiv dnt;
@@ -243,6 +244,10 @@
 
 struct W44K {
     f32x2 c2, c4, c5;
+};
+template <int V>
+struct W44Int {
+    static constexpr int value = V;
 };
 
 __device__ __forceinline__ void pk_bt(const f32x2 (&d)[6], f32x2 (&t)[6], const W44K& k) {
@@ -263,9 +268,9 @@
     f32x2 tA[6], tB[6], tC[6];
 };
 template <int C>
-__device__ __forceinline__ void w44_preread(W44Xf& d, const float* rawrow, const int (&roff)[6]) {
+__device__ __forceinline__ void w44_preread(W44Xf& d, const float* const (&col)[6]) {
     constexpr int ROWF = (QNCELL / 16) * QGRP;
-    const float* s = rawrow + roff[C];
+    const float* s = col[C];
 #pragma unroll
     for (int r = 0; r < 5; ++r) d.e[C][r] = *reinterpret_cast<const f32x2*>(s + r * ROWF);
 }
@@ -306,17 +311,17 @@
     }
 }
 template <int K, bool SPLIT>
-__device__ __forceinline__ void w44_xf_lds(W44Xf& d, const float* rawrow, const int (&roff)[6], float* vA, float* vB, float* vC) {
+__device__ __forceinline__ void w44_xf_lds(W44Xf& d, const float* const (&col)[6], float* vA, float* vB, float* vC) {
     auto st = [](float* v, int j, const f32x2 t) { w44_vstore<SPLIT>(v, j, t); };
     if constexpr (K == 0) {
         st(vB, 2, d.tB[2]); st(vB, 5, d.tB[5]);
-        w44_preread<0>(d, rawrow, roff); w44_preread<1>(d, rawrow, roff);
+        w44_preread<0>(d, col); w44_preread<1>(d, col);
     } else if constexpr (K == 1) {
         st(vC, 0, d.tC[0]); st(vC, 1, d.tC[1]);
-        w44_preread<2>(d, rawrow, roff); w44_preread<3>(d, rawrow, roff);
+        w44_preread<2>(d, col); w44_preread<3>(d, col);
     } else if constexpr (K == 2) {
         st(vC, 2, d.tC[2]); st(vC, 3, d.tC[3]);
-        w44_preread<4>(d, rawrow, roff); w44_preread<5>(d, rawrow, roff);
+        w44_preread<4>(d, col); w44_preread<5>(d, col);
     } else if constexpr (K == 3) {
         st(vC, 4, d.tC[4]); st(vC, 5, d.tC[5]);
     } else if constexpr (K == 5) {
@@ -341,10 +346,10 @@
     }
 }
 template <bool SPLIT>
-__device__ __forceinline__ void w44_xf_all(W44Xf& d, const float* rawrow, const int (&roff)[6], float* vA, float* vB, float* vC, bool lower,
+__device__ __forceinline__ void w44_xf_all(W44Xf& d, const float* const (&col)[6], float* vA, float* vB, float* vC, bool lower,
                                            const W44K& k) {
-    w44_preread<0>(d, rawrow, roff); w44_preread<1>(d, rawrow, roff); w44_preread<2>(d, rawrow, roff);
-    w44_preread<3>(d, rawrow, roff); w44_preread<4>(d, rawrow, roff); w44_preread<5>(d, rawrow, roff);
+    w44_preread<0>(d, col); w44_preread<1>(d, col); w44_preread<2>(d, col);
+    w44_preread<3>(d, col); w44_preread<4>(d, col); w44_preread<5>(d, col);
     w44_xf_valu<1>(d, lower, k); w44_xf_valu<2>(d, lower, k); w44_xf_valu<3>(d, lower, k);
     w44_xf_valu<4>(d, lower, k); w44_xf_valu<5>(d, lower, k); w44_xf_valu<6>(d, lower, k);
 #pragma unroll
@@ -356,9 +361,11 @@
 }
 
 __device__ __forceinline__ void q_bload2(f32x4 (&b)[2], unsigned voff, const float* sbase) {
-    asm volatile("global_load_dwordx4 %0, %2, %3\n\t"
-                 "global_load_dwordx4 %1, %2, %3 offset:1024"
-                 : "=&v"(b[0]), "=&v"(b[1]) : "v"(voff), "s"(sbase) : "memory");
+    unsigned long base;
+    asm volatile("s_mov_b64 %2, %4\n\t"
+                 "global_load_dwordx4 %0, %3, %2\n\t"
+                 "global_load_dwordx4 %1, %3, %2 offset:1024"
+                 : "=&v"(b[0]), "=&v"(b[1]), "=&s"(base) : "v"(voff), "s"(sbase) : "memory");
 }
 template <int N>
 __device__ __forceinline__ void q_bwait(f32x4 (&b)[2]) {
@@ -389,28 +396,46 @@
 static_assert(q_dma0(17) + q_ndma(17) == QLPW, "the second phase issues every patch load of a unit");
 
 template <bool SPLIT>
-__device__ __forceinline__ f32x4 q_aread(const float* v) {
+__device__ __forceinline__ f32x4 q_aread(const float* v, const float* v1) {
     if constexpr (SPLIT) {
         return f32x4{v[0], v[32], v[128], v[160]};
     } else {
-        const f32x2 lo = *reinterpret_cast<const f32x2*>(v), hi = *reinterpret_cast<const f32x2*>(v + 64);
+        const f32x2 lo = *reinterpret_cast<const f32x2*>(v), hi = *reinterpret_cast<const f32x2*>(v1);
         return f32x4{lo[0], lo[1], hi[0], hi[1]};
+    }
+}
+
+__device__ __forceinline__ float* w44_lds_hide(float* p) {
+    typedef __attribute__((address_space(3))) float lds_float;
+    unsigned a = (unsigned)(unsigned long)(lds_float*)p;
+    asm volatile("" : "+v"(a));
+    return (float*)(lds_float*)(unsigned long)a;
+}
+
+constexpr bool w44_deferred(int S) { return S == 4 || S == 8 || S == 13; }
+template <int S>
+__device__ __forceinline__ void w44_step_rest(f32x16& acc0, f32x16& acc1, const f32x4 (&b)[2], const f32x4& a_cur) {
+    constexpr bool VACC = S % 9 == 8;
+    q_mfma<VACC>(acc1, a_cur[0], b[1][0]);
+#pragma unroll
+    for (int t = 1; t < 4; ++t) {
+        q_mfma<VACC>(acc0, a_cur[t], b[0][t]);
+        q_mfma<VACC>(acc1, a_cur[t], b[1][t]);
     }
 }
 
 template <int S, bool SPLIT>
 __device__ __forceinline__ void w44_step(f32x16& acc0, f32x16& acc1, f32x4 (&bq)[QRING][2], unsigned bvoff, const float* bpre,
-                                         const float* anext, const f32x4& a_cur, f32x4& a_nxt, const float* const (&gsrc)[QLPW], long goff,
-                                         float* rawld, int wave, W44Xf& xf, const float* prerow, const int (&roff)[6], float* vA, float* vB,
+                                         const float* anext, const float* anext1, const f32x4& a_cur, f32x4& a_nxt, const w44_rsrc_t grsrc, const unsigned (&gvoff)[QLPW], int gsoff,
+                                         float* rawld, int wave, W44Xf& xf, const float* const (&col)[6], float* vA, float* vB,
                                          float* vC, bool lower, const W44K& kk) {
-    typedef __attribute__((address_space(1))) const void gptr_t;
     typedef __attribute__((address_space(3))) void lptr_t;
     constexpr int K = S % 9;
     q_bload2(bq[(S + QBD) % QRING], bvoff, bpre);
 #pragma unroll
     for (int i = 0; i < q_ndma(S); ++i) {
         constexpr int L0 = q_dma0(S);
-        __builtin_amdgcn_global_load_lds((gptr_t*)(gsrc[L0 + i] + goff), (lptr_t*)(rawld + ((L0 + i) * 4 + wave) * QGRP), 16, 0, 0);
+        __builtin_amdgcn_raw_ptr_buffer_load_lds(grsrc, (lptr_t*)(rawld + ((L0 + i) * 4 + wave) * QGRP), 16, gvoff[L0 + i], gsoff, 0, 0);
     }
     f32x4 (&b)[2] = bq[S % QRING];
     q_bwait<q_nwait(S)>(b);
@@ -419,8 +444,8 @@
     if constexpr (SPLIT) q_mfma16<VACC>(acc0, a_hi, f32x2{b[0][0], b[0][1]});
     else q_mfma<VACC>(acc0, a_cur[0], b[0][0]);
     if constexpr (!SPLIT) __builtin_amdgcn_sched_barrier(0);
-    if constexpr (K != 4 && K != 8) a_nxt = q_aread<SPLIT>(anext);
-    w44_xf_lds<K, SPLIT>(xf, prerow, roff, vA, vB, vC);
+    if constexpr (K != 4 && K != 8) a_nxt = q_aread<SPLIT>(anext, anext1);
+    w44_xf_lds<K, SPLIT>(xf, col, vA, vB, vC);
     if constexpr (!SPLIT) __builtin_amdgcn_sched_barrier(0);
     w44_xf_valu<K>(xf, lower, kk);
     if constexpr (!SPLIT) __builtin_amdgcn_sched_barrier(0);
@@ -438,13 +463,8 @@
                 __builtin_amdgcn_sched_group_barrier(0x300, 3, 0);
             }
         }
-    } else {
-        q_mfma<VACC>(acc1, a_cur[0], b[1][0]);
-#pragma unroll
-        for (int t = 1; t < 4; ++t) {
-            q_mfma<VACC>(acc0, a_cur[t], b[0][t]);
-            q_mfma<VACC>(acc1, a_cur[t], b[1][t]);
-        }
+    } else if constexpr (!w44_deferred(S)) {
+        w44_step_rest<S>(acc0, acc1, b, a_cur);
     }
     __builtin_amdgcn_sched_barrier(0);
 }
@@ -486,7 +506,6 @@
     extern __shared__ __attribute__((aligned(16))) float smem[];
     float* const raw0 = smem;
     float* const Vbuf = smem + 2 * QRAWF;
-    typedef __attribute__((address_space(1))) const void gptr_t;
     typedef __attribute__((address_space(3))) void lptr_t;
     const int tid = threadIdx.x, lane = tid & 63;
     const int wave = __builtin_amdgcn_readfirstlane(tid >> 6);
@@ -546,8 +565,10 @@
         }
         ts[QSEG] = at;
     }
-    const float* gsrc[QLPW];
+    unsigned gvoff[QLPW];
     const int img_pix0 = bi * g.H * g.W;
+    const w44_rsrc_t grsrc = __builtin_amdgcn_make_buffer_rsrc(const_cast<float*>(p.x) + (long)img_pix0 * p.ldx, 0,
+                                                               (int)((((long)g.H * g.W - 1) * p.ldx + p.C) * 4), 0x00020000);
     int tab_x, tab_y, tab_n;
     {
         int n = sn[0], yb = iy0[0], xb = ix0[0], s0 = 0;
@@ -574,11 +595,8 @@
         const int nn = __builtin_amdgcn_ds_bpermute(idx, tab_n);
         const int yy = y0 + r * g.dil, xx = x0 + gccd;
         const bool ok = (r < 6) & (gcc < nn) & ((unsigned)yy < (unsigned)g.H) & ((unsigned)xx < (unsigned)g.W);
-        const long m = -(long)ok;
-        const long eoff = ((long)(img_pix0 + yy * g.W + xx) * p.ldx) & m;
-        const unsigned long base = (unsigned long)p.zeros + (((unsigned long)p.x - (unsigned long)p.zeros) & (unsigned long)m);
-        gsrc[s_] = (const float*)base + eoff + gcq4;
-        __builtin_amdgcn_global_load_lds((gptr_t*)gsrc[s_], (lptr_t*)(raw0 + (s_ * 4 + wave) * QGRP), 16, 0, 0);
+        gvoff[s_] = ok ? ((unsigned)(yy * g.W + xx) * (unsigned)p.ldx + (unsigned)gcq4) * 4u : QPADOFF;
+        __builtin_amdgcn_raw_ptr_buffer_load_lds(grsrc, (lptr_t*)(raw0 + (s_ * 4 + wave) * QGRP), 16, gvoff[s_], 0, 0, 0);
         __builtin_amdgcn_sched_barrier(0);
     }
     int roff[6], tvoff;
@@ -598,14 +616,30 @@
         tvoff = SPLIT ? cp * 32 + tl : cp * 64 + tl * 2;
     }
     const bool lower = (wave >> 1) != 0;
-    float* const vA = Vbuf + (lower ? 3 : 0) * (6 * 256) + tvoff;
-    float* const vB = Vbuf + (lower ? 4 : 1) * (6 * 256) + tvoff;
-    float* const vC = Vbuf + (lower ? 5 : 2) * (6 * 256) + tvoff;
+    const float* rbo[2][4];
+    {
+        const int lowoff = lower ? (QNCELL / 16) * QGRP : 0;
+#pragma unroll
+        for (int par = 0; par < 2; ++par) {
+            rbo[par][0] = w44_lds_hide(raw0 + par * QRAWF + lowoff + roff[0]);
+            rbo[par][1] = w44_lds_hide(raw0 + par * QRAWF + lowoff + roff[1]);
+            rbo[par][2] = w44_lds_hide(raw0 + par * QRAWF + lowoff + roff[4]);
+            rbo[par][3] = w44_lds_hide(raw0 + par * QRAWF + lowoff + roff[5]);
+        }
+    }
+#define LM_QCOL(PAR, K, F) rbo[PAR][K] + (F)
+#define LM_QCOLS(PAR, HALF8)                                                                                                  \
+    {LM_QCOL(PAR, 0, HALF8), LM_QCOL(PAR, 1, HALF8), LM_QCOL(PAR, 0, 128 + (HALF8)), LM_QCOL(PAR, 1, 128 + (HALF8)), \
+     LM_QCOL(PAR, 2, HALF8), LM_QCOL(PAR, 3, HALF8)}
+    float* const vA = w44_lds_hide(Vbuf + (lower ? 3 : 0) * (6 * 256) + tvoff);
+    float* const vB = w44_lds_hide(Vbuf + (lower ? 4 : 1) * (6 * 256) + tvoff);
+    float* const vC = w44_lds_hide(Vbuf + (lower ? 5 : 2) * (6 * 256) + tvoff);
     const W44K kk = {f32x2{2.f, 2.f}, f32x2{4.f, 4.f}, f32x2{5.f, 5.f}};
     const int qa = wave >> 1, qb = wave & 1;
     const int xi00 = 18 * qa + 3 * qb;
-    const float* const Vq = SPLIT ? Vbuf + xi00 * 256 + (lane >> 5) * 64 + (lane & 31)
-                                  : Vbuf + xi00 * 256 + (lane >> 5) * 128 + (lane & 31) * 2;
+    const float* const Vq = w44_lds_hide(SPLIT ? Vbuf + xi00 * 256 + (lane >> 5) * 64 + (lane & 31)
+                                               : Vbuf + xi00 * 256 + (lane >> 5) * 128 + (lane & 31) * 2);
+    const float* const Vq1 = SPLIT ? Vq : w44_lds_hide(Vbuf + xi00 * 256 + (lane >> 5) * 128 + (lane & 31) * 2 + 64);
     const int nun = p.C / 16;
     const unsigned bvoff = (unsigned)lane * 16u;
     const long ustride = (long)p.NT * 256;
@@ -621,61 +655,85 @@
             for (int r = 0; r < 16; ++r) acc[k][b][r] = 0.f;
     f32x4 bq[QRING][2];
     W44Xf xf;
-    const int lowoff = lower ? (QNCELL / 16) * QGRP : 0;
 #define LM_QXI(K) (6 * ((K) / 3) + (K) % 3)
 #pragma unroll
     for (int k = 0; k < QBD; ++k) q_bload2(bq[k], bvoff, bbase + (long)LM_QXI(k) * xstride);
     {
-        const long goff1 = nun > 1 ? 16 : 0;
+        const int gsoff1 = nun > 1 ? 64 : 0;
 #pragma unroll
         for (int s_ = 0; s_ < QLPW; ++s_)
-            __builtin_amdgcn_global_load_lds((gptr_t*)(gsrc[s_] + goff1), (lptr_t*)(raw0 + QRAWF + (s_ * 4 + wave) * QGRP), 16, 0, 0);
+            __builtin_amdgcn_raw_ptr_buffer_load_lds(grsrc, (lptr_t*)(raw0 + QRAWF + (s_ * 4 + wave) * QGRP), 16, gvoff[s_], gsoff1, 0, 0);
     }
     q_bwait<QLPW>(bq[0]);
     __builtin_amdgcn_s_barrier();
-    w44_xf_all<SPLIT>(xf, raw0 + lowoff, roff, vA, vB, vC, lower, kk);
+    {
+        const float* const col0[6] = LM_QCOLS(0, 0);
+        w44_xf_all<SPLIT>(xf, col0, vA, vB, vC, lower, kk);
+    }
     asm volatile("s_waitcnt lgkmcnt(0)" ::: "memory");
     __builtin_amdgcn_s_barrier();
 
 #define LM_QBPRE(S5) ((S5) < 18 ? bu + (long)((S5) / 9) * ustride + (long)LM_QXI((S5) % 9) * xstride : bu_next + (long)LM_QXI((S5) - 18) * xstride)
+#define LM_QANEXT(S) (LM_QXI(((S) % 9) + 1 < 9 ? ((S) % 9) + 1 : 0) * 256)
 #define LM_QSTEP(S, AC, AN) \
-    w44_step<S, SPLIT>(acc[(S) % 9][0], acc[(S) % 9][1], bq, bvoff, LM_QBPRE((S) + QBD), Vq + LM_QXI(((S) % 9) + 1 < 9 ? ((S) % 9) + 1 : 0) * 256, \
-                AC, AN, gsrc, goff, rawc_w, wave, xf, (S) < 9 ? rawc + 8 + lowoff : rawn + lowoff, roff, vA, vB, vC, lower, kk)
+    w44_step<S, SPLIT>(acc[(S) % 9][0], acc[(S) % 9][1], bq, bvoff, LM_QBPRE((S) + QBD), Vq + LM_QANEXT(S), Vq1 + LM_QANEXT(S), \
+                AC, AN, grsrc, gvoff, gsoff, rawc_w, wave, xf, (S) < 9 ? colc : coln, vA, vB, vC, lower, kk)
 #define LM_QMID(AN)                                          \
     asm volatile("s_waitcnt lgkmcnt(0)" ::: "memory");       \
     __builtin_amdgcn_s_barrier();                            \
-    AN = q_aread<SPLIT>(Vq + LM_QXI(5) * 256);
-    for (int u = 0; u < nun; ++u) {
-        const float* const rawc = raw0 + (u & 1) * QRAWF;
-        float* const rawc_w = raw0 + (u & 1) * QRAWF;
-        const float* const rawn = raw0 + ((u + 1) & 1) * QRAWF;
-        const long goff = u + 2 < nun ? (long)(u + 2) * 16 : 0;
+    AN = q_aread<SPLIT>(Vq + LM_QXI(5) * 256, Vq1 + LM_QXI(5) * 256); \
+    __builtin_amdgcn_sched_barrier(0);
+#define LM_QREST(S, AC)                                                                               \
+    if constexpr (!SPLIT) {                                                                           \
+        w44_step_rest<S>(acc[(S) % 9][0], acc[(S) % 9][1], bq[(S) % QRING], AC);                      \
+        __builtin_amdgcn_sched_barrier(0);                                                            \
+    }
+    auto unit = [&](auto par_, const int u) __attribute__((always_inline)) {
+        constexpr int PAR = decltype(par_)::value;
+        const float* const colc[6] = LM_QCOLS(PAR, 8);
+        const float* const coln[6] = LM_QCOLS(PAR ^ 1, 0);
+        float* const rawc_w = raw0 + PAR * QRAWF;
+        const int gsoff = u + 2 < nun ? (u + 2) * 64 : 0;
         const float* const bu = bbase + (long)(2 * u) * ustride;
         const float* const bu_next = bbase + (long)(u + 1 < nun ? 2 * (u + 1) : 0) * ustride;
         f32x4 a0, a1;
-        a0 = q_aread<SPLIT>(Vq);
+        a0 = q_aread<SPLIT>(Vq, Vq1);
         LM_QSTEP(0, a0, a1); LM_QSTEP(1, a1, a0); LM_QSTEP(2, a0, a1); LM_QSTEP(3, a1, a0); LM_QSTEP(4, a0, a1);
         LM_QMID(a1)
+        LM_QREST(4, a0)
         LM_QSTEP(5, a1, a0); LM_QSTEP(6, a0, a1); LM_QSTEP(7, a1, a0); LM_QSTEP(8, a0, a1);
         asm volatile("s_waitcnt lgkmcnt(0)" ::: "memory");
         q_bwait<2 * 9>(bq[0]);
         __builtin_amdgcn_s_barrier();
-        a0 = q_aread<SPLIT>(Vq);
-        LM_QSTEP(9, a0, a1);  LM_QSTEP(10, a1, a0); LM_QSTEP(11, a0, a1); LM_QSTEP(12, a1, a0); LM_QSTEP(13, a0, a1);
-        LM_QMID(a1)
-        LM_QSTEP(14, a1, a0); LM_QSTEP(15, a0, a1); LM_QSTEP(16, a1, a0); LM_QSTEP(17, a0, a1);
+        a1 = q_aread<SPLIT>(Vq, Vq1);
+        __builtin_amdgcn_sched_barrier(0);
+        LM_QREST(8, a0)
+        LM_QSTEP(9, a1, a0);  LM_QSTEP(10, a0, a1); LM_QSTEP(11, a1, a0); LM_QSTEP(12, a0, a1); LM_QSTEP(13, a1, a0);
+        LM_QMID(a0)
+        LM_QREST(13, a1)
+        LM_QSTEP(14, a0, a1); LM_QSTEP(15, a1, a0); LM_QSTEP(16, a0, a1); LM_QSTEP(17, a1, a0);
         asm volatile("s_waitcnt lgkmcnt(0)" ::: "memory");
         __builtin_amdgcn_s_barrier();
-    }
+    };
+    for (int u = 0; u + 1 < nun; u += 2) {
+        unit(W44Int<0>{}, u);
+        unit(W44Int<1>{}, u + 1);
+    }
+    if (nun & 1) unit(W44Int<0>{}, nun - 1);
+#undef LM_QCOLS
+#undef LM_QCOL
+#undef LM_QREST
 #undef LM_QMID
 #undef LM_QSTEP
+#undef LM_QANEXT
 #undef LM_QBPRE
 #undef LM_QXI
     static_assert(18 % QRING == 0 && QBD < QRING, "eighteen steps per unit walk the ring a whole number of times");
 #pragma unroll
     for (int k = 0; k < QRING; ++k) q_bwait<0>(bq[k]);
 
-    const int etile = tid >> 3, ecq = tid & 7;
+    const int elane = (int)__builtin_amdgcn_mbcnt_hi(~0u, __builtin_amdgcn_mbcnt_lo(~0u, 0u)), etid = wave * 64 + elane;
+    const int etile = etid >> 3, ecq = etid & 7;
     int epix0;
     int eny = 0, enx = 0;
     {
@@ -692,7 +750,7 @@
             enx = min(4, (int)lm_fastdiv((unsigned)(g.W - ox + g.dil - 1), g.ddil));
         }
     }
-    float* const mw = smem + xi00 * 1024 + (4 * (lane >> 5)) * 32 + (lane & 31);
+    float* const mw = smem + xi00 * 1024 + (4 * (elane >> 5)) * 32 + (elane & 31);
     const float* const mr = smem + etile * 32 + ecq * 4;
     f32x4 gsum[2] = {{0.f, 0.f, 0.f, 0.f}, {0.f, 0.f, 0.f, 0.f}}, gsq[2] = {{0.f, 0.f, 0.f, 0.f}, {0.f, 0.f, 0.f, 0.f}};
     const bool full = eny == 4 && enx == 4;
@@ -789,17 +847,17 @@
                     gsq[blk][e] += __shfl_xor(gsq[blk][e], o);
                 }
         __syncthreads();
-        if (lane < 8) {
+        if (elane < 8) {
 #pragma unroll
             for (int blk = 0; blk < 2; ++blk) {
-                *reinterpret_cast<f32x4*>(smem + (((wave * 2 + blk) * 8 + lane) * 2) * 4) = gsum[blk];
-                *reinterpret_cast<f32x4*>(smem + (((wave * 2 + blk) * 8 + lane) * 2 + 1) * 4) = gsq[blk];
+                *reinterpret_cast<f32x4*>(smem + (((wave * 2 + blk) * 8 + elane) * 2) * 4) = gsum[blk];
+                *reinterpret_cast<f32x4*>(smem + (((wave * 2 + blk) * 8 + elane) * 2 + 1) * 4) = gsq[blk];
             }
         }
         __syncthreads();
-        if (tid < 16) {
+        if (etid < 16) {
 #pragma clang fp contract(off)
-            const int blk = tid >> 3, cq = tid & 7;
+            const int blk = etid >> 3, cq = etid & 7;
             const int n = n0 + blk * 32 + cq * 4;
             f32x4 s = {0.f, 0.f, 0.f, 0.f}, q = {0.f, 0.f, 0.f, 0.f};
 #pragma unroll
@@ -824,26 +882,16 @@
 
 bool w44_ok(const W44Geom& g) { return (QBM - 2) / g.Tx + 2 <= QSEG; }
 
-int w44_zeros(const float** out) {
-    static const float* cache[64] = {nullptr};
-    int dev = 0;
-    LM_HIP(hipGetDevice(&dev));
-    LM_REQUIRE(dev >= 0 && dev < 64, "conv_wino44: device index %d", dev);
-    if (!cache[dev]) {
-        void* sym = nullptr;
-        LM_HIP(hipGetSymbolAddress(&sym, HIP_SYMBOL(g_w44_zeros)));
-        cache[dev] = (const float*)sym;
-    }
-    *out = cache[dev];
-    return LM_OK;
-}
-
-}
-
-LM_API int lm_winograd44_supported(int H, int W, int Cin, int dil) {
-    if (dil < 1 || H < 1 || W < 1 || Cin < 16 || Cin % 16 != 0 || Cin > 1024) return 0;
-    return w44_ok(geom44(1, H, W, dil)) ? 1 : 0;
-}
+bool w44_image_ok(int H, int W, int Cin, int ldx) { return ((long)H * W - 1) * ldx * 4 + (long)Cin * 4 < (1L << 31); }
+
+}
+
+LM_API int lm_winograd44_supported_ld(int H, int W, int Cin, int dil, int ldx) {
+    if (dil < 1 || H < 1 || W < 1 || Cin < 16 || Cin % 16 != 0 || Cin > 1024 || ldx < Cin) return 0;
+    return w44_ok(geom44(1, H, W, dil)) && w44_image_ok(H, W, Cin, ldx) ? 1 : 0;
+}
+
+LM_API int lm_winograd44_supported(int H, int W, int Cin, int dil) { return lm_winograd44_supported_ld(H, W, Cin, dil, Cin); }
 
 LM_API int lm_winograd44_gn_chunks(int H, int W, int dil) { return dil < 1 ? 0 : geom44(1, H, W, dil).Tpad / 32; }
 
@@ -859,6 +907,7 @@
                       int Cin, int Cout, int dil, int act, double* gn_partial, float split_post) {
     LM_REQUIRE(x && wu_frag && y, "conv_wino44: null pointer");
     LM_REQUIRE(lm_winograd44_supported(H, W, Cin, dil) && B > 0, "conv_wino44: unsupported shape (H=%d W=%d Cin=%d dil=%d)", H, W, Cin, dil);
+    LM_REQUIRE(w44_image_ok(H, W, Cin, ldx), "conv_wino44: an image of the input spans 2^31 bytes or more (H=%d W=%d ldx=%d): use the direct kernel", H, W, ldx);
     LM_REQUIRE(CoutP >= Cout && CoutP % QBN == 0, "conv_wino44: CoutP=%d must be Cout=%d rounded up to %d", CoutP, Cout, QBN);
     LM_REQUIRE(ldx >= Cin && ldx % 4 == 0 && ldy >= Cout, "conv_wino44: bad leading dimension");
     LM_REQUIRE(act == LM_ACT_NONE || act == LM_ACT_RELU, "conv_wino44: activation %d not supported", act);
@@ -869,7 +918,6 @@
     p.x = x; p.U = wu_frag; p.scale = scale; p.shift = shift; p.res = res; p.y = y;
     p.ldx = ldx; p.ldr = ldr; p.ldy = ldy; p.C = Cin; p.Cout = Cout; p.NT = CoutP / 32; p.act = act;
     p.gn_part = gn_partial;
-    if (int e = w44_zeros(&p.zeros)) return e;
     static const int order = getenv("LANEMAP_W44_ORDER") ? atoi(getenv("LANEMAP_W44_ORDER")) : 1;
     p.n_inner = order;
     p.dnt = lm_fastdiv_make((unsigned)((Cout + QBN - 1) / QBN));
diff --git a/lanemapping_amd/ops.py b/lanemapping_amd/ops.py
--- a/lanemapping_amd/ops.py
+++ b/lanemapping_amd/ops.py
@@ -27,14 +27,19 @@
     return torch.empty((B, H, W, C_), device=device, dtype=dtype).permute(0, 3, 1, 2)
 
 
-def as_nhwc(x):
+def nhwc_ld(x):
     B, C_, H, W = x.shape
     sb, sc, sh, sw = x.stride()
     ok = (sc == 1 or C_ == 1) and sw >= C_ and (sh == W * sw or H == 1) and (sb == H * W * sw or B == 1)
-    if not ok:
+    return sw if ok else None
+
+
+def as_nhwc(x):
+    ld = nhwc_ld(x)
+    if ld is None:
         x = x.permute(0, 2, 3, 1).contiguous().permute(0, 3, 1, 2)
-        sw = C_
-    return x, sw
+        ld = x.shape[1]
+    return x, ld
 
 
 def fold_bn(bn, conv_bias=None, eps=1e-5):
@@ -175,8 +180,12 @@
         launch()
 
 
-def wino44_supported(H, W, cin, dil=1):
-    return bool(lib().lm_winograd44_supported(int(H), int(W), int(cin), int(dil)))
+def wino44_supported(H, W, cin, dil=1, ldx=None):
+    return bool(lib().lm_winograd44_supported_ld(int(H), int(W), int(cin), int(dil), int(cin if ldx is None else ldx)))
+
+
+def wino44_covers(x, dil=1):
+    return wino44_supported(x.shape[2], x.shape[3], x.shape[1], dil, nhwc_ld(x))
 
 
 def conv_wino44(x, wf, cout, dil=1, scale=None, shift=None, res=None, act=ACT_NONE, out=None, gn_eps=None, gn_split=1):
diff --git a/lanemapping_amd/pcencoder.py b/lanemapping_amd/pcencoder.py
--- a/lanemapping_amd/pcencoder.py
+++ b/lanemapping_amd/pcencoder.py
@@ -150,7 +150,7 @@
 
     @staticmethod
     def _c3(x, P, wkey, cout, stride, dil, **epi):
-        if (wkey + 'q') in P and stride == 1 and ops.wino44_supported(x.shape[2], x.shape[3], x.shape[1], dil):
+        if (wkey + 'q') in P and stride == 1 and ops.wino44_covers(x, dil):
             return ops.conv_wino44(x, P[wkey + 'q'], cout, dil, **epi)
         return ops.conv_mfma(x, P[wkey], cout, 3, 3, stride, dil, dil, **epi)
 
@@ -166,7 +166,7 @@
 
     def _conv_stats(self, P, src, conv, cout, gn):
         eps = getattr(self, gn).eps
-        if (conv + '.wq') in P and ops.wino44_supported(src.shape[2], src.shape[3], src.shape[1], 1):
+        if (conv + '.wq') in P and ops.wino44_covers(src):
             return ops.conv_wino44(src, P[conv + '.wq'], cout, 1, shift=P[conv + '.b'], gn_eps=eps)
         if (src.shape[2] * src.shape[3]) % 128 == 0:
             return ops.conv_mfma_gnstats(src, P[conv + '.w'], cout, 3, 3, 1, 1, 1, P[conv + '.b'], eps)
@@ -229,12 +229,12 @@
         if 'semantic_branch_ab.wq' in P:
             ch = self.semantic_branch.out_channels
             for i, src in enumerate((p2, p3)):
-                if ops.wino44_supported(src.shape[2], src.shape[3], src.shape[1], 1):
+                if ops.wino44_covers(src):
                     t, st = ops.conv_wino44(src, P['semantic_branch_ab.wq'], 2 * ch, 1, shift=P['semantic_branch_ab.b'],
                                             gn_eps=self.gn11.eps, gn_split=2)
                     pre_a[i], pre_b[i] = (t[:, :ch], st[0]), (t[:, ch:], st[1])
         a4 = b4 = None
-        if 'conv23.wq' in P and ops.wino44_supported(p4.shape[2], p4.shape[3], p4.shape[1], 1):
+        if 'conv23.wq' in P and ops.wino44_covers(p4):
             c4o = self.conv2.out_channels
             t, st = ops.conv_wino44(p4, P['conv23.wq'], 2 * c4o, 1, shift=P['conv23.b'], gn_eps=self.gn12.eps, gn_split=2)
             a4, b4 = (t[:, :c4o], st[0]), (t[:, c4o:], st[1])
```

New measurement: 397.5 tiles/s (median of 6 runs). 1.6% higher.
